# razvanmatisan/duodiff

Measured on AMD Instinct MI355X. Metric: images/sec (whole node) DuoDiff 1000-step CelebA-64, higher is better.
Workload: dtype bf16

## Files before the change

duodiff_amd/_lib.py:

```python
import ctypes as C
import os
from pathlib import Path

LIB_PATH = Path(os.environ.get("DUODIFF_LIB") or Path(__file__).resolve().parent / "libduodiff.so")

DD_OK = 0
DD_ERR_INVALID, DD_ERR_NOT_FOUND, DD_ERR_STATE, DD_ERR_HIP, DD_ERR_NOMEM, DD_ERR_UNSUPPORTED = -1, -2, -3, -4, -5, -6
DD_PREC_BF16, DD_PREC_FP32 = 0, 1
DD_VAR_BETA_TILDE, DD_VAR_BETA = 0, 1
DD_NOISE_NONE, DD_NOISE_BUFFER, DD_NOISE_PHILOX = 0, 1, 2
DD_X0_STATIC, DD_X0_DYNAMIC = 0, 1
DD_EE_MLP_PER_LAYER, DD_EE_MLP_PER_TIMESTEP, DD_EE_MLP_PER_LAYER_PER_TIMESTEP, DD_EE_ATTENTION_PROBE = 0, 1, 2, 3
ABI_VERSION = 6
DD_DEV_NO_FUSED_MLP, DD_DEV_NO_FUSED_PROJ, DD_DEV_NO_FUSED_HEAD, DD_DEV_GENERIC_EMBED, DD_DEV_MLP_EXTRAS_ONLY = 1, 2, 4, 8, 16
DD_DEV_NO_FUSED_SKIP, DD_DEV_NO_FUSED_QKV, DD_DEV_NO_FUSED_QA = 32, 64, 128
DD_PROF_DOMINANT, DD_PROF_BLOCK_TAIL, DD_PROF_FC1, DD_PROF_ROWLIN, DD_PROF_QKV_ATTENTION, DD_PROF_SPLITK = 0, 1, 2, 3, 4, 5
DD_DEV_NO_CHAINS, DD_DEV_FORCE_CHAINS, DD_DEV_NO_ROWLIN, DD_DEV_NO_ROWLIN_PROJ, DD_DEV_NO_EMBED_LN, DD_DEV_NO_SPLITK, DD_DEV_NO_ROWLIN_SKIP = 256, 512, 1024, 2048, 4096, 8192, 16384
DD_DEV_NO_SPLIT_HEADS = 32768


class dd_config(C.Structure):
    _fields_ = [(n, C.c_int32) for n in (
        "img_size", "patch_size", "in_chans", "embed_dim", "depth", "num_heads", "mlp_ratio",
        "num_classes", "normalize_timesteps", "max_batch", "qkv_bias", "mlp_time_embed")]


class dd_sample_args(C.Structure):
    _fields_ = [("first", C.c_void_p), ("late", C.c_void_p), ("t_switch", C.c_int32),
                ("t_start", C.c_int32), ("t_end", C.c_int32), ("variance", C.c_int32),
                ("noise_mode", C.c_int32), ("use_graph", C.c_int32), ("seed", C.c_uint64),
                ("y_dev", C.c_void_p), ("x_dev", C.c_void_p), ("B", C.c_int32), ("reserved", C.c_int32)]


class dd_affine_sample_args(C.Structure):
    _fields_ = [("first", C.c_void_p), ("late", C.c_void_p), ("n_steps", C.c_int32), ("switch_after", C.c_int32),
                ("t", C.POINTER(C.c_float)), ("a", C.POINTER(C.c_float)), ("b", C.POINTER(C.c_float)),
                ("c", C.POINTER(C.c_float)), ("noise", C.POINTER(C.c_int32)), ("noise_mode", C.c_int32),
                ("use_graph", C.c_int32), ("seed", C.c_uint64), ("y_dev", C.c_void_p), ("x_dev", C.c_void_p),
                ("B", C.c_int32), ("counter_base", C.c_int32)]


class dd_multistep_sample_args(C.Structure):
    _fields_ = dd_affine_sample_args._fields_ + [
        ("d", C.POINTER(C.c_float)), ("p", C.POINTER(C.c_float)), ("q", C.POINTER(C.c_float)), ("hist", C.POINTER(C.c_int32)),
        ("h_dev", C.c_void_p)]


class dd_guidance(C.Structure):
    _fields_ = [("scale", C.c_float), ("null_label", C.c_int32)]


class dd_autoguidance(C.Structure):
    _fields_ = [("guide", C.c_void_p), ("scale", C.c_float)]


class dd_pag(C.Structure):
    _fields_ = [("scale", C.c_float), ("layers_first", C.c_uint32), ("layers_late", C.c_uint32)]


class dd_known_region(C.Structure):
    _fields_ = [("x0_dev", C.c_void_p), ("mask_dev", C.c_void_p), ("ka", C.POINTER(C.c_float)), ("kb", C.POINTER(C.c_float))]


class dd_x0_threshold(C.Structure):
    _fields_ = [("mode", C.c_int32), ("quantile", C.c_float), ("range", C.c_float), ("s_max", C.c_float)]


class dd_ee_sample_args(C.Structure):
    _fields_ = [("model", C.c_void_p), ("threshold", C.c_float), ("t_start", C.c_int32), ("t_end", C.c_int32),
                ("noise_mode", C.c_int32), ("use_graph", C.c_int32), ("B", C.c_int32), ("seed", C.c_uint64),
                ("y_dev", C.c_void_p), ("x_dev", C.c_void_p), ("err_dev", C.c_void_p), ("idx_dev", C.c_void_p)]


SIGNATURES = {
    "dd_abi_version": (C.c_int, []),
    "dd_build_id": (C.c_char_p, []),
    "dd_ctx_create": (C.c_int, [C.c_int, C.POINTER(C.c_void_p)]),
    "dd_ctx_destroy": (None, [C.c_void_p]),
    "dd_last_error": (C.c_char_p, [C.c_void_p]),
    "dd_sync": (C.c_int, [C.c_void_p, C.c_void_p]),
    "dd_schedule_table": (C.c_int, [C.c_int, C.POINTER(C.c_float)]),
    "dd_schedule_build": (C.c_int, [C.c_float, C.c_float, C.c_int] + [C.POINTER(C.c_float)] * 5),
    "dd_model_create": (C.c_int, [C.c_void_p, C.POINTER(dd_config), C.POINTER(C.c_void_p)]),
    "dd_model_set_param": (C.c_int, [C.c_void_p, C.c_char_p, C.c_void_p, C.POINTER(C.c_int64), C.c_int]),
    "dd_model_finalize": (C.c_int, [C.c_void_p, C.c_int]),
    "dd_model_num_params": (C.c_int64, [C.c_void_p]),
    "dd_model_destroy": (None, [C.c_void_p]),
    "dd_forward": (C.c_int, [C.c_void_p, C.c_void_p, C.c_void_p, C.c_float, C.c_void_p, C.c_void_p, C.c_void_p, C.c_int, C.c_void_p]),
    "dd_model_enable_early_exit": (C.c_int, [C.c_void_p, C.c_int]),
    "dd_forward_early_exit": (C.c_int, [C.c_void_p, C.c_void_p, C.c_void_p, C.c_float, C.c_void_p, C.c_void_p, C.c_void_p,
                                        C.c_void_p, C.c_void_p, C.c_int, C.c_void_p]),
    "dd_early_exit_select": (C.c_int, [C.c_void_p, C.c_void_p, C.c_void_p, C.c_void_p, C.c_float, C.c_int, C.c_int, C.c_int64,
                                       C.c_void_p, C.c_void_p, C.c_void_p, C.c_void_p]),
    "dd_ddpm_step": (C.c_int, [C.c_void_p, C.c_void_p, C.c_void_p, C.c_void_p, C.c_int, C.c_int, C.c_void_p, C.c_int64, C.c_void_p]),
    "dd_ddpm_step_coef": (C.c_int, [C.c_void_p, C.c_void_p, C.c_void_p, C.c_void_p, C.c_float, C.c_float, C.c_float,
                                    C.c_void_p, C.c_int64, C.c_void_p]),
    "dd_affine_step": (C.c_int, [C.c_void_p, C.c_void_p, C.c_void_p, C.c_void_p, C.c_float, C.c_float, C.c_float,
                                 C.c_void_p, C.c_int64, C.c_void_p]),
    "dd_sample_step": (C.c_int, [C.c_void_p, C.c_void_p, C.c_void_p, C.c_int, C.c_void_p, C.c_int, C.c_void_p,
                                 C.c_uint64, C.c_int, C.c_void_p, C.c_int, C.c_void_p]),
    "dd_to_images": (C.c_int, [C.c_void_p, C.c_void_p, C.c_void_p, C.c_int, C.c_int, C.c_int, C.c_void_p]),
    "dd_sample": (C.c_int, [C.c_void_p, C.POINTER(dd_sample_args), C.c_void_p]),
    "dd_sample_affine": (C.c_int, [C.c_void_p, C.POINTER(dd_affine_sample_args), C.c_void_p]),
    "dd_sample_early_exit": (C.c_int, [C.c_void_p, C.POINTER(dd_ee_sample_args), C.c_void_p]),
    "dd_forward_guided": (C.c_int, [C.c_void_p, C.c_void_p, C.c_void_p, C.c_float, C.c_void_p, C.POINTER(dd_guidance), C.c_void_p,
                                    C.c_int, C.c_void_p]),
    "dd_sample_guided": (C.c_int, [C.c_void_p, C.POINTER(dd_sample_args), C.POINTER(dd_guidance), C.c_void_p]),
    "dd_sample_affine_guided": (C.c_int, [C.c_void_p, C.POINTER(dd_affine_sample_args), C.POINTER(dd_guidance), C.c_void_p]),
    "dd_multistep_step": (C.c_int, [C.c_void_p, C.c_void_p, C.c_void_p, C.c_void_p, C.c_void_p] + [C.c_float] * 6 +
                          [C.c_int, C.c_void_p, C.c_int64, C.c_void_p]),
    "dd_sample_multistep": (C.c_int, [C.c_void_p, C.POINTER(dd_multistep_sample_args), C.c_void_p]),
    "dd_sample_multistep_guided": (C.c_int, [C.c_void_p, C.POINTER(dd_multistep_sample_args), C.POINTER(dd_guidance), C.c_void_p]),
    "dd_forward_autoguided": (C.c_int, [C.c_void_p, C.c_void_p, C.c_void_p, C.c_float, C.c_void_p, C.POINTER(dd_autoguidance), C.c_void_p,
                                        C.c_int, C.c_void_p]),
    "dd_sample_autoguided": (C.c_int, [C.c_void_p, C.POINTER(dd_sample_args), C.POINTER(dd_autoguidance), C.c_void_p]),
    "dd_sample_affine_autoguided": (C.c_int, [C.c_void_p, C.POINTER(dd_affine_sample_args), C.POINTER(dd_autoguidance), C.c_void_p]),
    "dd_sample_multistep_autoguided": (C.c_int, [C.c_void_p, C.POINTER(dd_multistep_sample_args), C.POINTER(dd_autoguidance), C.c_void_p]),
    "dd_forward_perturbed": (C.c_int, [C.c_void_p, C.c_void_p, C.c_void_p, C.c_float, C.c_void_p, C.POINTER(dd_pag), C.c_void_p,
                                       C.c_int, C.c_void_p]),
    "dd_sample_perturbed": (C.c_int, [C.c_void_p, C.POINTER(dd_sample_args), C.POINTER(dd_pag), C.c_void_p]),
    "dd_sample_affine_perturbed": (C.c_int, [C.c_void_p, C.POINTER(dd_affine_sample_args), C.POINTER(dd_pag), C.c_void_p]),
    "dd_sample_multistep_perturbed": (C.c_int, [C.c_void_p, C.POINTER(dd_multistep_sample_args), C.POINTER(dd_pag), C.c_void_p]),
    "dd_known_blend": (C.c_int, [C.c_void_p] * 5 + [C.c_float, C.c_float, C.c_void_p, C.c_int, C.c_int, C.c_int, C.c_void_p]),
    "dd_sample_region": (C.c_int, [C.c_void_p, C.POINTER(dd_sample_args), C.POINTER(dd_guidance), C.POINTER(dd_autoguidance),
                                   C.POINTER(dd_known_region), C.c_void_p]),
    "dd_sample_affine_region": (C.c_int, [C.c_void_p, C.POINTER(dd_affine_sample_args), C.POINTER(dd_guidance), C.POINTER(dd_autoguidance),
                                          C.POINTER(dd_known_region), C.c_void_p]),
    "dd_sample_multistep_region": (C.c_int, [C.c_void_p, C.POINTER(dd_multistep_sample_args), C.POINTER(dd_guidance),
                                             C.POINTER(dd_autoguidance), C.POINTER(dd_known_region), C.c_void_p]),
    "dd_threshold_step": (C.c_int, [C.c_void_p] * 5 + [C.POINTER(dd_x0_threshold)] + [C.c_float] * 6 +
                          [C.c_int, C.c_void_p, C.c_int, C.c_int, C.c_int, C.c_void_p]),
    "dd_sample_multistep_threshold": (C.c_int, [C.c_void_p, C.POINTER(dd_multistep_sample_args), C.POINTER(dd_guidance),
                                                C.POINTER(dd_autoguidance), C.POINTER(dd_known_region), C.POINTER(dd_x0_threshold), C.c_void_p]),
    "dd_bench_gemm": (C.c_int, [C.c_void_p, C.c_void_p, C.c_int, C.c_int, C.c_void_p, C.POINTER(C.c_float), C.POINTER(C.c_double)]),
    "dd_vae_create": (C.c_int, [C.c_void_p, C.c_int, C.c_int, C.POINTER(C.c_void_p)]),
    "dd_vae_set_param": (C.c_int, [C.c_void_p, C.c_char_p, C.c_void_p, C.POINTER(C.c_int64), C.c_int]),
    "dd_vae_finalize": (C.c_int, [C.c_void_p, C.c_int]),
    "dd_vae_decode": (C.c_int, [C.c_void_p, C.c_void_p, C.c_void_p, C.c_void_p, C.c_int, C.c_int, C.c_void_p]),
    "dd_vae_destroy": (None, [C.c_void_p]),
    "dd_vae_has_encoder": (C.c_int, [C.c_void_p]),
    "dd_vae_encode": (C.c_int, [C.c_void_p, C.c_void_p, C.c_void_p, C.c_void_p, C.c_void_p, C.c_void_p, C.c_int, C.c_int, C.c_void_p]),
    "dd_vae_sample": (C.c_int, [C.c_void_p, C.c_void_p, C.c_void_p, C.c_void_p, C.c_int, C.c_int, C.c_void_p]),
    "dd_profile_steps": (C.c_int, [C.c_void_p, C.c_void_p, C.c_void_p, C.c_void_p, C.c_int, C.c_int, C.c_int, C.c_void_p,
                                   C.POINTER(C.c_float), C.POINTER(C.c_int)]),
    "dd_profile_steps_chained": (C.c_int, [C.c_void_p, C.c_void_p, C.c_void_p, C.c_void_p, C.c_int, C.c_int, C.c_int, C.c_void_p,
                                           C.POINTER(C.c_float), C.POINTER(C.c_int)]),
    "dd_profile_select": (C.c_int, [C.c_void_p, C.c_int]),
    "dd_dev_qkv_attention": (C.c_int, [C.c_void_p, C.c_int, C.c_int, C.c_int, C.c_int, C.c_void_p, C.c_void_p, C.c_void_p, C.c_void_p,
                                       C.c_int, C.c_void_p, C.POINTER(C.c_float)]),
    "dd_dev_qkv_attention_rows": (C.c_int, [C.c_void_p, C.c_int, C.c_int, C.c_int, C.c_int] + [C.c_void_p] * 6 + [C.c_int, C.c_void_p, C.POINTER(C.c_float)]),
    "dd_dev_v_identity": (C.c_int, [C.c_void_p, C.c_int, C.c_int, C.c_int, C.c_int] + [C.c_void_p] * 6 + [C.c_int, C.c_void_p, C.POINTER(C.c_float)]),
    "dd_dev_v_copy": (C.c_int, [C.c_void_p] + [C.c_int] * 4 + [C.c_void_p] * 2 + [C.c_int, C.c_void_p, C.POINTER(C.c_float)]),
    "dd_dev_mlp": (C.c_int, [C.c_void_p, C.c_int, C.c_int, C.c_int, C.c_int] + [C.c_void_p] * 10 + [C.c_int, C.c_void_p, C.POINTER(C.c_float)] + [C.c_void_p] * 8),
    "dd_dev_block_tail": (C.c_int, [C.c_void_p] + [C.c_int] * 7 + [C.c_void_p] * 21 + [C.c_int, C.c_void_p, C.c_int, C.c_void_p, C.POINTER(C.c_float)]),
    "dd_dev_head_dec": (C.c_int, [C.c_void_p] + [C.c_int] * 5 + [C.c_void_p] * 9 + [C.c_int, C.c_int, C.c_void_p, C.POINTER(C.c_float)]),
    "dd_dev_gemm": (C.c_int, [C.c_void_p] + [C.c_int] * 5 + [C.c_void_p] * 4 + [C.c_int] * 6 + [C.c_void_p] + [C.c_int] * 2 + [C.c_void_p] * 2 +
                    [C.c_int] + [C.c_void_p] * 3 + [C.c_int, C.c_int, C.c_void_p, C.POINTER(C.c_float)]),
    "dd_dev_rowlin": (C.c_int, [C.c_void_p] + [C.c_int] * 6 + [C.c_void_p] * 5 + [C.c_void_p] * 3 + [C.c_int, C.c_int, C.c_void_p, C.POINTER(C.c_float)]),
    "dd_dev_attention": (C.c_int, [C.c_void_p] + [C.c_int] * 4 + [C.c_void_p] * 4 + [C.c_int, C.c_void_p, C.POINTER(C.c_float)]),
    "dd_dev_layernorm": (C.c_int, [C.c_void_p] + [C.c_int] * 3 + [C.c_void_p] * 4 + [C.c_int] * 3 + [C.c_void_p, C.POINTER(C.c_float)]),
    "dd_dev_embed": (C.c_int, [C.c_void_p] + [C.c_int] * 9 + [C.c_void_p] * 7 + [C.c_float] + [C.c_void_p] * 3 + [C.c_int, C.c_void_p, C.POINTER(C.c_float)]),
    "dd_dev_time_mlp": (C.c_int, [C.c_void_p] + [C.c_int] * 5 + [C.c_void_p] * 6 + [C.c_float, C.c_void_p, C.c_int, C.c_void_p, C.POINTER(C.c_float)]),
    "dd_dev_vae_gather": (C.c_int, [C.c_void_p] + [C.c_int] * 6 + [C.c_void_p, C.c_void_p, C.c_size_t, C.c_void_p]),
    "dd_dev_poison_workspaces": (C.c_int, [C.c_void_p, C.c_void_p, C.c_void_p]),
    "dd_dev_graph_captures": (C.c_longlong, [C.c_void_p]),
    "dd_dev_last_sample_chains": (C.c_int, [C.c_void_p]),
    "dd_dev_set_flags": (C.c_int, [C.c_void_p, C.c_uint]),
    "dd_set_num_cus": (C.c_int, [C.c_void_p, C.c_int]),
    "dd_plan_rows": (C.c_int, [C.c_int, C.c_int, C.c_int, C.c_int, C.POINTER(C.c_int), C.POINTER(C.c_int)]),
    "dd_last_sample_timing": (C.c_int, [C.c_void_p, C.POINTER(C.c_float)]),
}

_lib = None


class EngineUnavailable(RuntimeError):
    """libduodiff.so is missing or unusable.  There is no CPU path to fall back to."""


def load():
    global _lib
    if _lib is not None:
        return _lib
    if not LIB_PATH.exists():
        raise EngineUnavailable(
            f"{LIB_PATH} not found: build it with `python -m duodiff_amd.build` "
            "(hipcc --offload-arch=gfx950).  duodiff_amd has no CPU fallback.")
    try:
        lib = C.CDLL(str(LIB_PATH))
    except OSError as e:
        raise EngineUnavailable(f"cannot load {LIB_PATH}: {e}") from e
    lib.dd_abi_version.restype = C.c_int
    if lib.dd_abi_version() != ABI_VERSION:
        raise EngineUnavailable(f"{LIB_PATH}: ABI version {lib.dd_abi_version()}, this package binds version {ABI_VERSION}; rebuild")
    for name, (res, args) in SIGNATURES.items():
        try:
            fn = getattr(lib, name)
        except AttributeError:
            if name.startswith("dd_dev_"):
                continue
            raise
        fn.restype = res
        fn.argtypes = args
    _lib = lib
    return lib
```

duodiff_amd/csrc/attention.hip:

```cpp
#include "dd_internal.h"
#include "wave_prims.h"

#include <type_traits>
#include <utility>

namespace dd {
namespace {

constexpr int kMaxKeyTiles = 9;
constexpr int kLP = kMaxKeyTiles * 32;
constexpr int kHD = 64;
constexpr int kPartBytes = 4 * 2 * 66 * 4;

__device__ __forceinline__ int k_swz(int r) { return ((r >> 1) & 7) ^ ((r & 1) << 2); }
__device__ __forceinline__ int v_swz(int r) { return (2 * (r & 3)) ^ ((r >> 2) & 1); }

template <typename T> struct AttnLayout;
template <> struct AttnLayout<bf16_t> {
    static constexpr int kRowK = 128;
    static constexpr int kRowV = 128;
    static constexpr int kVBytes = kLP * kRowV;
};
template <> struct AttnLayout<float> {
    static constexpr int kRowK = 256 + 16;
// ... 252 lines not shown
        f32x16 o[2];
        float mx, sum;
        attend_tiles<T, NKT, kMaxKeyTiles, false>(Ks, Vt, L, nkt, lane, [&](int k) { return k < nkt ? k : -1; }, qcur, o, mx, sum);
        const float inv = 1.0f / sum;

        T* orow = out + ((long long)b * L + (q < L ? q : L - 1)) * D + hh * kHD;
        if constexpr (sizeof(T) == 2) {
#pragma unroll
            for (int dt = 0; dt < 2; ++dt) {
                uint2 v[4];
#pragma unroll
                for (int g = 0; g < 4; ++g) {
                    bf16_t v4[4];
#pragma unroll
                    for (int e = 0; e < 4; ++e) v4[e] = f2bf(o[dt][4 * g + e] * inv);
                    v[g] = *reinterpret_cast<const uint2*>(v4);
                }
#pragma unroll
                for (int gp = 0; gp < 4; gp += 2) {
                    const auto s0 = __builtin_amdgcn_permlane32_swap(v[gp].x, v[gp + 1].x, false, false);
                    const auto s1 = __builtin_amdgcn_permlane32_swap(v[gp].y, v[gp + 1].y, false, false);
                    const uint4 o4 = {s0[0], s1[0], s0[1], s1[1]};
                    if (q < L) *reinterpret_cast<uint4*>(orow + dt * 32 + 8 * gp + 8 * half) = o4;
                }
            }
        } else if (q < L) {
#pragma unroll
            for (int dt = 0; dt < 2; ++dt)
#pragma unroll
                for (int g = 0; g < 4; ++g) {
                    const int d = dt * 32 + 8 * g + 4 * half;
                    *reinterpret_cast<f32x4*>(orow + d) = f32x4{o[dt][4 * g] * inv, o[dt][4 * g + 1] * inv, o[dt][4 * g + 2] * inv, o[dt][4 * g + 3] * inv};
                }
        }
    }

    if constexpr (SPLIT_LAST) {
        float* part = reinterpret_cast<float*>(smem + kLP * Lay::kRowK + Lay::kVBytes);
        const int rem = L - 256;
        f32x16 o[2];
        float mx, sum;
        attend_tiles<T, NKT, 3, false>(Ks, Vt, L, nkt, lane, [&](int k) { return k < 2 ? wave + 4 * k : (wave == 3 ? 8 : -1); }, qnext, o, mx, sum);
        if (r32 < rem) {
            float* pw = part + (wave * 2 + r32) * 66;
#pragma unroll
            for (int dt = 0; dt < 2; ++dt)
#pragma unroll
                for (int g = 0; g < 4; ++g)
                    *reinterpret_cast<f32x4*>(pw + dt * 32 + 8 * g + 4 * half) =
                        f32x4{o[dt][4 * g], o[dt][4 * g + 1], o[dt][4 * g + 2], o[dt][4 * g + 3]};
            if (half == 0) { pw[64] = mx; pw[65] = sum; }
        }
        __syncthreads();
        if (tid < rem * 64) {
            const int qi = tid >> 6, d = tid & 63;
            float m[4], M = -INFINITY;
#pragma unroll
            for (int w = 0; w < 4; ++w) { m[w] = part[(w * 2 + qi) * 66 + 64]; M = fmaxf(M, m[w]); }
            float num = 0.f, den = 0.f;
#pragma unroll
            for (int w = 0; w < 4; ++w) {
                float f;
                if constexpr (sizeof(T) == 2) f = __builtin_amdgcn_exp2f((m[w] - M) * (0.125f * 1.4426950408889634f));
                else f = expf((m[w] - M) * 0.125f);
                num = fmaf(f, part[(w * 2 + qi) * 66 + d], num);
                den = fmaf(f, part[(w * 2 + qi) * 66 + 65], den);
            }
            out[((long long)b * L + 256 + qi) * D + hh * kHD + d] = Elem<T>::from_f32(num / den);
        }
    }
}


struct QkvAttnArgs {
    const bf16_t* h;
    const bf16_t* wimg;
    const float* bias;
    const bf16_t* hx;
    const float* xres;
    const float* ln_g;
    const float* ln_b;
    bf16_t* out;
    int B, L, H, Lp, E;
};

constexpr int kQaPxBytes = 8 * 6 * 2 * 32 * 4;
constexpr int kQaHxPad = 64;
constexpr int kQaHxBytes = 2 * (1024 * 2 + kQaHxPad);
constexpr int kQaAuxBytes = kQaPxBytes + kQaHxBytes + 256;
constexpr int kQaKQ = 8;
constexpr int kQaBlk = 2 * kQaKQ * 1024;
constexpr int kQaRing = 4 * kQaBlk;
static_assert(8 * 2 * 66 * 4 <= kQaPxBytes, "the split chunk's partials reuse the px area");

constexpr int qa_dma_ops(int b, int nb) { return b < nb ? 2 : 0; }
constexpr int qa_pref_ops(int b, int nb) { return (b >= 0 && b % 3 == 0 && b / 3 + 1 < nb / 3) ? kQaKQ : 0; }
constexpr int qa_younger_dma(int b, int nb) { return qa_pref_ops(b - 1, nb) + qa_dma_ops(b + 2, nb) + qa_pref_ops(b, nb); }
constexpr int qa_younger_rows(int b, int nb) { return qa_dma_ops(b, nb) + qa_dma_ops(b + 1, nb) + qa_dma_ops(b + 2, nb); }

template <int D>
__global__ void __launch_bounds__(512, 1) qkv_attention_kernel(const QkvAttnArgs a) {
    using Lay = AttnLayout<bf16_t>;
    constexpr int KS = D / 16, NS = KS / kQaKQ, NB = 3 * NS;
    static_assert(D % 128 == 0 && D >= 512 && D <= 1024, "k range in slices of 8 k-steps; hxl holds two rows of D <= 1024");
    extern __shared__ __attribute__((aligned(16))) char smem[];
    char* Ks = smem;
    char* Vt = smem + kLP * Lay::kRowK;
    float* px = reinterpret_cast<float*>(smem + kLP * Lay::kRowK + Lay::kVBytes);
    float* part = px;
    char* hxl = smem + kLP * Lay::kRowK + Lay::kVBytes + kQaPxBytes;
    char* qxl = hxl + kQaHxBytes;
    char* ring = smem + kLP * Lay::kRowK + Lay::kVBytes + kQaAuxBytes;

    int b, hh;
    if ((a.B & 7) == 0) { const int slot = blockIdx.x >> 3; b = (blockIdx.x & 7) + 8 * (slot / a.H); hh = slot % a.H; }
    else { b = blockIdx.x / a.H; hh = blockIdx.x % a.H; }
    const int tid = threadIdx.x, lane = tid & 63, wave = __builtin_amdgcn_readfirstlane(tid >> 6);
    const int half = lane >> 5, r32 = lane & 31;
    const int L = a.L, E = a.E;

    const char* wsrc = reinterpret_cast<const char*>(a.wimg) + (size_t)hh * NB * kQaBlk;
    const unsigned lane16 = lane * 16;
    auto dma_block = [&](int bb) {
#pragma unroll
        for (int i = 0; i < 2; ++i) {
            const int pc = wave * 2 + i;
            lds_dma16s(wsrc + (size_t)bb * kQaBlk + pc * 1024, lane16, ring + (bb & 3) * kQaBlk + pc * 1024);
        }
    };
    dma_block(0);
    dma_block(1);
    dma_block(2);

    const int row = 32 * wave + r32;
    const bf16x8* hfr_u = reinterpret_cast<const bf16x8*>(a.h) + ((long long)b * 8 + wave) * KS * 64;
    const bf16x8* hfr = hfr_u + lane;
    bf16x8 xs[2][kQaKQ];
#pragma unroll
    for (int ks = 0; ks < kQaKQ; ++ks) xs[0][ks] = hfr[ks * 64];

    if (a.hx) {
        for (int i = tid; i < E * (D / 8); i += 512) {
            const int e = i / (D / 8), cch = i % (D / 8);
            *reinterpret_cast<f32x4*>(hxl + e * (D * 2 + kQaHxPad) + cch * 16) = *reinterpret_cast<const f32x4*>(a.hx + ((long long)b * L + e) * D + cch * 8);
        }
    } else if (wave < E) {
        constexpr int NV = D / 256;
        const float* xr = a.xres + ((long long)b * L + wave) * D + lane * (D / 64);
        f32x4 xv[NV];
        float s1 = 0.f;
#pragma unroll
        for (int v = 0; v < NV; ++v) {
            xv[v] = *reinterpret_cast<const f32x4*>(xr + 4 * v);
            s1 += (xv[v][0] + xv[v][1]) + (xv[v][2] + xv[v][3]);
        }
        const float mean = wave_reduce_add(s1) / (float)D;
        float s2 = 0.f;
#pragma unroll
        for (int v = 0; v < NV; ++v) {
            xv[v] = xv[v] - mean;
            s2 += (xv[v][0] * xv[v][0] + xv[v][1] * xv[v][1]) + (xv[v][2] * xv[v][2] + xv[v][3] * xv[v][3]);
        }
        const float rstd = 1.0f / sqrtf(wave_reduce_add(s2) / (float)D + 1e-5f);
#pragma unroll
        for (int v = 0; v < NV; ++v) {
            const f32x4 g = *reinterpret_cast<const f32x4*>(a.ln_g + lane * (D / 64) + 4 * v), c0 = *reinterpret_cast<const f32x4*>(a.ln_b + lane * (D / 64) + 4 * v);
// ... 51 lines not shown
                        const bf16x8 wa = *reinterpret_cast<const bf16x8*>(ring + (bb & 3) * kQaBlk + t * (kQaKQ * 1024) + wx16);
                        accx[2 * jj + t] = __builtin_amdgcn_mfma_f32_16x16x32_bf16(wa, hb, accx[2 * jj + t], 0, 0, 0);
                    }
                }
                const bf16x8 w0 = wq[f & 3];
                if (f + 4 < 2 * kQaKQ) wq[f & 3] = *reinterpret_cast<const bf16x8*>(wb + (f + 4) * 1024);
                else if (bb + 1 < NB) wq[f & 3] = *reinterpret_cast<const bf16x8*>(wbn + (f + 4 - 2 * kQaKQ) * 1024);
                acc[2 * jj + (f >> 3)] = __builtin_amdgcn_mfma_f32_32x32x16_bf16(w0, xs[S][f & 7], acc[2 * jj + (f >> 3)], 0, 0, 0);
            }
        }(), ...);
    }(std::make_integer_sequence<int, NB>{});

    if (xn < E) {
#pragma unroll
        for (int j = 0; j < 6; ++j) *reinterpret_cast<f32x4*>(px + (((wave * 6 + j) * 2 + xn) * 16 + 4 * xg)) = accx[j];
    }
    f32x4 qcur[4];
    const int swk = k_swz(row), swv = v_swz(row);
#pragma unroll
    for (int j = 0; j < 6; ++j) {
        if (a.bias) {
            const float* bj = a.bias + (j >> 1) * D + hh * kHD + 32 * (j & 1) + 4 * half;
#pragma unroll
            for (int g = 0; g < 4; ++g) {
                const f32x4 bv = *reinterpret_cast<const f32x4*>(bj + 8 * g);
#pragma unroll
                for (int e = 0; e < 4; ++e) acc[j][4 * g + e] += bv[e];
            }
        }
        unsigned pk[8];
#pragma unroll
        for (int i = 0; i < 8; ++i) pk[i] = cvt_pk_bf16(acc[j][2 * i], acc[j][2 * i + 1]);
        const int T = j & 1;
        if (j < 2) {
            qcur[2 * T] = __builtin_bit_cast(f32x4, uint4{pk[0], pk[1], pk[2], pk[3]});
            qcur[2 * T + 1] = __builtin_bit_cast(f32x4, uint4{pk[4], pk[5], pk[6], pk[7]});
        } else if (j < 4) {
            *reinterpret_cast<uint4*>(Ks + row * 128 + (((4 * T + 2 * half) ^ swk) << 4)) = uint4{pk[0], pk[1], pk[2], pk[3]};
            *reinterpret_cast<uint4*>(Ks + row * 128 + (((4 * T + 2 * half + 1) ^ swk) << 4)) = uint4{pk[4], pk[5], pk[6], pk[7]};
        } else {
#pragma unroll
            for (int gp = 0; gp < 4; gp += 2) {
                const auto s0 = __builtin_amdgcn_permlane32_swap(pk[2 * gp], pk[2 * gp + 2], false, false);
                const auto s1 = __builtin_amdgcn_permlane32_swap(pk[2 * gp + 1], pk[2 * gp + 3], false, false);
                *reinterpret_cast<uint4*>(Vt + row * 128 + (((4 * T + gp + half) ^ swv) << 4)) = uint4{s0[0], s1[0], s0[1], s1[1]};
            }
        }
    }
    __syncthreads();
    if (tid < E * 192) {
        const int e = tid / 192, c = tid % 192, j = c >> 5, col = c & 31;
        float v = a.bias ? a.bias[(j >> 1) * D + hh * kHD + 32 * (j & 1) + col] : 0.f;
#pragma unroll
        for (int kb = 0; kb < 4; ++kb) v += px[(((2 * kb + (col >> 4)) * 6 + j) * 2 + e) * 16 + (col & 15)];
        const bf16_t vb = f2bf(v);
        const int d = 32 * (j & 1) + col, r = 256 + e;
        if (j < 2) {
            *reinterpret_cast<bf16_t*>(qxl + e * 128 + d * 2) = vb;
        } else if (j < 4) {
            const int T = d >> 5, dd = d & 31, hf = (dd >> 2) & 1, ae = (dd & 3) + 4 * (dd >> 3);
            *reinterpret_cast<bf16_t*>(Ks + r * 128 + (((4 * T + 2 * hf + (ae >> 3)) ^ k_swz(r)) << 4) + (ae & 7) * 2) = vb;
        } else {
            *reinterpret_cast<bf16_t*>(Vt + r * 128 + (((d >> 3) ^ v_swz(r)) << 4) + (d & 7) * 2) = vb;
        }
    }
    __syncthreads();

    f32x4 qe[4];
    {
        const bf16_t* qrow = reinterpret_cast<const bf16_t*>(qxl) + (r32 < E ? r32 : E - 1) * kHD + 4 * half;
#pragma unroll
        for (int st = 0; st < 4; ++st) {
            const uint2 lo = *reinterpret_cast<const uint2*>(qrow + 32 * (st >> 1) + 16 * (st & 1));
            const uint2 hi = *reinterpret_cast<const uint2*>(qrow + 32 * (st >> 1) + 16 * (st & 1) + 8);
            qe[st] = __builtin_bit_cast(f32x4, uint4{lo.x, lo.y, hi.x, hi.y});
        }
    }

    {
        f32x16 o[2];
        float mx, sum;
        attend_tiles<bf16_t, 9, kMaxKeyTiles, true>(Ks, Vt, L, kMaxKeyTiles, lane, [&](int k) { return k; }, qcur, o, mx, sum);
        const float inv = 1.0f / sum;
        bf16_t* orow = a.out + ((long long)b * L + E + row) * D + hh * kHD;
#pragma unroll
        for (int dt = 0; dt < 2; ++dt) {
            uint2 v[4];
#pragma unroll
            for (int g = 0; g < 4; ++g) {
                bf16_t v4[4];
#pragma unroll
                for (int e = 0; e < 4; ++e) v4[e] = f2bf(o[dt][4 * g + e] * inv);
                v[g] = *reinterpret_cast<const uint2*>(v4);
            }
#pragma unroll
            for (int gp = 0; gp < 4; gp += 2) {
                const auto s0 = __builtin_amdgcn_permlane32_swap(v[gp].x, v[gp + 1].x, false, false);
                const auto s1 = __builtin_amdgcn_permlane32_swap(v[gp].y, v[gp + 1].y, false, false);
                *reinterpret_cast<uint4*>(orow + dt * 32 + 8 * gp + 8 * half) = uint4{s0[0], s1[0], s0[1], s1[1]};
            }
        }
    }

    {
        f32x16 o[2];
        float mx, sum;
        attend_tiles<bf16_t, 9, 2, true>(Ks, Vt, L, kMaxKeyTiles, lane, [&](int k) { return k == 0 ? wave : (wave == 7 ? 8 : -1); }, qe, o, mx, sum);
        if (r32 < E) {
            float* pw = part + (wave * 2 + r32) * 66;
#pragma unroll
            for (int dt = 0; dt < 2; ++dt)
#pragma unroll
                for (int g = 0; g < 4; ++g)
                    *reinterpret_cast<f32x4*>(pw + dt * 32 + 8 * g + 4 * half) =
                        f32x4{o[dt][4 * g], o[dt][4 * g + 1], o[dt][4 * g + 2], o[dt][4 * g + 3]};
            if (half == 0) { pw[64] = mx; pw[65] = sum; }
        }
        __syncthreads();
        if (tid < E * 64) {
            const int qi = tid >> 6, d = tid & 63;
            float m[8], M = -INFINITY;
#pragma unroll
            for (int w = 0; w < 8; ++w) { m[w] = part[(w * 2 + qi) * 66 + 64]; M = fmaxf(M, m[w]); }
            float num = 0.f, den = 0.f;
#pragma unroll
            for (int w = 0; w < 8; ++w) {
                const float f = __builtin_amdgcn_exp2f((m[w] - M) * (0.125f * 1.4426950408889634f));
                num = fmaf(f, part[(w * 2 + qi) * 66 + d], num);
                den = fmaf(f, part[(w * 2 + qi) * 66 + 65], den);
            }
            a.out[((long long)b * L + qi) * D + hh * kHD + d] = f2bf(num / den);
        }
    }
}


struct VIdentityArgs {
    const bf16_t* h;
    const bf16_t* wimg;
    const float* bias;
    const float* xres;
    const float* ln_g;
    const float* ln_b;
    bf16_t* out;
    int B, L, E;
};

template <int D>
__global__ void __launch_bounds__(512, 1) v_identity_kernel(const VIdentityArgs a) {
    constexpr int KS = D / 16, NS = KS / kQaKQ, NT = D / 256;
    static_assert(D % 256 == 0 && D >= 512 && D <= 1024, "8 waves share D / 32 column tiles; a lane normalises D / 64 columns in float4s");
    extern __shared__ __attribute__((aligned(16))) char smem[];
    const int tid = threadIdx.x, lane = tid & 63, wave = __builtin_amdgcn_readfirstlane(tid >> 6);
    const int half = lane >> 5, r32 = lane & 31;
    const int L = a.L, E = a.E, n_extra = a.B * E;
    const int wg_patch = a.B * 4;
    const bool extra_wg = (int)blockIdx.x >= wg_patch;
    const int q0 = ((int)blockIdx.x - wg_patch) * 64;

    if (!extra_wg) {
        const f32x4* src = reinterpret_cast<const f32x4*>(a.h) + (size_t)blockIdx.x * (2 * KS * 64);
        for (int i = tid; i < 2 * KS * 64; i += 512) reinterpret_cast<f32x4*>(smem)[i] = src[i];
    } else {
        constexpr int NV = D / 256;
        for (int i = wave; i < 64; i += 8) {
            const int q = q0 + i;
            f32x4 y[NV];
#pragma unroll
            for (int v = 0; v < NV; ++v) y[v] = f32x4{0.f, 0.f, 0.f, 0.f};
            if (q < n_extra) {
                const int b = q / E, l = q - b * E;
                const float* xr = a.xres + ((long long)b * L + l) * D + lane * (D / 64);
                f32x4 xv[NV];
                float s1 = 0.f;
#pragma unroll
                for (int v = 0; v < NV; ++v) {
                    xv[v] = *reinterpret_cast<const f32x4*>(xr + 4 * v);
                    s1 += (xv[v][0] + xv[v][1]) + (xv[v][2] + xv[v][3]);
                }
                const float mean = wave_reduce_add(s1) / (float)D;
                float s2 = 0.f;
#pragma unroll
// ... 49 lines not shown
        const int q = idx % NS;
        if (idx + 1 < NT * NS) load_w(idx + 1, wb[(idx + 1) & 1]);
        if (q == 0) { acc[0] = zero16; acc[1] = zero16; }
#pragma unroll
        for (int ks = 0; ks < kQaKQ; ++ks) {
            const bf16x8 h0 = hl[(q * kQaKQ + ks) * 64], h1 = hl[(KS + q * kQaKQ + ks) * 64];
            acc[0] = __builtin_amdgcn_mfma_f32_32x32x16_bf16(wb[idx & 1][ks], h0, acc[0], 0, 0, 0);
            acc[1] = __builtin_amdgcn_mfma_f32_32x32x16_bf16(wb[idx & 1][ks], h1, acc[1], 0, 0, 0);
        }
        if (q == NS - 1) {
            const int T = wave + 8 * (idx / NS), col0 = 32 * T;
#pragma unroll
            for (int g = 0; g < 2; ++g) {
                if (a.bias) {
                    const float* bj = a.bias + 2 * D + col0 + 4 * half;
#pragma unroll
                    for (int gq = 0; gq < 4; ++gq) {
                        const f32x4 bv = *reinterpret_cast<const f32x4*>(bj + 8 * gq);
#pragma unroll
                        for (int e = 0; e < 4; ++e) acc[g][4 * gq + e] += bv[e];
                    }
                }
                unsigned pk[8];
#pragma unroll
                for (int i = 0; i < 8; ++i) pk[i] = cvt_pk_bf16(acc[g][2 * i], acc[g][2 * i + 1]);
                bf16_t* op = a.out + orow[g] * D + col0 + 8 * half;
#pragma unroll
                for (int gp = 0; gp < 4; gp += 2) {
                    const auto s0 = __builtin_amdgcn_permlane32_swap(pk[2 * gp], pk[2 * gp + 2], false, false);
                    const auto s1 = __builtin_amdgcn_permlane32_swap(pk[2 * gp + 1], pk[2 * gp + 3], false, false);
                    if (valid[g]) *reinterpret_cast<uint4*>(op + 8 * gp) = uint4{s0[0], s1[0], s0[1], s1[1]};
                }
            }
        }
    }
}

template <typename T>
__global__ void __launch_bounds__(256) v_copy_kernel(const T* __restrict__ qkv, T* __restrict__ out, long long n_chunks, int L, int H, int Lp) {
    constexpr int EPC = 16 / (int)sizeof(T), CPR = kHD / EPC;
    const long long idx = (long long)blockIdx.x * 256 + threadIdx.x;
    if (idx >= n_chunks) return;
    const int ch = (int)(idx % CPR);
    long long r = idx / CPR;
    const int hh = (int)(r % H);
    r /= H;
    const int l = (int)(r % L);
    const long long b = r / L;
    const T* src = qkv + (((b * 3 + 2) * H + hh) * Lp + l) * kHD + ch * EPC;
    *reinterpret_cast<f32x4*>(out + idx * EPC) = *reinterpret_cast<const f32x4*>(src);
}

}

template <typename T>
hipError_t launch_attention(const T* qkv, T* out, int B, int L, int H, int D, hipStream_t s) {
    if (L > kLP || D != H * kHD || L < 1) return hipErrorInvalidValue;
    using Lay = AttnLayout<T>;
    const size_t lds = (size_t)kLP * Lay::kRowK + (size_t)Lay::kVBytes + kPartBytes;
    const int Lp = make_head_major(L, H).Lp;
    if (L == 257 || L == 258) hipLaunchKernelGGL((attention_kernel<T, 9>), dim3(B * H), dim3(256), lds, s, qkv, out, B, L, H, D, Lp);
    else hipLaunchKernelGGL((attention_kernel<T, 0>), dim3(B * H), dim3(256), lds, s, qkv, out, B, L, H, D, Lp);
    return hipGetLastError();
}

void qkv_attention_pack(int D, int H, const float* w, unsigned short (*to_bf16)(float), unsigned short* img) {
    const int NS = D / 16 / kQaKQ;
    for (int hh = 0; hh < H; ++hh)
        for (int q = 0; q < NS; ++q)
            for (int j = 0; j < 6; ++j)
                for (int ks = 0; ks < kQaKQ; ++ks)
                    pack_fragment(w, D, (j >> 1) * D + 64 * hh + 32 * (j & 1), 16 * (q * kQaKQ + ks), FRAG_K_NATURAL, to_bf16,
                                  img + ((((size_t)hh * NS + q) * 6 + j) * kQaKQ + ks) * 512);
}

bool qkv_attention_supported(int D, int H, int L, int extras) {
    return (D == 512 || D == 768 || D == 1024) && H * kHD == D && (extras == 1 || extras == 2) && L == 256 + extras;
}

static size_t v_identity_lds(int D) { return (size_t)2 * (D / 16) * 1024; }
static size_t qkv_attention_lds() { return (size_t)kLP * AttnLayout<bf16_t>::kRowK + AttnLayout<bf16_t>::kVBytes + kQaAuxBytes + kQaRing; }

hipError_t launch_qkv_attention(const bf16_t* h, const bf16_t* wimg, const float* bias, const bf16_t* hx, const float* xres,
                                const float* ln_g, const float* ln_b, bf16_t* out, int B, int L, int H, int D, int extras, hipStream_t s) {
    if (!qkv_attention_supported(D, H, L, extras) || !h || !wimg || (!hx && (!xres || !ln_g || !ln_b)) || !out || B < 1) return hipErrorInvalidValue;
    const QkvAttnArgs a{h, wimg, bias, hx, xres, ln_g, ln_b, out, B, L, H, make_head_major(L, H).Lp, extras};
    switch (D) {
        case 512: hipLaunchKernelGGL((qkv_attention_kernel<512>), dim3(B * H), dim3(512), qkv_attention_lds(), s, a); break;
        case 768: hipLaunchKernelGGL((qkv_attention_kernel<768>), dim3(B * H), dim3(512), qkv_attention_lds(), s, a); break;
        default: hipLaunchKernelGGL((qkv_attention_kernel<1024>), dim3(B * H), dim3(512), qkv_attention_lds(), s, a); break;
    }
    return hipGetLastError();
}

hipError_t launch_v_identity(const bf16_t* h, const bf16_t* wimg, const float* bias, const float* xres, const float* ln_g, const float* ln_b,
                             bf16_t* out, int B, int L, int H, int D, int extras, hipStream_t s) {
    if (!qkv_attention_supported(D, H, L, extras) || !h || !wimg || !xres || !ln_g || !ln_b || !out || B < 1) return hipErrorInvalidValue;
    const VIdentityArgs a{h, wimg, bias, xres, ln_g, ln_b, out, B, L, extras};
    const dim3 grid(B * 4 + (B * extras + 63) / 64);
    switch (D) {
        case 512: hipLaunchKernelGGL((v_identity_kernel<512>), grid, dim3(512), v_identity_lds(512), s, a); break;
        case 768: hipLaunchKernelGGL((v_identity_kernel<768>), grid, dim3(512), v_identity_lds(768), s, a); break;
        default: hipLaunchKernelGGL((v_identity_kernel<1024>), grid, dim3(512), v_identity_lds(1024), s, a); break;
    }
    return hipGetLastError();
}

template <typename T>
hipError_t launch_v_copy(const T* qkv, T* out, int B, int L, int H, int D, hipStream_t s) {
    if (!qkv || !out || B < 1 || L < 1 || L > kLP || H < 1 || D != H * kHD) return hipErrorInvalidValue;
    const long long n_chunks = (long long)B * L * D / (16 / (int)sizeof(T));
    hipLaunchKernelGGL((v_copy_kernel<T>), dim3((unsigned)((n_chunks + 255) / 256)), dim3(256), 0, s, qkv, out, n_chunks, L, H, make_head_major(L, H).Lp);
    return hipGetLastError();
}

hipError_t init_attention_kernels() {
    for (const void* f : {(const void*)qkv_attention_kernel<512>, (const void*)qkv_attention_kernel<768>, (const void*)qkv_attention_kernel<1024>})
        if (hipError_t e = hipFuncSetAttribute(f, hipFuncAttributeMaxDynamicSharedMemorySize, (int)qkv_attention_lds()); e != hipSuccess) return e;
    if (hipError_t e = hipFuncSetAttribute((const void*)v_identity_kernel<512>, hipFuncAttributeMaxDynamicSharedMemorySize, (int)v_identity_lds(512)); e != hipSuccess) return e;
    if (hipError_t e = hipFuncSetAttribute((const void*)v_identity_kernel<768>, hipFuncAttributeMaxDynamicSharedMemorySize, (int)v_identity_lds(768)); e != hipSuccess) return e;
    if (hipError_t e = hipFuncSetAttribute((const void*)v_identity_kernel<1024>, hipFuncAttributeMaxDynamicSharedMemorySize, (int)v_identity_lds(1024)); e != hipSuccess) return e;
    const int lb = kLP * AttnLayout<bf16_t>::kRowK + AttnLayout<bf16_t>::kVBytes + kPartBytes;
    const int lf = kLP * AttnLayout<float>::kRowK + AttnLayout<float>::kVBytes + kPartBytes;
    hipError_t e = hipFuncSetAttribute((const void*)attention_kernel<bf16_t, 9>, hipFuncAttributeMaxDynamicSharedMemorySize, lb);
    if (e == hipSuccess) e = hipFuncSetAttribute((const void*)attention_kernel<bf16_t, 0>, hipFuncAttributeMaxDynamicSharedMemorySize, lb);
    if (e == hipSuccess) e = hipFuncSetAttribute((const void*)attention_kernel<float, 9>, hipFuncAttributeMaxDynamicSharedMemorySize, lf);
    if (e == hipSuccess) e = hipFuncSetAttribute((const void*)attention_kernel<float, 0>, hipFuncAttributeMaxDynamicSharedMemorySize, lf);
    return e;
}

template hipError_t launch_attention<bf16_t>(const bf16_t*, bf16_t*, int, int, int, int, hipStream_t);
template hipError_t launch_attention<float>(const float*, float*, int, int, int, int, hipStream_t);
template hipError_t launch_v_copy<bf16_t>(const bf16_t*, bf16_t*, int, int, int, int, hipStream_t);
template hipError_t launch_v_copy<float>(const float*, float*, int, int, int, int, hipStream_t);

}
```

duodiff_amd/csrc/capi.hip:

```cpp
#include "../../include/duodiff.h"
#include "../../include/duodiff_dev.h"
#include "dd_internal.h"
#include "dev_scope.h"
#include "host_arena.h"
#include "launch_args.h"

#include <algorithm>
#include <atomic>
#include <cmath>
#include <cstdio>
#include <cstdlib>
#include <cstring>
#include <functional>
#include <map>
#include <new>
#include <string>
#include <vector>

using namespace dd;

namespace dd {
hipError_t init_gemm_kernels();
hipError_t init_attention_kernels();
hipError_t init_rowops_kernels();
// ... 44 lines not shown
    hipEvent_t ev_fork = nullptr, ev_join = nullptr;
    hipEvent_t ev_ee_fork = nullptr, ev_ee_join = nullptr;
    StepCoef* coef = nullptr;
    StepCoef coef_host[1000];
    hipEvent_t ev[3] = {nullptr, nullptr, nullptr};
    float timing[3] = {0, 0, 0};
    int num_cus = 256;
    DevBuf<float> x_stage;
    DevBuf<int64_t> y_stage;
    long long graph_captures = 0;
    int last_chains = 1;
    RowTable<AffineRow> atab;
    RowTable<HistRow> htab;
    DevBuf<float> h_stage;
    RowTable<KnownRow> ktab;
    DevBuf<float> k_stage;
    DevBuf<float> m_stage;
    int prof_kind = 0;
    unsigned dev_flags = 0;
};

namespace {

struct HostParam {
    std::vector<float> data;
    std::vector<int64_t> shape;
    bool set = false;
};

struct BlockW {
    const float *ln1_g, *ln1_b, *ln2_g, *ln2_b, *proj_b, *fc1_b, *fc2_b, *skip_b, *qkv_b;
    const void *qkv_w, *proj_w, *fc1_w, *fc2_w, *skip_w;
    const char* mlp_img;
    const float* mlp_b1p;
    const bf16_t* qa_img;
    const char* rl_img = nullptr;
    const char* rlp_img = nullptr;
    const char* rls_img = nullptr;
};

struct HeadW { const float *ng, *nb, *wdec, *bdec, *wconv, *bconv; const float *wg = nullptr, *dc = nullptr; const float *wsplit = nullptr, *dcs = nullptr; };

struct GraphKey {
    const void* x; const void* y; int B, noise, variance, num_cus;
    const void* atab;
    const void *aux0 = nullptr, *aux1 = nullptr;
    float thr = 0.f;
    int b0 = 0;
    int gnull = -1;
    unsigned gscale = 0;
    const void* aguide = nullptr;
    unsigned long long aserial = 0;
    const void *kx0 = nullptr, *kmask = nullptr, *ktab = nullptr;
    int tmode = -1;
    unsigned tq = 0, tr = 0, ts = 0;
    const void* tscratch = nullptr;
    int pag = 0;
    unsigned pfirst = 0, plate = 0;
    bool operator==(const GraphKey& o) const {
        return x == o.x && y == o.y && B == o.B && noise == o.noise && variance == o.variance && num_cus == o.num_cus &&
               atab == o.atab && aux0 == o.aux0 && aux1 == o.aux1 && thr == o.thr && b0 == o.b0 && gnull == o.gnull && gscale == o.gscale &&
               aguide == o.aguide && aserial == o.aserial && kx0 == o.kx0 && kmask == o.kmask && ktab == o.ktab && tmode == o.tmode &&
               tq == o.tq && tr == o.tr && ts == o.ts && tscratch == o.tscratch && pag == o.pag && pfirst == o.pfirst && plate == o.plate;
    }
    void perturb(const dd_pag* p) {
        if (p) { pag = 1; gscale = __builtin_bit_cast(unsigned, p->scale); pfirst = p->layers_first; plate = p->layers_late; }
    }
    void guide(const dd_guidance* g) {
        if (g) { gnull = g->null_label; gscale = __builtin_bit_cast(unsigned, g->scale); }
    }
};

enum GraphKind { GRAPH_DDPM, GRAPH_AFFINE, GRAPH_EARLY_EXIT, GRAPH_MULTISTEP, GRAPH_KINDS };

}

struct WsPtrs {
    float* x = nullptr; void *h = nullptr, *ao = nullptr, *qkv = nullptr, *hid = nullptr, *xb = nullptr;
    std::vector<void*> skips;
    float* dec = nullptr;
    float* mlp_partial = nullptr;
    bf16_t* qkv_dump = nullptr;
    bf16_t* hfrag = nullptr;
    float* ytap = nullptr;
};

struct dd_model {
    dd_ctx* ctx = nullptr;
    unsigned long long serial = 0;
    dd_config cfg{};
    int D = 0, L = 0, N = 0, extras = 0, pd = 0, pdp = 0, H = 0, hidden = 0, hid_ld = 0, half_depth = 0, Mp_max = 0;
    std::map<std::string, HostParam> params;
    bool finalized = false;
    int prec = DD_PREC_BF16;
    size_t esize = 2;
    char* warena = nullptr;
    std::vector<BlockW> blocks;
    const float *emb_wt = nullptr, *emb_b = nullptr, *pos = nullptr, *label = nullptr;
    const float *tm_w1t = nullptr, *tm_b1 = nullptr, *tm_w2t = nullptr, *tm_b2 = nullptr;
    HeadW head{};
    int ee_type = -1, n_probe = 0;
    std::vector<HeadW> heads;
    const float *probe_w = nullptr, *probe_b = nullptr;
    std::vector<AttnProbeW> attn_probes;
    bool ee_conv_stride_ok = false;
    long long ee_wconv_stride = 0, ee_bconv_stride = 0;
    bool ee_batched = false;
    bool fused_mlp = false;
    bool fused_proj = false;
    bool fused_skip = false;
    bool fused_qkv = false;
    bool splitk = false;
    bool rowlin_skip = false;
    bool rowlin_proj = false;
    bool rowlin_fc2 = false;
    bool fused_qa = false;
    size_t ws_bytes[2] = {0, 0};
    char* wsarena[2] = {nullptr, nullptr};
    WsPtrs ws[2];
    hipGraphExec_t graph[GRAPH_KINDS][2] = {};
    GraphKey gkey[GRAPH_KINDS][2]{};
    float* ee_ws = nullptr;
    bool time_fc1 = false;
    std::vector<hipEvent_t> fc1_events;
    size_t fc1_used = 0;
};

namespace dd {
int ctx_fail(dd_ctx* c, int code, const std::string& msg) {
    if (c) c->err = msg;
    return code;
}
int ctx_device(dd_ctx* c) { return c->device; }
int ctx_num_cus(dd_ctx* c) { return c->num_cus; }
unsigned ctx_dev_flags(dd_ctx* c) { return c->dev_flags; }
}

namespace {

void base_tables(float beta_init, float beta_final, int n, float* betas, float* alphas, float* abar, float* abar_prev) {
    const float start = beta_init, end = beta_final;
    const float stepf = n > 1 ? (end - start) / (float)(n - 1) : 0.0f;
    const double step = (double)stepf;
    const int half = n / 2;
    for (int i = 0; i < n; ++i) {
        betas[i] = i < half ? (float)((double)start + step * i) : (float)((double)end - step * (n - 1 - i));
        alphas[i] = 1.0f - betas[i];
    }
    double run = 1.0;
    for (int i = 0; i < n; ++i) {
        run *= (double)alphas[i];
        abar[i] = (float)run;
    }
    for (int i = 0; i < n; ++i) abar_prev[i] = i ? abar[i - 1] : 1.0f;
}
float bt_sampler_order(float beta, float abar_prev, float abar) {
    volatile float num = beta * (1.0f - abar_prev);
    return num / (1.0f - abar);
}
float bt_scheduler_order(float beta, float abar_prev, float abar) {
    volatile float ratio = (1.0f - abar_prev) / (1.0f - abar);
    return ratio * beta;
}

struct Schedule {
    float betas[1000], alphas[1000], abar[1000], abar_prev[1000], bt_sampler[1000], bt_sched[1000];
    float c1[1000], c2[1000], sigma[1000], sigma_beta[1000];
    Schedule() {
        base_tables(1e-4f, 0.02f, 1000, betas, alphas, abar, abar_prev);
        for (int i = 0; i < 1000; ++i) {
            bt_sampler[i] = bt_sampler_order(betas[i], abar_prev[i], abar[i]);
            bt_sched[i] = bt_scheduler_order(betas[i], abar_prev[i], abar[i]);
            c1[i] = sqrtf(1.0f / alphas[i]);
            c2[i] = (1.0f - alphas[i]) / sqrtf(1.0f - abar[i]);
            sigma[i] = sqrtf(bt_sampler[i]);
            sigma_beta[i] = sqrtf(betas[i]);
        }
    }
};
const Schedule& schedule() {
    static const Schedule s;
    return s;
}

void probe_grid(const dd_model* m, int& nt, int& nl) {
    nt = m->ee_type == DD_EE_MLP_PER_LAYER || m->ee_type == DD_EE_ATTENTION_PROBE ? 1 : 1000;
    nl = m->ee_type == DD_EE_MLP_PER_TIMESTEP ? 1 : m->cfg.depth;
}
std::string probe_key(const dd_model* m, int layer, int t) {
    switch (m->ee_type) {
        case DD_EE_MLP_PER_LAYER:
        case DD_EE_ATTENTION_PROBE: return std::to_string(layer);
        case DD_EE_MLP_PER_TIMESTEP: return std::to_string(t);
        default: return std::to_string(layer) + ", " + std::to_string(t);
    }
}
std::string block_prefix(const dd_model* m, int bi) {
    if (bi < m->half_depth) return "in_blocks." + std::to_string(bi) + ".";
    if (bi == m->half_depth) return "mid_block.";
    return "out_blocks." + std::to_string(bi - m->half_depth - 1) + ".";
}
std::string head_prefix(const dd_model* m, int layer) {
    if (layer < m->half_depth) return "in_blocks_heads." + std::to_string(layer) + ".";
    if (layer == m->half_depth) return "mid_block_head.";
    return "out_blocks_heads." + std::to_string(layer - m->half_depth - 1) + ".";
}

std::map<std::string, HostParam> catalogue(const dd_model* m) {
    std::map<std::string, HostParam> c;
    const int64_t D = m->D, C = m->cfg.in_chans, P = m->cfg.patch_size, hid = m->hidden;
    auto add = [&](const std::string& n, std::vector<int64_t> shape) { c[n].shape = std::move(shape); };
    auto linear = [&](const std::string& n, int64_t out, int64_t in) { add(n + ".weight", {out, in}); add(n + ".bias", {out}); };
    auto head = [&](const std::string& p) {
        add(p + "norm.weight", {D}); add(p + "norm.bias", {D});
        linear(p + "decoder_pred", m->pd, D);
        add(p + "final_layer.weight", {C, C, 3, 3}); add(p + "final_layer.bias", {C});
    };
    add("pos_embed", {1, m->L, D});
    add("patch_embed.proj.weight", {D, C, P, P}); add("patch_embed.proj.bias", {D});
    if (m->cfg.mlp_time_embed) { linear("time_embed.0", 4 * D, D); linear("time_embed.2", D, 4 * D); }
    if (m->cfg.num_classes > 0) add("label_emb.weight", {m->cfg.num_classes, D});
    for (int bi = 0; bi < m->cfg.depth; ++bi) {
        const std::string p = block_prefix(m, bi);
        add(p + "norm1.weight", {D}); add(p + "norm1.bias", {D});
        add(p + "attn.qkv.weight", {3 * D, D});
        if (m->cfg.qkv_bias) add(p + "attn.qkv.bias", {3 * D});
        linear(p + "attn.proj", D, D);
        add(p + "norm2.weight", {D}); add(p + "norm2.bias", {D});
        linear(p + "mlp.fc1", hid, D); linear(p + "mlp.fc2", D, hid);
        if (bi > m->half_depth) linear(p + "skip_linear", D, 2 * D);
    }
    head("");
    if (m->ee_type < 0) return c;
    for (int layer = 0; layer < m->cfg.depth; ++layer) head(head_prefix(m, layer));
    int nt, nl;
    probe_grid(m, nt, nl);
    for (int t = 0; t < nt; ++t)
        for (int layer = 0; layer < nl; ++layer) {
            const std::string p = "matrix." + probe_key(m, layer, t) + ".";
            if (m->ee_type == DD_EE_ATTENTION_PROBE) {
                add(p + "q", {1, 1, 1, D});
                linear(p + "weight_kv", 2 * D, D); linear(p + "classification.0", D, D); linear(p + "classification.2", 1, D);
            } else {
                linear(p + "classifier.0", 1, D);
            }
        }
    return c;
}

void ws_layout(const dd_model* m, int batch, WsPtrs& w, Arena& a) {
    const int D = m->D, L = m->L, hid = m->hidden;
    const size_t es = m->esize;
    const size_t Mp = (size_t)round_up(batch * L, 256);
    const size_t qkv_elems = (size_t)batch * 3 * D * (size_t)make_head_major(L, m->H).Lp;
    a.space(w.x, Mp * D * 4); a.space(w.h, Mp * D * es); a.space(w.ao, Mp * D * es); a.space(w.qkv, std::max(Mp * 3 * D, qkv_elems) * es);
    a.space(w.hid, Mp * (size_t)m->hid_ld * es); a.space(w.xb, Mp * D * es);
    w.skips.assign(m->half_depth, nullptr);
    for (void*& sk : w.skips) a.space(sk, Mp * D * es);
    a.space(w.dec, Mp * m->pd * 4);
    const size_t part_bytes = m->fused_mlp ? mlp_fused_partial_bytes(batch, m->extras, D, hid)
                              : m->splitk ? (size_t)2 * Mp * D * 4
                              : m->rowlin_fc2 ? std::max(std::max(rowlin_partial_bytes(batch, m->extras, hid), rowlin_partial_bytes(batch, m->extras, 2 * D)), rowlin_partial_bytes(batch, m->extras, D)) : 0;
    if (part_bytes) a.space(w.mlp_partial, part_bytes);
    if (m->fused_qkv) a.space(w.qkv_dump, 16384);
    if (m->fused_qa) a.space(w.hfrag, (size_t)batch * m->N * D * 2);
    if (m->ee_type >= 0 && m->fused_skip) a.space(w.ytap, Mp * D * 4);
}
void choose_paths(dd_model* m, int precision, unsigned flags) {
    const int D = m->D, hid = m->hidden, L = m->L;
    m->fused_mlp = precision == DD_PREC_BF16 && mlp_fused_supported(D, hid) && !(flags & DD_DEV_NO_FUSED_MLP);
    m->fused_proj = m->fused_mlp && D % 128 == 0 && !(flags & DD_DEV_NO_FUSED_PROJ);
    m->fused_skip = m->fused_proj && (hid / 32) % 2 == 0 && !(flags & DD_DEV_NO_FUSED_SKIP);
    m->fused_qkv = m->fused_proj && m->ee_type < 0 && (hid / 32) % 2 == 0 && !m->cfg.qkv_bias && !(flags & DD_DEV_NO_FUSED_QKV);
    m->fused_qa = precision == DD_PREC_BF16 && qkv_attention_supported(D, m->H, L, m->extras) && !(flags & DD_DEV_NO_FUSED_QA);
    m->rowlin_fc2 = precision == DD_PREC_BF16 && !m->fused_mlp && rowlin_supported(D, hid) && m->N % 32 == 0 && !(flags & DD_DEV_NO_ROWLIN);
    m->rowlin_proj = m->rowlin_fc2 && !(flags & DD_DEV_NO_ROWLIN_PROJ);
    m->rowlin_skip = m->rowlin_fc2 && rowlin_supported(D, 2 * D) && !(flags & DD_DEV_NO_ROWLIN_SKIP);
    m->splitk = precision == DD_PREC_BF16 && !m->fused_mlp && !m->rowlin_fc2 && D % 256 == 0 && !(flags & DD_DEV_NO_SPLITK) &&
                (long long)(m->cfg.max_batch * L / 256) * (D / 256) * 2 <= device_num_cus() &&
                (hid / 64) % 2 == 0;
    for (int b = 1; m->splitk && b <= m->cfg.max_batch; ++b)
        m->splitk = gemm_splitk_supported(b * L, D, D, D, 2);
}

const std::vector<float>& param(const dd_model* m, const std::string& name) { return m->params.at(name).data; }

void pack_block(dd_model* m, Arena& a, int bi, const std::string& next_skip, const std::string& next_qkv) {
    const int D = m->D, hid = m->hidden;
    const std::string p = block_prefix(m, bi);
    auto P = [&](const std::string& n) -> const std::vector<float>& { return param(m, n); };
    BlockW& w = m->blocks[bi];
    a.f32(w.ln1_g, P(p + "norm1.weight")); a.f32(w.ln1_b, P(p + "norm1.bias"));
    a.f32(w.ln2_g, P(p + "norm2.weight")); a.f32(w.ln2_b, P(p + "norm2.bias"));
    a.f32(w.proj_b, P(p + "attn.proj.bias"));
    a.f32(w.fc1_b, P(p + "mlp.fc1.bias")); a.f32(w.fc2_b, P(p + "mlp.fc2.bias"));
    a.mat(w.qkv_w, P(p + "attn.qkv.weight")); a.mat(w.proj_w, P(p + "attn.proj.weight"));
    if (m->cfg.qkv_bias) a.f32(w.qkv_b, P(p + "attn.qkv.bias"));
    a.mat(w.fc1_w, P(p + "mlp.fc1.weight")); a.mat(w.fc2_w, P(p + "mlp.fc2.weight"));
    const bool skip = bi > m->half_depth;
    if (skip) { a.f32(w.skip_b, P(p + "skip_linear.bias")); a.mat(w.skip_w, P(p + "skip_linear.weight")); }
    if (m->fused_mlp) {
        const bool with_skip = m->fused_skip && !next_skip.empty();
        const bool with_qkv = m->fused_qkv && !m->fused_qa && !next_qkv.empty() && (next_skip.empty() || with_skip);
        const MlpImage im = MlpImage::of(D, hid, m->fused_proj, with_skip, with_qkv);
        char* img = a.raw(w.mlp_img, im.bytes());
        auto section = [&](size_t block) { return (unsigned short*)(img + im.at(block)); };
        std::vector<float> b1p(hid);
        if (m->fused_proj) mlp_fused_pack_proj(D, P(p + "attn.proj.weight").data(), host_f2bf, section(0));
        mlp_fused_pack(D, hid, P(p + "mlp.fc1.weight").data(), P(p + "mlp.fc1.bias").data(), P(p + "mlp.fc2.weight").data(), true, host_f2bf,
                       section(im.mlp), b1p.data());
        if (with_skip) mlp_fused_pack_skip(D, P(next_skip + "skip_linear.weight").data(), host_f2bf, section(im.skip));
        if (with_qkv) mlp_fused_pack_rows(D, 3 * D, P(next_qkv + "attn.qkv.weight").data(), host_f2bf, section(im.qkv));
        a.f32(w.mlp_b1p, b1p);
    }
    if (m->fused_qa)
        qkv_attention_pack(D, m->H, P(p + "attn.qkv.weight").data(), host_f2bf, (unsigned short*)a.raw(w.qa_img, (size_t)3 * D * D * 2));
    if (m->rowlin_fc2) {
        rowlin_pack(hid, P(p + "mlp.fc2.weight").data(), host_f2bf, (unsigned short*)a.raw(w.rl_img, (size_t)D * hid * 2));
        rowlin_pack(D, P(p + "attn.proj.weight").data(), host_f2bf, (unsigned short*)a.raw(w.rlp_img, (size_t)D * D * 2));
        if (skip) rowlin_pack(2 * D, P(p + "skip_linear.weight").data(), host_f2bf, (unsigned short*)a.raw(w.rls_img, (size_t)D * 2 * D * 2));
    }
}

void pack_embed(dd_model* m, Arena& a) {
    const int D = m->D, pd = m->pd;
    auto P = [&](const std::string& n) -> const std::vector<float>& { return param(m, n); };
    std::vector<float> wt((size_t)pd * D);
    const std::vector<float>& pe = P("patch_embed.proj.weight");
    for (int d = 0; d < D; ++d) for (int k = 0; k < pd; ++k) wt[(size_t)k * D + d] = pe[(size_t)d * pd + k];
    a.f32(m->emb_wt, wt); a.f32(m->emb_b, P("patch_embed.proj.bias")); a.f32(m->pos, P("pos_embed"));
    if (m->cfg.num_classes > 0) a.f32(m->label, P("label_emb.weight"));
    if (m->cfg.mlp_time_embed) {
        const std::vector<float>&w1 = P("time_embed.0.weight"), &w2 = P("time_embed.2.weight");
        std::vector<float> w1t((size_t)D * 4 * D), w2t((size_t)4 * D * D);
        for (int j = 0; j < 4 * D; ++j) for (int k = 0; k < D; ++k) w1t[(size_t)k * 4 * D + j] = w1[(size_t)j * D + k];
        for (int d = 0; d < D; ++d) for (int k = 0; k < 4 * D; ++k) w2t[(size_t)k * D + d] = w2[(size_t)d * 4 * D + k];
        a.f32(m->tm_w1t, w1t); a.f32(m->tm_b1, P("time_embed.0.bias"));
        a.f32(m->tm_w2t, w2t); a.f32(m->tm_b2, P("time_embed.2.bias"));
    }
}

void pack_head(const dd_model* m, Arena& a, const std::string& p, HeadW& h, bool fused, bool split) {
    const int D = m->D, pd = m->pd;
    auto P = [&](const std::string& n) -> const std::vector<float>& { return param(m, n); };
    const std::vector<float>&ng = P(p + "norm.weight"), &nb = P(p + "norm.bias"), &wd = P(p + "decoder_pred.weight"), &bd = P(p + "decoder_pred.bias");
    a.f32(h.ng, ng); a.f32(h.nb, nb); a.f32(h.wdec, wd); a.f32(h.bdec, bd);
    a.f32(h.wconv, P(p + "final_layer.weight")); a.f32(h.bconv, P(p + "final_layer.bias"));
    if (!fused) return;
    std::vector<float> wg, dc;
    fold_head_norm(D, pd, wd.data(), bd.data(), ng.data(), nb.data(), wg, dc);
    a.f32(h.wg, wg); a.f32(h.dc, dc);
    if (!split) return;
    const size_t img_bytes = (size_t)(D / 32) * ((pd + 15) / 16) * 2 * 64 * 8 * 2;
    std::vector<float> dcs(dc);
    pack_head_split(D, pd, wg.data(), host_f2bf, (unsigned short*)a.raw(h.wsplit, img_bytes), dcs.data() + pd);
    a.f32(h.dcs, dcs);
}
// ... 34 lines not shown
        for (int layer = 0; layer < nl; ++layer) {
            const std::string pre = "matrix." + probe_key(m, layer, t) + ".classifier.0.";
            const int row = t * nl + layer;
            std::memcpy(&pw[(size_t)row * D], P(pre + "weight").data(), (size_t)D * 4);
            pb[row] = P(pre + "bias")[0];
        }
    a.f32(m->probe_w, pw); a.f32(m->probe_b, pb);
}

struct Chain {
    const WsPtrs* ws;
    StepState* st;
    int cus;
    bool ee_fork;
};
Chain whole_batch(dd_ctx* c, dd_model* m) { return Chain{&m->ws[0], c->st[0], c->num_cus, true}; }

struct Known {
    const float* x0 = nullptr;
    const float* mask = nullptr;
    const KnownRow* ktab = nullptr;
    Known at(int b0, const dd_model* m) const {
        if (!x0) return *this;
        const size_t hw = (size_t)m->cfg.img_size * m->cfg.img_size;
        return Known{x0 + (size_t)b0 * hw * m->cfg.in_chans, mask + (size_t)b0 * hw, ktab};
    }
};

struct Mods {
    const dd_guidance* g = nullptr;
    const dd_autoguidance* ag = nullptr;
    const dd_known_region* kr = nullptr;
    bool region = false;
    Known kn{};
    const char* missing = nullptr;
    const dd_x0_threshold* thr = nullptr;
    bool thresholded = false;
    const dd_pag* pag = nullptr;
    const dd_model* pag_late = nullptr;
    unsigned pag_mask(const dd_model* m) const { return !pag ? 0u : (pag_late && m == pag_late) ? pag->layers_late : pag->layers_first; }
};
Mods guided(const dd_guidance* g) { return Mods{.g = g, .missing = g ? nullptr : "null dd_guidance"}; }
Mods perturbed(const dd_pag* p, const dd_model* late) {
    Mods mo{};
    mo.pag = p; mo.pag_late = late; mo.missing = p ? nullptr : "null dd_pag";
    return mo;
}
Mods autoguided(const dd_autoguidance* ag) { return Mods{.ag = ag, .missing = ag ? nullptr : "null dd_autoguidance"}; }
Mods in_region(const dd_guidance* g, const dd_autoguidance* ag, const dd_known_region* kr) { return Mods{.g = g, .ag = ag, .kr = kr, .region = true}; }
Mods thresholding(const dd_guidance* g, const dd_autoguidance* ag, const dd_known_region* kr, const dd_x0_threshold* thr) {
    return Mods{.g = g, .ag = ag, .kr = kr, .region = kr != nullptr, .thr = thr, .thresholded = true};
}

const char* check_threshold(const dd_x0_threshold* t) {
    if (!t) return "null dd_x0_threshold";
    if (t->mode == DD_X0_STATIC) return t->range > 0.f && std::isfinite(t->range) ? nullptr : "dd_x0_threshold: range must be positive and finite";
    if (t->mode != DD_X0_DYNAMIC) return "dd_x0_threshold: unknown mode";
    if (!(t->quantile > 0.f && t->quantile <= 1.f)) return "dd_x0_threshold: quantile outside (0, 1]";
    if (!(t->s_max >= 1.f)) return "dd_x0_threshold: s_max must be at least 1 (it may be +inf)";
    return nullptr;
}
X0Threshold kernel_threshold(const dd_x0_threshold* t, long long n) {
    if (t->mode == DD_X0_STATIC) return X0Threshold{0, 0, 0.f, t->range, 0.f};
    const double pos = (double)t->quantile * (double)(n - 1);
    const double i = std::floor(pos);
    return X0Threshold{1, (int)i, (float)(pos - i), 0.f, t->s_max};
}

FinalArgs final_args(const dd_model* m, const Chain& ch, const float* dec, const float* wconv, const float* bconv, int B) {
    FinalArgs fa{};
    fa.dec = dec; fa.wconv = wconv; fa.bconv = bconv;
    fa.st = ch.st; fa.coef = m->ctx->coef;
    fa.B = B; fa.C = m->cfg.in_chans; fa.S = m->cfg.img_size; fa.P = m->cfg.patch_size; fa.L = m->L; fa.extras = m->extras;
    return fa;
}

struct EeTaps { float* cls; float* outs; int t; };

struct Handoff {
    bool h = false;
    bool frag = false;
    bool qkv = false;
    bool skip = false;
};

template <typename T>
struct Backbone {
    static constexpr bool bf16 = sizeof(T) == 2;
    dd_model* m;
    const Chain& ch;
    int B;
    hipStream_t s;
    const EeTaps* ee;
    int pert_first = 0;
    unsigned pert_mask = 0;
    dd_ctx* c = m->ctx;
    const WsPtrs& ws = *ch.ws;
    const int D = m->D, L = m->L, M = B * L, nb = (int)m->blocks.size();
    const int prof = c->prof_kind == DD_PROF_DOMINANT ? ((bf16 && m->fused_mlp) ? DD_PROF_BLOCK_TAIL : DD_PROF_FC1) : c->prof_kind;
    T *h = (T*)ws.h, *ao = (T*)ws.ao, *qkv = (T*)ws.qkv, *hid = (T*)ws.hid, *xb = (T*)ws.xb;
    float* ee_dec_all = ee && m->ee_batched ? (float*)ws.hid : nullptr;
    float* ee_srow_all = ee_dec_all ? ee_dec_all + (size_t)nb * M * m->pd : nullptr;

    int mark(int kind) {
        if (!m->time_fc1 || kind != prof) return DD_OK;
        while (m->fc1_events.size() < m->fc1_used + 1) {
            hipEvent_t e;
            DD_HIP(c, hipEventCreate(&e));
            m->fc1_events.push_back(e);
        }
        DD_HIP(c, hipEventRecord(m->fc1_events[m->fc1_used++], s));
        return DD_OK;
    }
#define DD_TIMED(kind, expr) \
    do { if (int rc_ = mark(kind)) return rc_; DD_HIP(c, expr); if (int rc_ = mark(kind)) return rc_; } while (0)

    int tile128(int N, int K, int K1) const { return bf16 && gemm_prefers_128(m->cfg.max_batch * L, N, K, K1, c->num_cus) ? 1 : 0; }
    const T* skip_of(int bi) const { return (const T*)ws.skips[nb - 1 - bi]; }
    Handoff norm1_written() const { return Handoff{!m->fused_qa, m->fused_qa}; }

    int rowlin_then_reduce(const GemmArgs<bf16_t>& g, int resid, const char* wimg, const float* ln_g, const float* ln_b, bool frag) {
        const RowLinArgs ra = rowlin_args(g, resid, wimg, ws.mlp_partial, ln_g, ln_b, (bf16_t*)h, frag ? ws.hfrag : nullptr, B, m->N, m->extras);
        DD_TIMED(DD_PROF_ROWLIN, launch_rowlin(ra, s));
        DD_HIP(c, launch_mlp_reduce(rowlin_reduce_args(ra), D, s));
        return DD_OK;
    }
    int splitk_then_reduce_ln(GemmArgs<bf16_t> g, int resid, const float* ln_g, const float* ln_b, bool frag) {
        g.partial = ws.mlp_partial; g.splits = 2;
        DD_TIMED(DD_PROF_SPLITK, launch_gemm_splitk(g, s, ch.cus));
        DD_HIP(c, launch_reduce_ln(splitk_reduce_args(g, resid, ln_g, ln_b, (bf16_t*)h, frag ? ws.hfrag : nullptr, L, m->extras), D, s));
        return DD_OK;
    }

    int embed(const float* x_img, const float* t_vec, const int64_t* y_dev, Handoff& first) {
        EmbedArgs ea{x_img, m->emb_wt, m->emb_b, m->pos, m->label, (const long long*)y_dev, t_vec, ch.st, ws.x,
                     B, m->cfg.in_chans, m->cfg.img_size, m->cfg.patch_size, D, L, m->extras,
                     m->cfg.num_classes, m->cfg.normalize_timesteps, round_up(M, 256), (c->dev_flags & DD_DEV_GENERIC_EMBED) ? 1 : 0};
        if constexpr (bf16) {
            if (m->fused_qa && !(c->dev_flags & DD_DEV_NO_EMBED_LN) && embed_ln_supported(ea)) {
                ea.ln_g = m->blocks[0].ln1_g; ea.ln_b = m->blocks[0].ln1_b; ea.ln_frag = ws.hfrag;
                first.frag = true;
            }
        }
        DD_HIP(c, launch_embed(ea, s));
        if (m->tm_w1t) {
            TimeMlpArgs ta{m->tm_w1t, m->tm_b1, m->tm_w2t, m->tm_b2, m->pos, t_vec, ch.st, ws.x, B, D, L, m->extras, m->cfg.normalize_timesteps};
            DD_HIP(c, launch_time_mlp(ta, s));
        }
        return DD_OK;
    }

    int ee_taps(int bi, const Handoff& in, bool& side) {
        if (!ee) return DD_OK;
        const HeadW& hd = m->heads[bi];
        const float* xin = (in.skip && ws.ytap) ? ws.ytap : ws.x;
        side = bi <= m->half_depth && ch.ee_fork && c->side && s != c->side;
        hipStream_t hs = side ? c->side : s;
        if (side) {
            DD_HIP(c, hipEventRecord(c->ev_ee_fork, s));
            DD_HIP(c, hipStreamWaitEvent(c->side, c->ev_ee_fork, 0));
        }
        const int t_mul = m->ee_type == DD_EE_MLP_PER_LAYER ? 0 : m->ee_type == DD_EE_MLP_PER_TIMESTEP ? 1 : nb;
        const int add = m->ee_type == DD_EE_MLP_PER_TIMESTEP ? 0 : bi;
        bool probe_done = false;
        if (hd.wg) {
            HeadDecArgs ha{xin, hd.wg, hd.dc, ee_dec_all ? ee_dec_all + (size_t)bi * M * m->pd : ws.dec, M, m->pd, (L - m->extras) % 16 == 0 ? L : 0, m->extras};
            if (hd.wsplit) { ha.wg = hd.wsplit; ha.c = hd.dcs; ha.split = 1; }
            if (ee_srow_all && m->ee_type != DD_EE_ATTENTION_PROBE && head_dec_probe_supported(D)) {
                ha.srow = ee_srow_all + (size_t)bi * B * L; ha.pw_base = m->probe_w; ha.pb_base = m->probe_b; ha.st = ch.st; ha.t_mul = t_mul; ha.add = add;
                probe_done = true;
            }
            DD_HIP(c, launch_head_dec(ha, D, ch.cus, hs));
        } else {
            float* hf = (float*)ws.hid;
            DD_HIP(c, launch_layernorm<float>(xin, hd.ng, hd.nb, hf, M, D, hs));
            GemmArgs<float> g{hf, nullptr, hd.wdec, hd.bdec, ws.dec, nullptr, M, m->pd, D, D, D, 0, m->pd};
            DD_HIP(c, launch_gemm<float>(g, EPI_BIAS_SET, hs, ch.cus));
        }
        if (!ee_dec_all) {
            const long long chw = (long long)m->cfg.in_chans * m->cfg.img_size * m->cfg.img_size;
            FinalArgs fa = final_args(m, ch, ws.dec, hd.wconv, hd.bconv, B);
            fa.eps_out = ee->outs + (long long)bi * B * chw;
            DD_HIP(c, launch_final(fa, hs));
        }
        if (m->ee_type == DD_EE_ATTENTION_PROBE) {
            DD_HIP(c, launch_ee_attn_probe(xin, m->attn_probes[bi], ee->cls + (long long)bi * B, B, L, D, hs));
        } else if (!probe_done) {
            if (ee_srow_all) DD_HIP(c, launch_ee_probe(xin, m->probe_w, m->probe_b, nullptr, ee_srow_all + (size_t)bi * B * L, B, L, D, ch.st, t_mul, add, hs));
            else DD_HIP(c, launch_ee_probe(xin, m->probe_w, m->probe_b, ee->cls + (long long)bi * B, (float*)ws.hid, B, L, D, ch.st, t_mul, add, hs));
        }
        if (side) DD_HIP(c, hipEventRecord(c->ev_ee_join, c->side));
        return DD_OK;
    }

    int skip_linear(int bi, Handoff& hand) {
        if (bi <= m->half_depth || hand.skip) return DD_OK;
        const BlockW& w = m->blocks[bi];
        GemmArgs<T> g{xb, skip_of(bi), (const T*)w.skip_w, w.skip_b, ws.x, nullptr, M, D, 2 * D, D, D, D, D};
        g.tile128 = tile128(D, 2 * D, D);
        if constexpr (bf16) {
            if (m->rowlin_skip || m->splitk) hand = norm1_written();
            if (m->rowlin_skip) return rowlin_then_reduce(g, 0, w.rls_img, w.ln1_g, w.ln1_b, m->fused_qa);
            if (m->splitk) return splitk_then_reduce_ln(g, 0, w.ln1_g, w.ln1_b, m->fused_qa);
        }
        DD_HIP(c, launch_gemm<T>(g, EPI_BIAS_SET, s, ch.cus));
        return DD_OK;
    }

    int norm1_attention(int bi, const Handoff& in) {
        const BlockW& w = m->blocks[bi];
        bool qa = in.frag;
        if (!in.h && !in.frag && !in.qkv) {
            if (bf16 && m->fused_qa) {
                DD_HIP(c, launch_layernorm_frag(ws.x, w.ln1_g, w.ln1_b, (bf16_t*)h, ws.hfrag, M, D, L, m->extras, s));
                qa = true;
            } else {
                DD_HIP(c, launch_layernorm<T>(ws.x, w.ln1_g, w.ln1_b, h, M, D, s));
            }
        }
        const bool masked = (pert_mask >> bi) & 1u;
        const int Bn = masked ? pert_first : B, Bi = B - Bn;
        if (qa) {
            if constexpr (bf16) {
                if (Bn > 0)
                    DD_TIMED(DD_PROF_QKV_ATTENTION, launch_qkv_attention(ws.hfrag, w.qa_img, w.qkv_b, nullptr, ws.x, w.ln1_g, w.ln1_b, (bf16_t*)ao, Bn, L, m->H, D, m->extras, s));
                if (Bi > 0)
                    DD_HIP(c, launch_v_identity(ws.hfrag + (size_t)Bn * m->N * D, w.qa_img, w.qkv_b, ws.x + (size_t)Bn * L * D, w.ln1_g, w.ln1_b,
                                                (bf16_t*)ao + (size_t)Bn * L * D, Bi, L, m->H, D, m->extras, s));
            }
            return DD_OK;
        }
        if (!in.qkv) {
            GemmArgs<T> g{h, nullptr, (const T*)w.qkv_w, w.qkv_b, nullptr, qkv, M, 3 * D, D, D, D, 0, 3 * D};
            g.hm = make_head_major(L, m->H);
            DD_HIP(c, launch_gemm<T>(g, w.qkv_b ? EPI_BIAS_STORE : EPI_STORE, s, ch.cus));
        }
        if (Bn > 0) DD_TIMED(DD_PROF_QKV_ATTENTION, launch_attention<T>(qkv, ao, Bn, L, m->H, D, s));
        if (Bi > 0)
            DD_HIP(c, launch_v_copy<T>(qkv + (size_t)Bn * 3 * D * make_head_major(L, m->H).Lp, ao + (size_t)Bn * L * D, Bi, L, m->H, D, s));
        return DD_OK;
    }

    int proj(int bi) {
        const BlockW& w = m->blocks[bi];
        GemmArgs<T> g{ao, nullptr, (const T*)w.proj_w, w.proj_b, ws.x, nullptr, M, D, D, D, D, 0, D};
        g.tile128 = tile128(D, D, D);
        if constexpr (bf16) {
            if (m->rowlin_proj) return rowlin_then_reduce(g, 1, w.rlp_img, w.ln2_g, w.ln2_b, false);
            if (m->splitk) return splitk_then_reduce_ln(g, 1, w.ln2_g, w.ln2_b, false);
            if (m->fused_proj) return DD_OK;
        }
        DD_HIP(c, launch_gemm<T>(g, EPI_BIAS_RESID, s, ch.cus));
        if (!(bf16 && m->fused_mlp)) DD_HIP(c, launch_layernorm<T>(ws.x, w.ln2_g, w.ln2_b, h, M, D, s));
        return DD_OK;
    }

    int mlp(int bi, Handoff& next) {
        const BlockW& w = m->blocks[bi];
        const bool is_in = bi < m->half_depth;
        const BlockW* wn = bi + 1 < nb ? &m->blocks[bi + 1] : nullptr;
        T* copy = is_in ? (T*)ws.skips[bi] : (wn ? xb : nullptr);
        next = Handoff{};
        if constexpr (bf16) {
            if (m->fused_mlp) return block_tail(bi, copy, next);
        }
        GemmArgs<T> g1{h, nullptr, (const T*)w.fc1_w, w.fc1_b, nullptr, hid, M, m->hidden, D, D, D, 0, m->hid_ld};
        g1.tile128 = tile128(m->hidden, D, D);
        DD_TIMED(DD_PROF_FC1, launch_gemm<T>(g1, EPI_BIAS_GELU, s, ch.cus));
        GemmArgs<T> g{hid, nullptr, (const T*)w.fc2_w, w.fc2_b, ws.x, copy, M, D, m->hidden, m->hidden, m->hid_ld, m->hid_ld, D};
        g.tile128 = tile128(D, m->hidden, m->hidden);
        if constexpr (bf16) {
            const float *ln_g = is_in ? wn->ln1_g : nullptr, *ln_b = is_in ? wn->ln1_b : nullptr;
            if (is_in && (m->rowlin_fc2 || m->splitk)) next = norm1_written();
            if (m->rowlin_fc2) return rowlin_then_reduce(g, 1, w.rl_img, ln_g, ln_b, m->fused_qa);
            if (m->splitk) return splitk_then_reduce_ln(g, 1, ln_g, ln_b, m->fused_qa);
        }
        DD_HIP(c, launch_gemm<T>(g, EPI_BIAS_RESID, s, ch.cus));
        return DD_OK;
    }

    int block_tail(int bi, T* copy, Handoff& next) {
        const BlockW& w = m->blocks[bi];
        MlpFusedArgs fa{};
        fa.X = nullptr; fa.ldx = D; fa.wimg = w.mlp_img; fa.b1p = w.mlp_b1p; fa.b2 = w.fc2_b;
        fa.ln_in_g = w.ln2_g; fa.ln_in_b = w.ln2_b;
        fa.xres = ws.x; fa.out = (bf16_t*)copy; fa.ldo = D; fa.partial = ws.mlp_partial;
        if (m->fused_proj) { fa.ao = (const bf16_t*)ao; fa.bproj = w.proj_b; fa.nproj = D / 32; }
        next.skip = m->fused_skip && bi >= m->half_depth && bi + 1 < nb;
        if (next.skip) {
            fa.skip = (const bf16_t*)skip_of(bi + 1);
            if (ee) fa.y_tap = ws.ytap;
            fa.bskip = m->blocks[bi + 1].skip_b; fa.nskip = D / 16;
        }
        const bool h_next = bi < m->half_depth || next.skip;
        next.frag = m->fused_qa && h_next;
        next.qkv = !next.frag && m->fused_qkv && h_next;
        next.h = h_next && !next.frag && !next.qkv;
        if (h_next) { fa.ln_out_g = m->blocks[bi + 1].ln1_g; fa.ln_out_b = m->blocks[bi + 1].ln1_b; fa.ln_out = (bf16_t*)h; }
        if (next.frag) fa.ln_out_frag = ws.hfrag;
        if (next.qkv) { fa.qkv_out = (bf16_t*)qkv; fa.qkv_dump = ws.qkv_dump; fa.hm = make_head_major(L, m->H); fa.nqkv = 3 * D / 32; }
        mlp_fused_plan(B, m->N, m->extras, L, m->hidden, fa);
        if (bi + 1 == nb && m->fused_proj) { fa.n_extra = 0; fa.tiles_left = 0; }
        if (m->fused_proj) fa.reduce_set = 1;
        DD_TIMED(DD_PROF_BLOCK_TAIL, launch_mlp_fused(fa, D, s));
        MlpFusedArgs fr = fa;
        if (next.skip || next.frag) fr.ln_out = nullptr;
        DD_HIP(c, launch_mlp_reduce(fr, D, s));
        if (next.skip) DD_HIP(c, launch_skip_rows_ln(fa, D, s, !next.frag));
        if (next.qkv) DD_HIP(c, launch_qkv_rows(fa, D, s));
        return DD_OK;
    }

    int ee_finish() {
        if (!ee_dec_all) return DD_OK;
        FinalArgs fa = final_args(m, ch, ee_dec_all, m->heads[0].wconv, m->heads[0].bconv, nb * B);
        fa.eps_out = ee->outs;
        fa.layer_B = B; fa.w_stride = m->ee_wconv_stride; fa.b_stride = m->ee_bconv_stride;
        DD_HIP(c, launch_final(fa, s));
        if (m->ee_type != DD_EE_ATTENTION_PROBE) DD_HIP(c, launch_ee_probe_reduce(ee_srow_all, ee->cls, nb * B, L, s));
        return DD_OK;
    }

    int head() {
        const HeadW& hd = m->head;
        if (hd.wg) {
            HeadDecArgs ha{ws.x, hd.wg, hd.dc, ws.dec, M, m->pd, (L - m->extras) % 16 == 0 ? L : 0, m->extras};
            DD_HIP(c, launch_head_dec(ha, D, ch.cus, s));
            return DD_OK;
        }
        float* hf = (float*)ws.hid;
        DD_HIP(c, launch_layernorm<float>(ws.x, hd.ng, hd.nb, hf, M, D, s));
        GemmArgs<float> g{hf, nullptr, hd.wdec, hd.bdec, ws.dec, nullptr, M, m->pd, D, D, D, 0, m->pd};
        DD_HIP(c, launch_gemm<float>(g, EPI_BIAS_SET, s, ch.cus));
        return DD_OK;
    }
#undef DD_TIMED
};

struct Perturb { int first = 0; unsigned mask = 0; };

template <typename T>
int run_backbone(dd_model* m, const Chain& ch, const float* x_img, const float* t_vec, const int64_t* y_dev, int B, hipStream_t s,
                 const EeTaps* ee = nullptr, Perturb pert = {}) {
    Backbone<T> f{m, ch, B, s, ee, pert.first, pert.mask};
    Handoff hand;
    if (int rc = f.embed(x_img, t_vec, y_dev, hand)) return rc;
    for (int bi = 0; bi < f.nb; ++bi) {
        bool side = false;
        if (int rc = f.ee_taps(bi, hand, side)) return rc;
        if (int rc = f.skip_linear(bi, hand)) return rc;
        if (int rc = f.norm1_attention(bi, hand)) return rc;
        if (side) DD_HIP(m->ctx, hipStreamWaitEvent(s, m->ctx->ev_ee_join, 0));
        if (int rc = f.proj(bi)) return rc;
        if (int rc = f.mlp(bi, hand)) return rc;
    }
    if (int rc = f.ee_finish()) return rc;
    return f.head();
}

int run_model(dd_model* m, const Chain& ch, const float* x_img, const float* t_vec, const int64_t* y_dev, int B, hipStream_t s,
              const EeTaps* ee = nullptr, Perturb pert = {}) {
    return m->prec == DD_PREC_BF16 ? run_backbone<bf16_t>(m, ch, x_img, t_vec, y_dev, B, s, ee, pert)
                                   : run_backbone<float>(m, ch, x_img, t_vec, y_dev, B, s, ee, pert);
}

int check_model(dd_ctx* c, dd_model* m, int B) {
    if (!c || !m) return DD_ERR_INVALID;
    if (m->ctx != c) return ctx_fail(c, DD_ERR_INVALID, "model belongs to another context");
    if (!m->finalized) return ctx_fail(c, DD_ERR_STATE, "dd_model_finalize has not been called");
    if (B < 1 || B > m->cfg.max_batch) return ctx_fail(c, DD_ERR_INVALID, "batch size outside [1, max_batch]");
    return DD_OK;
}
int check_call(dd_ctx* c, dd_model* m, int B, const int64_t* y_dev) {
    if (int rc = check_model(c, m, B)) return rc;
    if (m->cfg.num_classes > 0 && !y_dev)
        return ctx_fail(c, DD_ERR_INVALID, "class-conditional model called without labels (pos_embed has L=extras+N rows)");
    if (m->cfg.num_classes <= 0 && y_dev)
// ... 1130 lines not shown
```

duodiff_amd/csrc/dd_internal.h:

```cpp
#pragma once
#include <hip/hip_runtime.h>
#include <stdint.h>

namespace dd {

typedef unsigned short bf16_t;

typedef __attribute__((ext_vector_type(8))) short bf16x8;
typedef __attribute__((ext_vector_type(4))) float f32x4;
typedef __attribute__((ext_vector_type(16))) float f32x16;
typedef unsigned u32x2 __attribute__((ext_vector_type(2)));
typedef unsigned u32x4 __attribute__((ext_vector_type(4)));

__device__ __forceinline__ bf16_t f2bf(float f) {
    __bf16 b = (__bf16)f;
    return __builtin_bit_cast(unsigned short, b);
}
__device__ __forceinline__ float bf2f(bf16_t b) {
    return __builtin_bit_cast(float, ((unsigned)b) << 16);
}

template <typename T> struct Elem;
template <> struct Elem<float> {
    static constexpr int kPerChunk = 4;
// ... 28 lines not shown
};

struct KnownRow {
    float ka, kb;
};

enum GemmEpilogue {
    EPI_STORE = 0,
    EPI_BIAS_GELU = 1,
    EPI_BIAS_RESID = 2,
    EPI_BIAS_SET = 3,
    EPI_BIAS_STORE = 4,
    EPI_PARTIAL = 5
};

struct HeadMajor {
    int L, Lp, H;
    unsigned magic;
};
inline HeadMajor make_head_major(int L, int H) {
    return HeadMajor{L, (L + 7) / 8 * 8, H, (unsigned)((1ull << 32) / (unsigned)L + 1ull)};
}
__device__ __forceinline__ long long hm_offset(const HeadMajor& hm, int row, int col) {
    const int b = (int)__umulhi((unsigned)row, hm.magic), l = row - b * hm.L;
    return (((long long)b * (3 * hm.H) + (col >> 6)) * hm.Lp + l) * 64 + (col & 63);
}

template <typename T>
struct GemmArgs {
    const T* A;
    const T* A2;
    const T* W;
    const float* bias;
    float* xres;
    T* out;
    int M, N, K, K1;
    int lda, lda2, ldo;
    HeadMajor hm;
    float* partial = nullptr;
    int splits = 0;
    int tile128 = -1;
};

template <typename T> hipError_t launch_gemm(const GemmArgs<T>& a, int epilogue, hipStream_t s, int num_cus);
bool plan_rows_256(int M, int N, int K, int num_cus, int* q, int* e);
bool gemm_prefers_128(int M, int N, int K, int K1, int num_cus);
bool gemm_splitk_supported(int M, int N, int K, int K1, int splits);
hipError_t launch_gemm_splitk(const GemmArgs<bf16_t>& a, hipStream_t s, int num_cus);
int device_num_cus();

struct MlpFusedArgs {
    const bf16_t* X;
    int ldx;
    const float* ln_in_g;
    const float* ln_in_b;
    const bf16_t* ao;
    const float* bproj;
    int nproj;
    const bf16_t* skip;
    const float* bskip;
    int nskip;
    bf16_t* qkv_out;
    bf16_t* ln_out_frag;
    bf16_t* qkv_dump;
    HeadMajor hm;
    int nqkv;
    const float* ln_out_g;
    const float* ln_out_b;
    bf16_t* ln_out;
    const char* wimg;
    const float* b1p;
    const float* b2;
    float* xres;
    bf16_t* out;
    int ldo;
    float* partial;
    int nchunks;
    int tok_n, tok_e, tok_l;
    int n_main, n_extra;
    int tiles_main, tiles_left, groups, cpg;
    int prows;
    float* y_tap = nullptr;
    int reduce_set = 0;
};
enum FragK { FRAG_K_NATURAL = 0, FRAG_K_ACC = 1 };
__host__ __device__ constexpr int frag_k_natural(int h, int j) { return 8 * h + j; }
__host__ __device__ constexpr int frag_k_acc(int h, int j) { return 8 * (j >> 2) + 4 * h + (j & 3); }
inline void pack_fragment(const float* w, size_t ld, int row0, int k0, FragK order, unsigned short (*to_bf16)(float), unsigned short* dst) {
    for (int lane = 0; lane < 64; ++lane)
        for (int j = 0; j < 8; ++j) {
            const int h = lane >> 5, k = order == FRAG_K_ACC ? frag_k_acc(h, j) : frag_k_natural(h, j);
            dst[lane * 8 + j] = to_bf16(w[(size_t)(row0 + (lane & 31)) * ld + k0 + k]);
        }
}

struct MlpImage {
    size_t blk;
    size_t mlp, skip, qkv;
    size_t end;
    __host__ __device__ constexpr MlpImage(int D, int nproj, int nchunks, int nskip, int nqkv)
        : blk((size_t)(D / 16) * 1024), mlp((size_t)nproj), skip(mlp + 2 * (size_t)nchunks), qkv(skip + (size_t)nskip), end(qkv + (size_t)nqkv) {}
    static MlpImage of(int D, int hidden, bool with_proj, bool with_skip, bool with_qkv) {
        return MlpImage(D, with_proj ? D / 32 : 0, hidden / 32, with_skip ? D / 16 : 0, with_qkv ? 3 * D / 32 : 0);
    }
    __host__ __device__ constexpr size_t at(size_t block) const { return block * blk; }
    constexpr size_t bytes() const { return at(end + 4); }
};
bool mlp_fused_supported(int D, int hidden);
void mlp_fused_pack_rows(int D, int nrows, const float* w, unsigned short (*to_bf16)(float), unsigned short* img);
hipError_t launch_qkv_rows(const MlpFusedArgs& a, int D, hipStream_t s);
void mlp_fused_pack_proj(int D, const float* wp, unsigned short (*to_bf16)(float), unsigned short* img);
void mlp_fused_pack_skip(int D, const float* ws, unsigned short (*to_bf16)(float), unsigned short* img);
hipError_t launch_skip_rows_ln(const MlpFusedArgs& a, int D, hipStream_t s, bool with_ln = true);
size_t mlp_fused_partial_bytes(int max_batch, int extras, int D, int hidden);
void mlp_fused_plan(int B, int n_patches, int extras, int seq_len, int hidden, MlpFusedArgs& a);
void mlp_fused_pack(int D, int hidden, const float* w1, const float* b1, const float* w2, bool kperm,
                    unsigned short (*to_bf16)(float), unsigned short* img, float* b1p);
hipError_t launch_mlp_fused(const MlpFusedArgs& a, int D, hipStream_t s);
hipError_t launch_mlp_reduce(const MlpFusedArgs& a, int D, hipStream_t s);
hipError_t init_mlp_fused_kernels();

struct RowLinArgs {
    const bf16_t* A;
    const bf16_t* A2;
    int k_split;
    int set_x;
    int lda, K;
    const char* wimg;
    const float* bias;
    float* xres;
    const float *ln_g, *ln_b;
    bf16_t* h_out;
    bf16_t* h_frag;
    bf16_t* x_copy;
    float* partial;
    int M;
    int tok_n, tok_e, tok_l, n_main, n_extra, tiles_main, tiles_extra, groups, cpg;
};
bool rowlin_supported(int D, int K);
void rowlin_pack(int K, const float* w, unsigned short (*to_bf16)(float), unsigned short* img);
void rowlin_plan(int B, int n_patches, int extras, int seq_len, int K, RowLinArgs& a);
size_t rowlin_partial_bytes(int max_batch, int extras, int K);
hipError_t launch_rowlin(const RowLinArgs& a, hipStream_t s);
hipError_t init_rowlin_kernels();

struct EmbedArgs {
    const float* x_img;
    const float* wt;
    const float* bias;
    const float* pos;
    const float* label_emb;
    const long long* y;
    const float* t_vec;
    StepState* st;
    float* x_tok;
    int B, C, S, P, D, L, extras, num_classes, normalize, Mp;
    int generic;
    const float* ln_g = nullptr;
    const float* ln_b = nullptr;
    bf16_t* ln_frag = nullptr;
};
bool embed_ln_supported(const EmbedArgs& a);

struct ReduceLnArgs {
    float* x;
    const float* partial;
    long long slab;
    int splits, resid;
    const float* bias;
    bf16_t* copy;
    int ldo;
    const float *ln_g, *ln_b;
    bf16_t* h;
    bf16_t* frag;
    int tok_l, tok_e;
    int rows;
};
hipError_t launch_reduce_ln(const ReduceLnArgs& a, int D, hipStream_t s);
hipError_t launch_embed(const EmbedArgs& a, hipStream_t s);

struct TimeMlpArgs {
    const float *w1t, *b1, *w2t, *b2, *pos, *t_vec;
    const StepState* st;
    float* x_tok;
    int B, D, L, extras, normalize;
};
hipError_t launch_time_mlp(const TimeMlpArgs& a, hipStream_t s);

template <typename T>
hipError_t launch_layernorm(const float* x, const float* gamma, const float* beta, T* out,
                            int rows, int D, hipStream_t s);
hipError_t launch_layernorm_frag(const float* x, const float* gamma, const float* beta, bf16_t* out, bf16_t* frag, int rows, int D,
                                 int tok_l, int tok_e, hipStream_t s);

template <typename T>
hipError_t launch_attention(const T* qkv, T* out, int B, int L, int H, int D, hipStream_t s);
bool qkv_attention_supported(int D, int H, int L, int extras);
void qkv_attention_pack(int D, int H, const float* w, unsigned short (*to_bf16)(float), unsigned short* img);
hipError_t launch_qkv_attention(const bf16_t* h, const bf16_t* wimg, const float* bias, const bf16_t* hx, const float* xres,
                                const float* ln_g, const float* ln_b, bf16_t* out, int B, int L, int H, int D, int extras, hipStream_t s);

hipError_t launch_v_identity(const bf16_t* h, const bf16_t* wimg, const float* bias, const float* xres, const float* ln_g, const float* ln_b,
                             bf16_t* out, int B, int L, int H, int D, int extras, hipStream_t s);
template <typename T>
hipError_t launch_v_copy(const T* qkv, T* out, int B, int L, int H, int D, hipStream_t s);

struct FinalArgs {
    const float* dec;
    const float* wconv;
    const float* bconv;
    const float* x_in;
    const float* z;
    float* eps_out;
    float* x_out;
    StepState* st;
    const StepCoef* coef;
    int B, C, S, P, L, extras, noise_mode, variance;
    int advance;
    const AffineRow* atab;
    int b0 = 0;
    int layer_B = 0;
    long long w_stride = 0, b_stride = 0;
    float guide_scale = 0.f;
    int pair_B = 0;
    const HistRow* htab = nullptr;
    float* h = nullptr;
    const float* dec2 = nullptr;
    const float* wconv2 = nullptr;
    const float* bconv2 = nullptr;
    int L2 = 0, extras2 = 0;
    const float* kx0 = nullptr;
    const float* kmask = nullptr;
    const KnownRow* ktab = nullptr;
};
hipError_t launch_final(const FinalArgs& a, hipStream_t s);

struct HeadDecArgs {
    const float* x;
    const float* wg;
    const float* c;
    float* dec;
    int M, pd;
    int tok_l, tok_e;
    float* srow = nullptr;
    const float* pw_base = nullptr;
    const float* pb_base = nullptr;
    const StepState* st = nullptr;
    int t_mul = 0, add = 0;
    int split = 0;
};
bool head_dec_probe_supported(int D);
void pack_head_split(int D, int pd, const float* wg, unsigned short (*f2bf)(float), unsigned short* img, float* wsum);
bool head_dec_supported(int D, int pd);
hipError_t launch_head_dec(const HeadDecArgs& a, int D, int num_cus, hipStream_t s);

hipError_t launch_ddpm_step(const float* x, const float* eps, const float* z, float* out,
                            StepCoef c, int use_noise, long long n, hipStream_t s);
template <typename T> hipError_t launch_fill_random(T* p, long long n, unsigned seed, float scale, hipStream_t s);
hipError_t launch_vae_input(const float* z, const float* w, const float* b, float inv_scale, float* out, int B, int HW, hipStream_t s);
hipError_t launch_vae_output(const float* in, float* out, int B, int C, int HW, int ldc, hipStream_t s);
template <typename T> hipError_t launch_im2col3x3(const T* src, T* dst, int B, int H, int W, int C, int up, int Kpad, hipStream_t s);
template <typename T> hipError_t launch_im2col3x3_s2(const T* src, T* dst, int B, int H, int W, int C, int Kpad, hipStream_t s);
hipError_t launch_vae_image(const float* x, float* out, int B, int HW, hipStream_t s);
hipError_t launch_vae_moments(const float* h, const float* w, const float* b, const float* eps, float* moments, float* z, int B, int HW,
                              hipStream_t s);
hipError_t launch_vae_sample(const float* moments, const float* eps, float* z, int B, int HW, hipStream_t s);
template <typename T> hipError_t launch_im2col3x3_c4(const float* src, T* dst, int B, int H, int W, int Kpad, hipStream_t s);
template <typename T> hipError_t launch_groupnorm(const float* x, float* part, const float* gamma, const float* beta, T* out, int B, int HW, int C, int swish, hipStream_t s);
int groupnorm_partials(int B, int HW);
template <typename T> hipError_t launch_softmax_rows(const float* sc, T* p, long long rows, int n, float scale, hipStream_t s);
template <typename T> hipError_t launch_cast(const float* x, T* out, long long n, hipStream_t s);

hipError_t launch_affine_step(const float* x, const float* m, const float* z, float* out, float a, float b, float c,
                              long long n, hipStream_t s);
hipError_t launch_multistep_step(const float* x, const float* m, const float* z, float* h, float* out, float a, float b, float c, float d,
                                 float p, float q, int use_hist, long long n, hipStream_t s);
hipError_t launch_known_blend(const float* x, const float* x0, const float* mask, const float* z2, float ka, float kb, float* out, int B, int C,
                              int S, hipStream_t s);
struct X0Threshold {
    int dynamic;
    int i;
    float f;
    float range, s_max;
// ... 38 lines not shown
```

duodiff_amd/csrc/dev_harness.hip:

```cpp
#include "../../include/duodiff.h"
#include "../../include/duodiff_dev.h"
#include "dd_internal.h"
#include "dev_scope.h"
#include "launch_args.h"

#include <cstring>
#include <vector>

using namespace dd;

extern "C" {

int dd_dev_mlp(dd_ctx* c, int M, int D, int hidden, int extras, const float* x_host, const float* w1, const float* b1, const float* w2,
               const float* b2, float* xres_host, unsigned short* out_host, const float* ln_in, const float* ln_out,
               unsigned short* ln_out_host, int iters, void* stream, float* ms_out, const float* ao_host, const float* wproj,
               const float* bproj, const float* skip_host, const float* wskip, const float* bskip, const float* wqkv,
               unsigned short* qkv_out_host) {
    const bool proj = ao_host && wproj && bproj;
    const bool skp = skip_host && wskip && bskip;
    const bool qk = wqkv && qkv_out_host;
    if (qk && (!proj || !ln_out || (hidden / 32) % 2)) return DD_ERR_INVALID;
    if (proj && (!ln_in || D % 128)) return DD_ERR_INVALID;
    if (skp && (!proj || !ln_out || !ln_out_host || (hidden / 32) % 2)) return DD_ERR_INVALID;
    if (!c || !x_host || !w1 || !b1 || !w2 || !b2 || !xres_host || M < 1 || iters < 0 || extras < 0 || (extras > 0 && M % (1 + extras))) return DD_ERR_INVALID;
    if (!mlp_fused_supported(D, hidden)) return ctx_fail(c, DD_ERR_UNSUPPORTED, "fused MLP: D in {64,128,256,512}, hidden % 64 == 0");
    hipStream_t s = (hipStream_t)stream;
    const size_t Mp = (size_t)round_up(M, 256), row_bytes = Mp * D * 2;
    const MlpImage im = MlpImage::of(D, hidden, proj, skp, qk);
    std::vector<unsigned short> img(im.bytes() / 2, 0);
    auto section = [&](size_t block) { return img.data() + im.at(block) / 2; };
    std::vector<float> b1p(hidden), xr(Mp * D, 0.f);
    std::memcpy(xr.data(), xres_host, (size_t)M * D * 4);
    if (proj) mlp_fused_pack_proj(D, wproj, host_f2bf, section(0));
    mlp_fused_pack(D, hidden, w1, b1, w2, ln_in != nullptr, host_f2bf, section(im.mlp), b1p.data());
    if (skp) mlp_fused_pack_skip(D, wskip, host_f2bf, section(im.skip));
    if (qk) mlp_fused_pack_rows(D, 3 * D, wqkv, host_f2bf, section(im.qkv));
    MlpFusedArgs a{};
    if (extras > 0) mlp_fused_plan(M / (1 + extras), 1, extras, 1 + extras, hidden, a);
    else mlp_fused_plan(1, M, 0, M, hidden, a);
    if (ctx_dev_flags(c) & DD_DEV_MLP_EXTRAS_ONLY) { a.tiles_main = 0; a.n_main = 0; }
    const size_t part = (size_t)a.tiles_left * a.groups * 128 * D * sizeof(float);
    DevScope dev(c);
    a.X = dev.upload(bf16_rows(x_host, M, D, Mp, 0).data(), row_bytes); a.ldx = D;
    a.wimg = (const char*)dev.upload(img.data(), img.size() * 2);
    a.b1p = dev.upload(b1p.data(), (size_t)hidden * 4); a.b2 = dev.upload(b2, (size_t)D * 4);
    a.xres = dev.upload(xr.data(), xr.size() * 4);
    bf16_t* dO = dev.filled<bf16_t>(row_bytes, 0);
    a.out = out_host ? dO : nullptr; a.ldo = D;
    a.partial = part ? dev.alloc<float>(part) : nullptr;
    bf16_t* dH = dev.filled<bf16_t>(row_bytes, 0);
    if (ln_in) { a.ln_in_g = dev.upload(ln_in, (size_t)2 * D * 4); a.ln_in_b = a.ln_in_g + D; }
    if (ln_out && ln_out_host) { a.ln_out_g = dev.upload(ln_out, (size_t)2 * D * 4); a.ln_out_b = a.ln_out_g + D; a.ln_out = dH; }
    if (proj) {
        a.ao = dev.upload(bf16_rows(ao_host, M, D, Mp, 0).data(), row_bytes); a.bproj = dev.upload(bproj, (size_t)D * 4); a.nproj = D / 32;
        a.reduce_set = 1;
    }
    MlpFusedArgs ar = a;
    if (skp) {
        a.skip = dev.upload(bf16_rows(skip_host, M, D, Mp, 0).data(), row_bytes); a.bskip = dev.upload(bskip, (size_t)D * 4); a.nskip = D / 16;
        a.out = dO;
        ar = a; ar.ln_out = nullptr;
    }
    size_t qkv_elems = 0;
    if (qk) {
        a.hm = make_head_major(a.tok_l, D / 64);
        const size_t images = (size_t)(M / a.tok_l);
        qkv_elems = images * 3 * D * (size_t)a.hm.Lp;
        a.qkv_out = dev.filled<bf16_t>(qkv_elems * 2, 0); a.qkv_dump = dev.alloc<bf16_t>(16384); a.nqkv = 3 * D / 32;
        ar.qkv_out = a.qkv_out; ar.qkv_dump = a.qkv_dump; ar.nqkv = a.nqkv; ar.hm = a.hm;
        if (!skp) ar = a;
    }
    auto once = [&]() -> hipError_t {
        hipError_t e = launch_mlp_fused(a, D, s);
        if (e == hipSuccess) e = launch_mlp_reduce(ar, D, s);
        if (e == hipSuccess) e = launch_skip_rows_ln(a, D, s);
        return e == hipSuccess ? launch_qkv_rows(a, D, s) : e;
    };
    DEV_HIP(dev, once());
    DEV_HIP(dev, hipStreamSynchronize(s));
    if (qk) dev.download(qkv_out_host, a.qkv_out, qkv_elems * 2);
    dev.download(xres_host, a.xres, (size_t)M * D * 4);
    if (out_host) dev.download(out_host, dO, (size_t)M * D * 2);
    if (a.ln_out) dev.download(ln_out_host, dH, (size_t)M * D * 2);
    DEV_HIP(dev, time_launches(s, iters, once, ms_out));
    return dev.status();
}

int dd_dev_block_tail(dd_ctx* c, int B, int n_patches, int extras, int D, int hidden, int last, int poison, const float* h_host,
                      const float* w1, const float* b1, const float* w2, const float* b2, const float* ln_in, const float* ao_host,
                      const float* wproj, const float* bproj, const float* ln_out, const float* skip_host, const float* wskip,
                      const float* bskip, const float* wqkv, float* xres_host, unsigned short* out_host, unsigned short* ln_out_host,
                      unsigned short* frag_host, float* tap_host, unsigned short* qkv_host, float* slab_host, int slab_rows, int* plan_out,
                      int iters, void* stream, float* ms_out) {
    const bool proj = ao_host && wproj && bproj;
    const bool skp = skip_host && wskip && bskip;
    const bool qk = wqkv && qkv_host;
    const bool lnout = ln_out && ln_out_host;
    const bool frag = frag_host != nullptr, tap = tap_host != nullptr;
    if (!c || B < 1 || n_patches < 1 || extras < 0 || extras > 2 || D < 1 || hidden < 1 || !w1 || !b1 || !w2 || !b2 || !xres_host || iters < 0 ||
        poison < 0 || poison > 255 || slab_rows < 0 || (slab_rows > 0) != (slab_host != nullptr) || (ln_in != nullptr) == (h_host != nullptr))
        return DD_ERR_INVALID;
    if ((proj && !ln_in) || (lnout && !ln_in) || (frag && !lnout) || (skp && (!proj || !lnout || !out_host)) || (tap && !skp) ||
        (qk && (!proj || !lnout)) || (last && (!proj || lnout || skp || qk)))
        return DD_ERR_INVALID;
    if (!mlp_fused_supported(D, hidden)) return ctx_fail(c, DD_ERR_UNSUPPORTED, "fused MLP: D in {64,128,256,512}, hidden % 64 == 0");
    if (frag && skp && extras > 0 && D != 512) return ctx_fail(c, DD_ERR_UNSUPPORTED, "block tail: skip rows without their LayerNorm at D = 512 only");
    hipStream_t s = (hipStream_t)stream;
    const int L = extras + n_patches, M = B * L;
    const size_t Mo = (size_t)round_up(M, 256) + 8, n16 = Mo * D * 2, n32 = Mo * D * 4;
    const MlpImage im = MlpImage::of(D, hidden, proj, skp, qk);
    std::vector<unsigned short> img(im.bytes() / 2, 0);
    auto section = [&](size_t block) { return img.data() + im.at(block) / 2; };
    std::vector<float> b1p(hidden);
    if (proj) mlp_fused_pack_proj(D, wproj, host_f2bf, section(0));
    mlp_fused_pack(D, hidden, w1, b1, w2, ln_in != nullptr, host_f2bf, section(im.mlp), b1p.data());
    if (skp) mlp_fused_pack_skip(D, wskip, host_f2bf, section(im.skip));
    if (qk) mlp_fused_pack_rows(D, 3 * D, wqkv, host_f2bf, section(im.qkv));
    MlpFusedArgs a{};
    mlp_fused_plan(B, n_patches, extras, L, hidden, a);
    if (last) { a.n_extra = 0; a.tiles_left = 0; }
    if ((size_t)slab_rows < (size_t)a.tiles_left * a.groups * a.prows) return DD_ERR_INVALID;
    if (plan_out) { plan_out[0] = a.tiles_main; plan_out[1] = a.tiles_left; plan_out[2] = a.groups; plan_out[3] = a.prows; }
    DevScope dev(c);
    a.X = h_host ? dev.upload(bf16_rows(h_host, M, D, Mo, (unsigned char)poison).data(), n16) : nullptr; a.ldx = D;
    a.wimg = (const char*)dev.upload(img.data(), img.size() * 2);
    a.b1p = dev.upload(b1p.data(), (size_t)hidden * 4); a.b2 = dev.upload(b2, (size_t)D * 4);
    if (ln_in) { a.ln_in_g = dev.upload(ln_in, (size_t)2 * D * 4); a.ln_in_b = a.ln_in_g + D; }
    a.xres = dev.upload(xres_host, n32);
    a.out = out_host ? dev.filled<bf16_t>(n16, 0xFF) : nullptr; a.ldo = D;
    a.partial = slab_rows ? dev.filled<float>((size_t)slab_rows * D * 4, poison) : nullptr;
    if (proj) {
        a.ao = dev.upload(bf16_rows(ao_host, M, D, Mo, (unsigned char)poison).data(), n16); a.bproj = dev.upload(bproj, (size_t)D * 4); a.nproj = D / 32;
        a.reduce_set = 1;
    }
    if (skp) {
        a.skip = dev.upload(bf16_rows(skip_host, M, D, Mo, (unsigned char)poison).data(), n16);
        if (tap) a.y_tap = dev.filled<float>(n32, 0xFF);
        a.bskip = dev.upload(bskip, (size_t)D * 4); a.nskip = D / 16;
    }
    if (lnout) { a.ln_out_g = dev.upload(ln_out, (size_t)2 * D * 4); a.ln_out_b = a.ln_out_g + D; a.ln_out = dev.filled<bf16_t>(n16, 0xFF); }
    if (frag) a.ln_out_frag = dev.filled<bf16_t>(n16, 0xFF);
    const size_t qkv_elems = qk ? ((size_t)B * 3 * (D / 64) * make_head_major(L, D / 64).Lp + 64) * 64 : 0;
    if (qk) { a.qkv_out = dev.filled<bf16_t>(qkv_elems * 2, 0xFF); a.qkv_dump = dev.alloc<bf16_t>(16384); a.hm = make_head_major(L, D / 64); a.nqkv = 3 * D / 32; }
    MlpFusedArgs fr = a;
    if (skp || frag) fr.ln_out = nullptr;
    auto rest = [&]() -> hipError_t {
        hipError_t e = launch_mlp_reduce(fr, D, s);
        if (e == hipSuccess && skp) e = launch_skip_rows_ln(a, D, s, !frag);
        if (e == hipSuccess && qk) e = launch_qkv_rows(a, D, s);
        return e;
    };
    auto once = [&]() -> hipError_t {
        const hipError_t e = launch_mlp_fused(a, D, s);
        return e == hipSuccess ? rest() : e;
    };
    const hipError_t first = dev.ok() ? launch_mlp_fused(a, D, s) : hipSuccess;
    if (first == hipErrorInvalidValue) return ctx_fail(c, DD_ERR_UNSUPPORTED, "block tail: a combination of modes launch_mlp_fused refuses");
    DEV_HIP(dev, first);
    DEV_HIP(dev, rest());
    DEV_HIP(dev, hipStreamSynchronize(s));
    dev.download(xres_host, a.xres, n32);
    if (out_host) dev.download(out_host, a.out, n16);
    if (lnout) dev.download(ln_out_host, a.ln_out, n16);
    if (frag) dev.download(frag_host, a.ln_out_frag, n16);
    if (tap) dev.download(tap_host, a.y_tap, n32);
    if (qk) dev.download(qkv_host, a.qkv_out, qkv_elems * 2);
    if (slab_rows) dev.download(slab_host, a.partial, (size_t)slab_rows * D * 4);
    DEV_HIP(dev, time_launches(s, iters, once, ms_out));
    return dev.status();
}

int dd_dev_qkv_attention_rows(dd_ctx* c, int B, int L, int H, int extras, const float* h_host, const float* wqkv, const float* bqkv,
                              const float* xres_host, const float* ln, unsigned short* out_host, int iters, void* stream, float* ms_out) {
    if (!c || !h_host || !wqkv || !out_host || (xres_host && !ln) || B < 1 || iters < 0) return DD_ERR_INVALID;
    const int D = 64 * H;
    if (!qkv_attention_supported(D, H, L, extras)) return ctx_fail(c, DD_ERR_UNSUPPORTED, "qkv_attention: D = 512 / 768 / 1024, L = 256 + 1 or 2 extra tokens only");
    hipStream_t s = (hipStream_t)stream;
    const size_t M = (size_t)B * L;
    std::vector<unsigned short> hb = bf16_rows(h_host, M, D, M, 0);
    std::vector<unsigned short> hf((size_t)B * 256 * D), img((size_t)3 * D * D);
    for (int b = 0; b < B; ++b)
        for (int n = 0; n < 256; ++n)
            for (int k = 0; k < D; ++k)
                hf[((((size_t)b * 8 + n / 32) * (D / 16) + k / 16) * 64 + (n % 32) + 32 * ((k % 16) / 8)) * 8 + k % 8] = hb[((size_t)b * L + extras + n) * D + k];
    qkv_attention_pack(D, H, wqkv, host_f2bf, img.data());
    std::vector<float> xr;
    if (xres_host) {
        xr.resize(M * D);
        std::memset(xr.data(), 0xFF, xr.size() * 4);
        for (int b = 0; b < B; ++b) std::memcpy(xr.data() + (size_t)b * L * D, xres_host + (size_t)b * L * D, (size_t)extras * D * 4);
    } else {
        for (int b = 0; b < B; ++b) std::memset(hb.data() + ((size_t)b * L + extras) * D, 0xFF, (size_t)256 * D * 2);
    }
    DevScope dev(c);
    const bf16_t* dH = dev.upload(hf.data(), hf.size() * 2);
    const bf16_t* dW = dev.upload(img.data(), img.size() * 2);
    const bf16_t* dQ = xres_host ? nullptr : dev.upload(hb.data(), hb.size() * 2);
    const float* dX = xres_host ? dev.upload(xr.data(), xr.size() * 4) : nullptr;
    const float* dL = xres_host ? dev.upload(ln, (size_t)2 * D * 4) : nullptr;
    bf16_t* dO = dev.filled<bf16_t>((M + 8) * D * 2, 0xFF);
    const float* dB = bqkv ? dev.upload(bqkv, (size_t)3 * D * 4) : nullptr;
    auto once = [&]() { return launch_qkv_attention(dH, dW, dB, dQ, dX, dL, dL ? dL + D : nullptr, dO, B, L, H, D, extras, s); };
    DEV_HIP(dev, once());
    DEV_HIP(dev, hipStreamSynchronize(s));
    dev.download(out_host, dO, (M + 8) * D * 2);
    DEV_HIP(dev, time_launches(s, iters, once, ms_out));
    return dev.status();
}

int dd_dev_v_identity(dd_ctx* c, int B, int L, int H, int extras, const float* h_host, const float* wqkv, const float* bqkv,
                      const float* xres_host, const float* ln, unsigned short* out_host, int iters, void* stream, float* ms_out) {
    if (!c || !h_host || !wqkv || !out_host || !xres_host || !ln || B < 1 || iters < 0) return DD_ERR_INVALID;
    const int D = 64 * H;
    if (!qkv_attention_supported(D, H, L, extras)) return ctx_fail(c, DD_ERR_UNSUPPORTED, "v_identity: D = 512 / 768 / 1024, L = 256 + 1 or 2 extra tokens only");
    hipStream_t s = (hipStream_t)stream;
    const size_t M = (size_t)B * L;
    std::vector<unsigned short> hb = bf16_rows(h_host, M, D, M, 0);
    std::vector<unsigned short> hf((size_t)B * 256 * D), img((size_t)3 * D * D);
    for (int b = 0; b < B; ++b)
        for (int n = 0; n < 256; ++n)
            for (int k = 0; k < D; ++k)
                hf[((((size_t)b * 8 + n / 32) * (D / 16) + k / 16) * 64 + (n % 32) + 32 * ((k % 16) / 8)) * 8 + k % 8] = hb[((size_t)b * L + extras + n) * D + k];
    qkv_attention_pack(D, H, wqkv, host_f2bf, img.data());
    std::vector<float> xr(M * D);
    std::memset(xr.data(), 0xFF, xr.size() * 4);
    for (int b = 0; b < B; ++b) std::memcpy(xr.data() + (size_t)b * L * D, xres_host + (size_t)b * L * D, (size_t)extras * D * 4);
    DevScope dev(c);
    const bf16_t* dH = dev.upload(hf.data(), hf.size() * 2);
    const bf16_t* dW = dev.upload(img.data(), img.size() * 2);
    const float* dX = dev.upload(xr.data(), xr.size() * 4);
    const float* dL = dev.upload(ln, (size_t)2 * D * 4);
    bf16_t* dO = dev.filled<bf16_t>((M + 8) * D * 2, 0xFF);
    const float* dB = bqkv ? dev.upload(bqkv, (size_t)3 * D * 4) : nullptr;
    auto once = [&]() { return launch_v_identity(dH, dW, dB, dX, dL, dL ? dL + D : nullptr, dO, B, L, H, D, extras, s); };
    DEV_HIP(dev, once());
    DEV_HIP(dev, hipStreamSynchronize(s));
    dev.download(out_host, dO, (M + 8) * D * 2);
    DEV_HIP(dev, time_launches(s, iters, once, ms_out));
    return dev.status();
}

int dd_dev_v_copy(dd_ctx* c, int precision, int B, int L, int H, const float* qkv_host, void* out_host, int iters, void* stream, float* ms_out) {
    const bool bf = precision == DD_PREC_BF16;
    if (!c || (!bf && precision != DD_PREC_FP32) || B < 1 || L < 1 || H < 1 || !qkv_host || !out_host || iters < 0) return DD_ERR_INVALID;
    hipStream_t s = (hipStream_t)stream;
    const int D = 64 * H;
    const size_t esz = bf ? 2 : 4, Lp = (size_t)make_head_major(L, H).Lp;
    const size_t qkv_elems = ((size_t)B * 3 * H * Lp + 64) * 64, out_elems = ((size_t)B * L + 8) * D;
    std::vector<unsigned char> img(qkv_elems * esz, 0xFF);
    for (size_t u = 0; u < (size_t)B * 3 * H; ++u)
        for (int l = 0; l < L; ++l) {
            const float* row = qkv_host + (u * L + l) * 64;
            const size_t at = (u * Lp + l) * 64;
            if (bf) for (int d = 0; d < 64; ++d) reinterpret_cast<unsigned short*>(img.data())[at + d] = host_f2bf(row[d]);
            else std::memcpy(img.data() + at * 4, row, 64 * 4);
        }
    DevScope dev(c);
    const void* dQ = dev.upload(img.data(), img.size());
    void* dO = dev.filled(out_elems * esz, 0xFF);
    auto once = [&]() {
        return bf ? launch_v_copy<bf16_t>((const bf16_t*)dQ, (bf16_t*)dO, B, L, H, D, s) : launch_v_copy<float>((const float*)dQ, (float*)dO, B, L, H, D, s);
    };
    const hipError_t first = dev.ok() ? once() : hipSuccess;
    if (first == hipErrorInvalidValue) return ctx_fail(c, DD_ERR_UNSUPPORTED, "v_copy: 1 <= L <= 288, heads of 64");
    DEV_HIP(dev, first);
    DEV_HIP(dev, hipStreamSynchronize(s));
    dev.download(out_host, dO, out_elems * esz);
    DEV_HIP(dev, time_launches(s, iters, once, ms_out));
    return dev.status();
}

int dd_dev_qkv_attention(dd_ctx* c, int B, int L, int H, int extras, const float* h_host, const float* wqkv, const float* bqkv,
                         unsigned short* out_host, int iters, void* stream, float* ms_out) {
    if (!out_host) return DD_ERR_INVALID;
    std::vector<unsigned short> whole(B > 0 && L > 0 && H > 0 ? ((size_t)B * L + 8) * 64 * H : 0);
    const int st = dd_dev_qkv_attention_rows(c, B, L, H, extras, h_host, wqkv, bqkv, nullptr, nullptr, whole.data(), iters, stream, ms_out);
    if (st == DD_OK) std::memcpy(out_host, whole.data(), (size_t)B * L * 64 * H * 2);
    return st;
}

int dd_dev_head_dec(dd_ctx* c, int M, int D, int pd, int tok_l, int tok_e, const float* x_host, const float* norm_g, const float* norm_b,
                    const float* wdec, const float* bdec, float* dec_host, const float* probe_w, const float* probe_b, float* srow_host,
                    int split, int iters, void* stream, float* ms_out) {
    if (!c || !x_host || !norm_g || !norm_b || !wdec || !bdec || !dec_host || M < 1 || iters < 0) return DD_ERR_INVALID;
    if (!head_dec_supported(D, pd)) return ctx_fail(c, DD_ERR_UNSUPPORTED, "head_dec: D in {256, 512, 768, 1024}, pd % 4 == 0, pd <= 64");
    const bool probe = probe_w && probe_b && srow_host;
    if (probe && !head_dec_probe_supported(D)) return ctx_fail(c, DD_ERR_UNSUPPORTED, "head_dec with the probe: D in {256, 512}");
    hipStream_t s = (hipStream_t)stream;
    if (split && !head_dec_probe_supported(D)) return ctx_fail(c, DD_ERR_UNSUPPORTED, "head_dec as a split-bf16 product: D in {256, 512}");
    std::vector<float> wg, dc;
// ... 300 lines not shown
```

duodiff_amd/csrc/mlp_fused.hip:

```cpp
#include "dd_internal.h"
#include "wave_prims.h"

#include <type_traits>
#include <utility>

namespace dd {
namespace {

constexpr int kMaxHidden = 4096;
constexpr int kProjRowsLds = 4 * 32 * (1024 + 32);
constexpr int kGroups = 16;

__device__ __forceinline__ const char* uniform_ptr(const char* p) {
    asm volatile("" : "+s"(p));
    return p;
}
__device__ __forceinline__ void glds16u(const char* ubase, unsigned voff, void* lds_dst) {
    __builtin_amdgcn_global_load_lds((gptr_t)(ubase + voff), (lptr_t)lds_dst, 16, 0, 0);
}
template <int J>
__device__ __forceinline__ void glds16u_j(const char* ublock, unsigned voff, char* lds_block) {
    constexpr int HI = (J >> 2) * 4096, IMM = (J & 3) * 1024;
    __builtin_amdgcn_global_load_lds((gptr_t)(ublock + HI + voff), (lptr_t)(lds_block + HI), 16, IMM, 0);
}
// ... 21 lines not shown
    if constexpr (LG >= 0) {                                                      \
        if constexpr (READ) DD_GAP_ASM(DD_S_MFMA_W DD_S_READ GSTR, ACC_C);        \
        else DD_GAP_ASM(DD_S_MFMA_W GSTR, ACC_C);                                 \
    } else {                                                                      \
        if constexpr (READ) DD_GAP_ASM(DD_S_MFMA_N DD_S_READ GSTR, ACC_C);        \
        else DD_GAP_ASM(DD_S_MFMA_N GSTR, ACC_C);                                 \
    }
#define DD_GAP_K(KK, GSTR, ACC_C) else if constexpr (K == KK) { DD_GAP_SEL(GSTR, ACC_C) }
template <int KIND, int LG, bool READ, int LO, int K>
__device__ __forceinline__ void gap_stmt(f32x16& acc, bf16x8& wa, const bf16x8& xb, unsigned la, float va, float vb,
                                         const GeluConst& k, GeluPair& r, unsigned& out) {
    if constexpr (KIND == 0) {
        if constexpr (K < 0) { DD_GAP_SEL("", "+v") }
        DD_GAP_K(0, DD_S_G0, "+v") DD_GAP_K(1, DD_S_G1, "+v") DD_GAP_K(2, DD_S_G2, "+v") DD_GAP_K(3, DD_S_G3, "+v")
        DD_GAP_K(4, DD_S_G4, "+v") DD_GAP_K(5, DD_S_G5, "+v") DD_GAP_K(6, DD_S_G6, "+v") DD_GAP_K(7, DD_S_G7, "+v")
    } else {
        if constexpr (K < 0) { DD_GAP_SEL("", "+a") }
        DD_GAP_K(0, DD_S_G0, "+a") DD_GAP_K(1, DD_S_G1, "+a") DD_GAP_K(2, DD_S_G2, "+a") DD_GAP_K(3, DD_S_G3, "+a")
        DD_GAP_K(4, DD_S_G4, "+a") DD_GAP_K(5, DD_S_G5, "+a") DD_GAP_K(6, DD_S_G6, "+a") DD_GAP_K(7, DD_S_G7, "+a")
    }
}

template <int K>
__device__ __forceinline__ void gelu_piece(float va, float vb, const GeluConst& k, GeluPair& r, unsigned& out) {
    if constexpr (K == 0) asm volatile(DD_S_G0 : [sa] "+v"(r.sa), [sb] "+v"(r.sb), [s2a] "+v"(r.s2a) : [va] "v"(va), [vb] "v"(vb), [kn] "s"(-3.8f), [kh] "v"(k.hi));
    else if constexpr (K == 1) asm volatile(DD_S_G1 : [s2b] "+v"(r.s2b), [pa] "+v"(r.pa), [pb] "+v"(r.pb) : [sb] "v"(r.sb), [s2a] "v"(r.s2a), [kc] "v"(k.c5));
    else if constexpr (K == 2) asm volatile(DD_S_G2 : [pa] "+v"(r.pa), [pb] "+v"(r.pb) : [s2a] "v"(r.s2a), [s2b] "v"(r.s2b));
    else if constexpr (K == 3) asm volatile(DD_S_G3 : [pa] "+v"(r.pa), [pb] "+v"(r.pb) : [s2a] "v"(r.s2a), [s2b] "v"(r.s2b));
    else if constexpr (K == 4) asm volatile(DD_S_G4 : [pa] "+v"(r.pa), [pb] "+v"(r.pb) : [s2a] "v"(r.s2a), [s2b] "v"(r.s2b));
    else if constexpr (K == 5) asm volatile(DD_S_G5 : [pb] "+v"(r.pb), [ha] "+v"(r.ha), [hb] "+v"(r.hb) : [s2b] "v"(r.s2b), [sa] "v"(r.sa), [sb] "v"(r.sb), [pa] "v"(r.pa));
    else if constexpr (K == 6) asm volatile(DD_S_G6 : [ha] "+v"(r.ha), [hb] "+v"(r.hb) : [va] "v"(va), [vb] "v"(vb));
    else asm volatile(DD_S_G7 : [out] "+v"(out) : [ha] "v"(r.ha), [hb] "v"(r.hb));
}

template <int OFF>
__device__ __forceinline__ void load_quad_agpr(f32x4& q, const float* p) {
    asm volatile("global_load_dwordx4 %0, %1, off offset:%2" : "=a"(q) : "v"(p), "i"(OFF));
}

__device__ __forceinline__ void acc_pin(f32x16& y) { asm volatile("" : "+a"(y)); }

template <int NT>
__device__ __forceinline__ void pin_tiles(f32x16 (&y)[NT]) {
    static_assert(NT == 2 || NT == 4 || NT == 8 || NT == 16, "D in {64, 128, 256, 512}");
    if constexpr (NT == 2) asm volatile("" : "+a"(y[0]), "+a"(y[1]));
    else if constexpr (NT == 4) asm volatile("" : "+a"(y[0]), "+a"(y[1]), "+a"(y[2]), "+a"(y[3]));
    else if constexpr (NT == 8)
        asm volatile("" : "+a"(y[0]), "+a"(y[1]), "+a"(y[2]), "+a"(y[3]), "+a"(y[4]), "+a"(y[5]), "+a"(y[6]), "+a"(y[7]));
    else
        asm volatile("" : "+a"(y[0]), "+a"(y[1]), "+a"(y[2]), "+a"(y[3]), "+a"(y[4]), "+a"(y[5]), "+a"(y[6]), "+a"(y[7]), "+a"(y[8]),
                     "+a"(y[9]), "+a"(y[10]), "+a"(y[11]), "+a"(y[12]), "+a"(y[13]), "+a"(y[14]), "+a"(y[15]));
}

template <int D>
__device__ __forceinline__ void ln_stats_shifted(float c, float s, float q, float& mean, float& rstd) {
    constexpr float n = (float)(D / 2);
    const float mh = c + s / n;
    const float m2h = q - s * s / n;
    const auto pm = __builtin_amdgcn_permlane32_swap(__builtin_bit_cast(unsigned, mh), __builtin_bit_cast(unsigned, mh), false, false);
    const auto p2 = __builtin_amdgcn_permlane32_swap(__builtin_bit_cast(unsigned, m2h), __builtin_bit_cast(unsigned, m2h), false, false);
    const unsigned u_lo = pm[0], u_hi = pm[1], w_lo = p2[0], w_hi = p2[1];
    const float m_lo = __builtin_bit_cast(float, u_lo), m_hi = __builtin_bit_cast(float, u_hi);
    const float q_lo = __builtin_bit_cast(float, w_lo), q_hi = __builtin_bit_cast(float, w_hi);
    mean = 0.5f * (m_lo + m_hi);
    const float d = m_lo - m_hi;
    const float m2 = (q_lo + q_hi) + d * d * (0.5f * n);
    const float var = m2 / (float)D;
    rstd = 1.0f / sqrtf((var > 0.f ? var : 0.f) + 1e-5f);
}

template <int D>
struct MlpCfg {
    static constexpr int NT = D / 32;
    static constexpr int KS = D / 16;
    static constexpr int F = D / 16;
    static constexpr int BLK = F * 1024;
    static constexpr int RING = 4 * BLK;
    static constexpr int FPW = F / 4;
};

template <int D, bool LNIN, bool PARTIAL, bool PROJ, bool SKIP = false, bool QKV = false, bool TAP = false>
__device__ __forceinline__ void mlp_body(const MlpFusedArgs& a, char* smem, const int tile_idx, const int c0, int c1, const int slab) {
    using C = MlpCfg<D>;
    static_assert(!PROJ || (LNIN && C::NT % 4 == 0), "proj fusion: the LayerNorm-in kernel, D % 128 == 0");
    static_assert(!SKIP || (PROJ && !PARTIAL), "skip fusion rides on the proj-fused main tiles");
    static_assert(!QKV || (PROJ && !PARTIAL), "qkv fusion rides on the proj-fused main tiles");
    float* b1s = reinterpret_cast<float*>(smem + C::RING);
    float* vecs = b1s + (a.nchunks + 1) * 32;
    const char* const wproj = a.wimg;
    const char* const wmlp = a.wimg + (size_t)a.nproj * C::BLK;

    const int tid = threadIdx.x;
    const int lane = tid & 63;
    const int wave = __builtin_amdgcn_readfirstlane(tid >> 6);
    const int h = lane >> 5, r32 = lane & 31;

    auto row_of = [&](bool& ok) -> long long {
        unsigned l = (unsigned)threadIdx.x;
        asm volatile("" : "+v"(l));
        const int local = (int)l / 64 * 32 + ((int)l & 31);
        const int idx = tile_idx * (PARTIAL ? a.prows : 128) + local;
        if constexpr (!PARTIAL) {
            ok = idx < a.n_main;
            const int p = ok ? idx : 0, b = p / a.tok_n;
            return (long long)b * a.tok_l + a.tok_e + (p - b * a.tok_n);
        } else {
            ok = local < a.prows && idx < a.n_extra;
            const int q = ok ? idx : 0, b = q / a.tok_e;
            return (long long)b * a.tok_l + (q - b * a.tok_e);
        }
    };
    auto half_of = [&]() -> int {
        unsigned l = (unsigned)threadIdx.x;
        asm volatile("" : "+v"(l));
        return (int)(l >> 5) & 1;
    };

    const unsigned dma_voff = (wave * C::FPW) * 1024 + lane * 16;
    auto dma_block = [&](int b, int slot) {
        const char* src = uniform_ptr((PROJ ? wproj : wmlp) + (size_t)b * C::BLK);
        char* dst = smem + slot * C::BLK + (wave * C::FPW) * 1024;
        [&]<int... J>(std::integer_sequence<int, J...>) { (glds16u_j<J>(src, dma_voff, dst), ...); }(std::make_integer_sequence<int, C::FPW>{});
    };

    const int pb0 = PROJ ? 0 : 2 * c0;
    dma_block(pb0, 0);
    dma_block(pb0 + 1, 1);
    dma_block(pb0 + 2, 2);
    if constexpr (!PROJ) {
        f32x4* z = reinterpret_cast<f32x4*>(smem + 3 * C::BLK);
        for (int i = tid; i < C::BLK / 16; i += 256) z[i] = f32x4{0.f, 0.f, 0.f, 0.f};
    }

    {
        constexpr int TB = kMaxHidden / 4 / 256, VQ = 7 * (D / 4), VI = (VQ + 255) / 256;
        const int nb1 = a.nchunks * 8;
        f32x4 tb[TB], tv[VI];
        bool tvok[VI];
#pragma unroll
        for (int k = 0; k < TB; ++k) {
            const int i = tid + 256 * k;
            tb[k] = reinterpret_cast<const f32x4*>(a.b1p)[i < nb1 ? i : 0];
        }
#pragma unroll
        for (int k = 0; k < VI; ++k) {
            const int item = tid + 256 * k, v = item / (D / 4), i = item - v * (D / 4);
            const float* sp = v == 0 ? a.ln_in_g : v == 1 ? a.ln_in_b : v == 2 ? a.ln_out_g : v == 3 ? a.ln_out_b : v == 4 ? a.b2 : v == 5 ? a.bproj : a.bskip;
            tvok[k] = item < VQ && sp != nullptr;
            tv[k] = f32x4{0.f, 0.f, 0.f, 0.f};
            if (tvok[k]) tv[k] = reinterpret_cast<const f32x4*>(sp)[i];
        }
        __builtin_amdgcn_sched_barrier(0);
#pragma unroll
        for (int k = 0; k < TB; ++k)
            if (tid + 256 * k < nb1) reinterpret_cast<f32x4*>(b1s)[tid + 256 * k] = tb[k];
#pragma unroll
        for (int k = 0; k < VI; ++k)
            if (tvok[k]) reinterpret_cast<f32x4*>(vecs)[tid + 256 * k] = tv[k];
    }
    const float* lg_in = vecs + 4 * h;
    const float* lb_in = vecs + D + 4 * h;
    bool row_ok_pro;
    const long long row_pro = row_of(row_ok_pro);

    bf16x8 xf[C::KS];
    f32x16 Y[C::NT];
    if constexpr (!LNIN) {
        const bf16_t* xr = a.X + row_pro * a.ldx + 8 * h;
#pragma unroll
        for (int ks = 0; ks < C::KS; ++ks) xf[ks] = *reinterpret_cast<const bf16x8*>(xr + 16 * ks);
#pragma unroll
        for (int t = 0; t < C::NT; ++t)
#pragma unroll
            for (int e = 0; e < 16; ++e) Y[t][e] = 0.f;
        __syncthreads();
    } else {
        const float* xr = a.xres + row_pro * D + 4 * h;
        f32x4 s4 = {0.f, 0.f, 0.f, 0.f}, q4 = {0.f, 0.f, 0.f, 0.f};
        float cshift = 0.f;
        constexpr int LA = C::NT < 4 ? C::NT : (PARTIAL && !PROJ && C::NT >= 8) ? 8 : 4;
        f32x4 xq[LA][4];
        const float* lbp = vecs + 5 * D + 4 * h;
        if constexpr (PROJ) {
            const bf16_t* ar = a.ao + row_pro * D + 8 * h;
#pragma unroll
            for (int ks = 0; ks < C::KS; ++ks) xf[ks] = *reinterpret_cast<const bf16x8*>(ar + 16 * ks);
            __syncthreads();
        }
#pragma unroll
        for (int t = 0; t < LA - 1; ++t)
#pragma unroll
            for (int g = 0; g < 4; ++g) xq[t][g] = *reinterpret_cast<const f32x4*>(xr + 32 * t + 8 * g);
#pragma unroll
        for (int t = 0; t < C::NT; ++t) {
            if (t + LA - 1 < C::NT) {
#pragma unroll
                for (int g = 0; g < 4; ++g) xq[(t + LA - 1) % LA][g] = *reinterpret_cast<const f32x4*>(xr + 32 * (t + LA - 1) + 8 * g);
            }
            __builtin_amdgcn_sched_barrier(0);
#pragma unroll
            for (int g = 0; g < 4; ++g) {
                f32x4 q = xq[t % LA][g];
                if constexpr (PROJ) q += *reinterpret_cast<const f32x4*>(lbp + 32 * t + 8 * g);
                if constexpr (!PROJ) {
                    if (t == 0 && g == 0) cshift = q[0];
                    const f32x4 dq = q - cshift;
                    s4 += dq;
                    q4 += dq * dq;
                }
#pragma unroll
                for (int e = 0; e < 4; ++e) Y[t][4 * g + e] = q[e];
            }
            acc_pin(Y[t]);
            __builtin_amdgcn_sched_barrier(0);
        }
        if constexpr (PROJ) {
            const unsigned lds_lo_p = lds_offset(smem) + lane * 16;
            const unsigned lds_hi_p = lds_lo_p + 65536u;
            constexpr int PDp = C::F / 2 < 8 ? C::F / 2 : 8;
            constexpr int NGp = C::NT * C::F;
            bf16x8 wp[PDp];
            GeluPair gr0{0.f, 0.f, 0.f, 0.f, 0.f, 0.f, 0.f, 0.f};
            const GeluConst gk0{0.f, 0.f};
            unsigned none = 0;
            [&]<int... J>(std::integer_sequence<int, J...>) {
                (ds_read16<J * 1024>(wp[J], lds_lo_p), ...);
            }(std::make_integer_sequence<int, PDp>{});
            [&]<int... GI>(std::integer_sequence<int, GI...>) {
                ([&] {
                    constexpr int g = GI, t = g / C::F, f = g % C::F;
                    if constexpr (f == C::F / 2) {
                        waitcnt_vm<C::FPW>();
                        __builtin_amdgcn_s_barrier();
                        const char* src = uniform_ptr(a.wimg + (size_t)(t + 3) * C::BLK + (t + 3 >= C::NT ? (size_t)(2 * c0) * C::BLK : (size_t)0));
                        char* dst = smem + ((t + 3) & 3) * C::BLK + (wave * C::FPW) * 1024;
                        [&]<int... J>(std::integer_sequence<int, J...>) { (glds16u_j<J>(src, dma_voff, dst), ...); }(std::make_integer_sequence<int, C::FPW>{});
                    }
                    constexpr int gn = g + PDp, left = NGp - 1 - g;
                    constexpr int lg_self = left < PDp - 1 ? left : PDp - 1, lg_next = left - 1 < PDp - 1 ? left - 1 : PDp - 1;
                    constexpr int LG = (g & 1) ? -1 : (left >= 1 ? lg_next - (left >= PDp ? 1 : 0) : lg_self);
                    constexpr bool RD = gn < NGp;
                    constexpr int LO = RD ? ((gn / C::F) & 3) * C::BLK + (gn % C::F) * 1024 : 0;
                    constexpr int LOA = LO < 65536 ? LO : LO - 65536;
                    gap_stmt<1, LG, RD, LOA, -1>(Y[t], wp[g % PDp], xf[f], LO < 65536 ? lds_lo_p : lds_hi_p, 0.f, 0.f, gk0, gr0, none);
                }(), ...);
            }(std::make_integer_sequence<int, NGp>{});
            mfma_drain();
            s4 = f32x4{0.f, 0.f, 0.f, 0.f};
            q4 = f32x4{0.f, 0.f, 0.f, 0.f};
#pragma unroll
            for (int t = 0; t < C::NT; ++t) {
                acc_pin(Y[t]);
                const f32x16 yt = Y[t];
                if (t == 0) cshift = yt[0];
#pragma unroll
                for (int g = 0; g < 4; ++g) {
                    const f32x4 q = {yt[4 * g], yt[4 * g + 1], yt[4 * g + 2], yt[4 * g + 3]};
                    const f32x4 dq = q - cshift;
                    s4 += dq;
                    q4 += dq * dq;
                }
                __builtin_amdgcn_sched_barrier(0);
            }
        }
        float mean, rstd;
        ln_stats_shifted<D>(cshift, (s4[0] + s4[1]) + (s4[2] + s4[3]), (q4[0] + q4[1]) + (q4[2] + q4[3]), mean, rstd);
        const float shift = -mean * rstd;
        __syncthreads();
#pragma unroll
        for (int t = 0; t < C::NT; ++t) {
            acc_pin(Y[t]);
            const f32x16 yt = Y[t];
#pragma unroll
            for (int kq = 0; kq < 2; ++kq) {
                const int ks = 2 * t + kq;
                unsigned u[4];
#pragma unroll
                for (int gq = 0; gq < 2; ++gq) {
                    const int col = 16 * ks + 8 * gq, g = 2 * kq + gq;
                    const f32x4 q = {yt[4 * g], yt[4 * g + 1], yt[4 * g + 2], yt[4 * g + 3]};
// ... 41 lines not shown
    GeluPair gr{0.f, 0.f, 0.f, 0.f, 0.f, 0.f, 0.f, 0.f};
    unsigned pw_none = 0;
    f32x16 sA, sB;
    bf16x8 wq[PD];
    bias_init(c0, sA);
    [&]<int... J>(std::integer_sequence<int, J...>) { (frag(std::integral_constant<int, frag_off(0, J)>{}, wq[J]), ...); }
    (std::make_integer_sequence<int, PD>{});
    [&]<int... FI>(std::integer_sequence<int, FI...>) {
        ([&] {
            constexpr int f = FI, left = C::F - 1 - f, LG = left < PD - 1 ? left : PD - 1;
            constexpr bool RD = f + PD < C::F;
            constexpr int LO = RD ? frag_off(0, f + PD) : 0;
            gap_stmt<0, LG, RD, LO, -1>(sA, wq[f % PD], xf[f], lds_lo, 0.f, 0.f, gk, gr, pw_none);
        }(), ...);
    }(std::make_integer_sequence<int, C::F>{});
    [&]<int... J>(std::integer_sequence<int, J...>) { (frag(std::integral_constant<int, frag_off(3, J)>{}, wq[J]), ...); }
    (std::make_integer_sequence<int, PD>{});

    constexpr int PPG = 32 / C::F;
    constexpr int KB = C::F / 2;
    constexpr int DSTEP = C::F / C::FPW;
    auto iteration = [&](auto par_tag, int c, f32x16& s_cur, f32x16& s_next, const bf16x8 (&p_prev)[2], bf16x8 (&p_out)[2]) {
        constexpr int PAR = decltype(par_tag)::value;
        constexpr int SLOT_A = PAR ? 1 : 3;
        constexpr int SLOT_B = PAR ? 0 : 2;
        constexpr int SLOT_N = PAR ? 3 : 1;
        constexpr int NG = 2 * C::F;
        unsigned pw[8];
        const char* src_e = uniform_ptr(wmlp + (size_t)(2 * c + 4) * C::BLK);
        const char* src_m = uniform_ptr(wmlp + (size_t)(2 * c + 3) * C::BLK);
        char* dst_e = smem + (PAR ? 2 : 0) * C::BLK + (wave * C::FPW) * 1024;
        char* dst_m = smem + (PAR ? 1 : 3) * C::BLK + (wave * C::FPW) * 1024;
        [&]<int... GI>(std::integer_sequence<int, GI...>) {
            ([&] {
                constexpr int g = GI;
                if constexpr (g == 0 || g == C::F) {
                    waitcnt_vm<C::FPW>();
                    __builtin_amdgcn_s_barrier();
                }
                constexpr int gn = g + PD;
                constexpr int LO = gn < C::F ? frag_off(SLOT_A, gn) : gn < NG ? frag_off(SLOT_B, gn - C::F) : frag_off(SLOT_N, gn - NG);
                constexpr int LOA = LO < 65536 ? LO : LO - 65536;
                const unsigned la = LO < 65536 ? lds_lo : lds_hi;
                constexpr int lg_next = PD - 1 + ((g + 1 > KB && g + 1 <= KB + PD) ? 4 : 0);
                constexpr int LG = (g & 1) ? -1 : lg_next - 1 - (g == KB ? 4 : 0);
                static_assert(KB % 2 == 0 || C::F < 4, "pair waits assume an even bias gap");
                constexpr int id0 = g * PPG;
                constexpr int K = PPG == 1 ? (id0 & 7) : -1;
                constexpr int pair = (g * PPG) >> 3;
                if constexpr (g < C::F)
                    gap_stmt<1, LG, true, LOA, K>(Y[g >> 1], wq[g % PD], p_prev[g & 1], la, s_cur[2 * pair], s_cur[2 * pair + 1], gk, gr, pw[pair]);
                else
                    gap_stmt<0, LG, true, LOA, K>(s_next, wq[g % PD], xf[g - C::F], la, s_cur[2 * pair], s_cur[2 * pair + 1], gk, gr, pw[pair]);
                if constexpr (PPG > 1) {
                    [&]<int... Q>(std::integer_sequence<int, Q...>) {
                        ([&] {
                            constexpr int id = g * PPG + Q, pr = id >> 3;
                            gelu_piece<(id & 7)>(s_cur[2 * pr], s_cur[2 * pr + 1], gk, gr, pw[pr]);
                        }(), ...);
                    }(std::make_integer_sequence<int, PPG>{});
                }
                if constexpr (g == KB) bias_init(c + 1, s_next);
                if constexpr (g % DSTEP == DSTEP / 2) {
                    constexpr int j = (g % C::F) / DSTEP;
                    if constexpr (g < C::F) glds16u_j<j>(src_e, dma_voff, dst_e);
                    else glds16u_j<j>(src_m, dma_voff, dst_m);
                }
            }(), ...);
        }(std::make_integer_sequence<int, NG>{});
        p_out[0] = __builtin_bit_cast(bf16x8, u32x4{pw[0], pw[1], pw[2], pw[3]});
        p_out[1] = __builtin_bit_cast(bf16x8, u32x4{pw[4], pw[5], pw[6], pw[7]});
    };

    bf16x8 pA[2], pB[2];
    pA[0] = pA[1] = bf16x8{0, 0, 0, 0, 0, 0, 0, 0};
    for (int c = c0; c < c1; c += 2) {
        iteration(std::integral_constant<int, 0>{}, c, sA, sB, pA, pB);
        iteration(std::integral_constant<int, 1>{}, c + 1, sB, sA, pB, pA);
    }
    bf16x8 sk[C::F / 2];
    const bf16_t* sr = nullptr;
    if constexpr (SKIP) {
        bool ok_s;
        sr = a.skip + row_of(ok_s) * D + 8 * half_of();
#pragma unroll
        for (int ks = 0; ks < C::F / 2; ++ks) sk[ks] = *reinterpret_cast<const bf16x8*>(sr + 16 * ks);
    }
    [&]<int... FI>(std::integer_sequence<int, FI...>) {
        ([&] {
            constexpr int f = FI, left = C::F - 1 - f, LG = left < PD - 1 ? left : PD - 1;
            constexpr bool RD = f + PD < C::F;
            constexpr int LO = RD ? frag_off(3, f + PD) : 0;
            constexpr int LOA = LO < 65536 ? LO : LO - 65536;
            gap_stmt<1, LG, RD, LOA, -1>(Y[f >> 1], wq[f % PD], pA[f & 1], LO < 65536 ? lds_lo : lds_hi, 0.f, 0.f, gk, gr, pw_none);
        }(), ...);
    }(std::make_integer_sequence<int, C::F>{});
    waitcnt_vm<0>();
    mfma_drain();
#pragma unroll
    for (int t = 0; t < C::NT; ++t) asm volatile("" : "+a"(Y[t]));

    if constexpr (SKIP) {
        __builtin_amdgcn_s_barrier();
        {
            const int hs = half_of();
            const float* lb2s = vecs + 4 * D + 4 * hs;
            const float* lbsk = vecs + 6 * D + 4 * hs;
            bool tap_ok = false;
            float* tap = nullptr;
            if constexpr (TAP) { tap = a.y_tap + row_of(tap_ok) * D + 4 * hs; }
#pragma unroll
            for (int t = 0; t < C::NT; ++t) {
                acc_pin(Y[t]);
                const f32x16 yt = Y[t];
#pragma unroll
                for (int kq = 0; kq < 2; ++kq) {
                    const int ks = 2 * t + kq;
                    unsigned u[4];
#pragma unroll
                    for (int gq = 0; gq < 2; ++gq) {
                        const int col = 16 * ks + 8 * gq, g = 2 * kq + gq;
                        f32x4 q = {yt[4 * g], yt[4 * g + 1], yt[4 * g + 2], yt[4 * g + 3]};
                        q += *reinterpret_cast<const f32x4*>(lb2s + col);
                        if constexpr (TAP) { if (tap_ok) *reinterpret_cast<f32x4*>(tap + col) = q; }
                        u[2 * gq] = cvt_pk_bf16(q[0], q[1]);
                        u[2 * gq + 1] = cvt_pk_bf16(q[2], q[3]);
                    }
                    xf[ks] = __builtin_bit_cast(bf16x8, u32x4{u[0], u[1], u[2], u[3]});
                }
#pragma unroll
                for (int g = 0; g < 4; ++g) {
                    const f32x4 bq = *reinterpret_cast<const f32x4*>(lbsk + 32 * t + 8 * g);
#pragma unroll
                    for (int e = 0; e < 4; ++e) Y[t][4 * g + e] = bq[e];
                }
                acc_pin(Y[t]);
                __builtin_amdgcn_sched_barrier(0);
            }
        }
        const char* const wskip = wmlp + (size_t)(2 * a.nchunks) * C::BLK;
        const unsigned lds_lo_s = lds_offset(smem) + lane * 16;
        const unsigned lds_hi_s = lds_lo_s + 65536u;
        constexpr int PDs = C::F / 2 < 8 ? C::F / 2 : 8;
        constexpr int NPs = 2 * C::NT, NGs = NPs * C::F, H2 = C::F / 2;
        bf16x8 ws[PDs];
        [&]<int... J>(std::integer_sequence<int, J...>) {
            (ds_read16<J * 1024>(ws[J], lds_lo_s), ...);
        }(std::make_integer_sequence<int, PDs>{});
        [&]<int... GI>(std::integer_sequence<int, GI...>) {
            ([&] {
                constexpr int g = GI, p = g / C::F, f = g % C::F;
                if constexpr (f == C::F / 2) {
                    constexpr int extra = (p == C::NT + 1 || p == C::NT + 2) ? H2 : 0;
                    waitcnt_vm<C::FPW + extra>();
                    __builtin_amdgcn_s_barrier();
                    const char* src = uniform_ptr(wskip + (size_t)(p + 3) * C::BLK);
                    char* dst = smem + ((p + 3) & 3) * C::BLK + (wave * C::FPW) * 1024;
                    [&]<int... J>(std::integer_sequence<int, J...>) { (glds16u_j<J>(src, dma_voff, dst), ...); }(std::make_integer_sequence<int, C::FPW>{});
                    if constexpr (p == C::NT) {
                        asm volatile("" ::: "memory");
                        __builtin_amdgcn_sched_barrier(0);
#pragma unroll
                        for (int ks = 0; ks < H2; ++ks) xf[ks] = *reinterpret_cast<const bf16x8*>(sr + 16 * (H2 + ks));
                        __builtin_amdgcn_sched_barrier(0);
                        asm volatile("" ::: "memory");
                    }
                }
                constexpr int gn = g + PDs, left = NGs - 1 - g;
                constexpr int lg_self = left < PDs - 1 ? left : PDs - 1, lg_next = left - 1 < PDs - 1 ? left - 1 : PDs - 1;
                constexpr int LG = (g & 1) ? -1 : (left >= 1 ? lg_next - (left >= PDs ? 1 : 0) : lg_self);
                constexpr bool RD = gn < NGs;
                constexpr int LO = RD ? ((gn / C::F) & 3) * C::BLK + (gn % C::F) * 1024 : 0;
                constexpr int LOA = LO < 65536 ? LO : LO - 65536;
                constexpr int tile = p < C::NT ? p : 2 * ((p - C::NT) % (C::NT / 2)) + (f >= H2 ? 1 : 0);
                if constexpr (p < C::NT)
                    mfma_gap<true, LG, RD, LOA>(Y[tile], ws[g % PDs], xf[f], LO < 65536 ? lds_lo_s : lds_hi_s);
                else if constexpr (p < C::NT + C::NT / 2)
                    mfma_gap<true, LG, RD, LOA>(Y[tile], ws[g % PDs], sk[f % H2], LO < 65536 ? lds_lo_s : lds_hi_s);
                else
                    mfma_gap<true, LG, RD, LOA>(Y[tile], ws[g % PDs], xf[f % H2], LO < 65536 ? lds_lo_s : lds_hi_s);
            }(), ...);
        }(std::make_integer_sequence<int, NGs>{});
        waitcnt_vm<0>();
        mfma_drain();
#pragma unroll
        for (int t = 0; t < C::NT; ++t) asm volatile("" : "+a"(Y[t]));
    }

    const int he = half_of();
    if constexpr (PARTIAL) {
        if (wave * 32 >= a.prows) return;
        float* pp = a.partial + ((long long)slab * a.prows + wave * 32 + r32) * D + 4 * he;
#pragma unroll
        for (int t = 0; t < C::NT; ++t) {
            const f32x16 yt = Y[t];
#pragma unroll
            for (int g = 0; g < 4; ++g)
                *reinterpret_cast<f32x4*>(pp + 32 * t + 8 * g) = f32x4{yt[4 * g], yt[4 * g + 1], yt[4 * g + 2], yt[4 * g + 3]};
        }
    } else {
        bool row_ok;
        const long long row = row_of(row_ok);
        if constexpr (!QKV) {
            if (!row_ok) return;
        }
        const float* lg_out = vecs + 2 * D + 4 * he;
        const float* lb_out = vecs + 3 * D + 4 * he;
        const float* lb2 = vecs + 4 * D + 4 * he;
        float* xrow = (!QKV || row_ok) ? a.xres + row * D + 4 * he : reinterpret_cast<float*>(reinterpret_cast<char*>(a.qkv_dump) + 8192) + 4 * he;
        bf16_t* orow = (!QKV || row_ok) ? a.out + row * a.ldo + 8 * he : reinterpret_cast<bf16_t*>(reinterpret_cast<char*>(a.qkv_dump) + 12288) + 8 * he;
        f32x4 xl[2][4];
        if constexpr (!LNIN) {
#pragma unroll
            for (int g = 0; g < 4; ++g) xl[0][g] = *reinterpret_cast<const f32x4*>(xrow + 8 * g);
        }
        f32x4 s4 = {0.f, 0.f, 0.f, 0.f}, q4 = {0.f, 0.f, 0.f, 0.f};
        float cshift = 0.f;
#pragma unroll
        for (int t = 0; t < C::NT; ++t) {
            if constexpr (!LNIN) {
                if (t + 1 < C::NT) {
#pragma unroll
                    for (int g = 0; g < 4; ++g) xl[(t + 1) & 1][g] = *reinterpret_cast<const f32x4*>(xrow + 32 * (t + 1) + 8 * g);
                }
            }
            uint2 v[4];
            const f32x16 yt = Y[t];
#pragma unroll
            for (int g = 0; g < 4; ++g) {
                f32x4 q = {yt[4 * g], yt[4 * g + 1], yt[4 * g + 2], yt[4 * g + 3]};
                if constexpr (!SKIP) q += *reinterpret_cast<const f32x4*>(lb2 + 32 * t + 8 * g);
                if constexpr (!LNIN) q = xl[t & 1][g] + q;
                *reinterpret_cast<f32x4*>(xrow + 32 * t + 8 * g) = q;
                v[g] = uint2{cvt_pk_bf16(q[0], q[1]), cvt_pk_bf16(q[2], q[3])};
                if (t == 0 && g == 0) cshift = q[0];
                const f32x4 dq = q - cshift;
                s4 += dq;
                q4 += dq * dq;
            }
            if (!SKIP && a.out) {
#pragma unroll
                for (int gp = 0; gp < 4; gp += 2) {
                    const auto s0 = __builtin_amdgcn_permlane32_swap(v[gp].x, v[gp + 1].x, false, false);
                    const auto s1 = __builtin_amdgcn_permlane32_swap(v[gp].y, v[gp + 1].y, false, false);
                    const uint4 o = {s0[0], s1[0], s0[1], s1[1]};
                    *reinterpret_cast<uint4*>(orow + 32 * t + 8 * gp) = o;
                }
            }
            acc_pin(Y[t]);
            asm volatile("" : "+v"(s4), "+v"(q4));
            __builtin_amdgcn_sched_barrier(0);
        }
        if (QKV || (LNIN && a.ln_out)) {
            float mean, rstd;
            ln_stats_shifted<D>(cshift, (s4[0] + s4[1]) + (s4[2] + s4[3]), (q4[0] + q4[1]) + (q4[2] + q4[3]), mean, rstd);
            const float shift = -mean * rstd;
            const float* lb2r = lb2;
            asm volatile("" : "+v"(lb2r));
            bf16_t* lnp = nullptr;
            long long lnstride = 16;
            if constexpr (!QKV && !PARTIAL) {
                unsigned l = (unsigned)threadIdx.x;
                asm volatile("" : "+v"(l));
                if (a.ln_out_frag) { lnp = a.ln_out_frag + (((long long)tile_idx * 4 + (l >> 6)) * C::F * 64 + (l & 63)) * 8; lnstride = 512; }
                else lnp = a.ln_out + row * D + 8 * he;
            }
#pragma unroll
            for (int t = 0; t < C::NT; ++t) {
                uint2 v[4];
                const f32x16 yt = Y[t];
#pragma unroll
                for (int g = 0; g < 4; ++g) {
                    f32x4 q = {yt[4 * g], yt[4 * g + 1], yt[4 * g + 2], yt[4 * g + 3]};
                    if constexpr (!SKIP) q += *reinterpret_cast<const f32x4*>(lb2r + 32 * t + 8 * g);
                    const f32x4 gv = *reinterpret_cast<const f32x4*>(lg_out + 32 * t + 8 * g), bv = *reinterpret_cast<const f32x4*>(lb_out + 32 * t + 8 * g);
                    const f32x4 w = (q * rstd + shift) * gv + bv;
                    v[g] = uint2{cvt_pk_bf16(w[0], w[1]), cvt_pk_bf16(w[2], w[3])};
                }
                if constexpr (QKV) {
                    xf[2 * t] = __builtin_bit_cast(bf16x8, u32x4{v[0].x, v[0].y, v[1].x, v[1].y});
                    xf[2 * t + 1] = __builtin_bit_cast(bf16x8, u32x4{v[2].x, v[2].y, v[3].x, v[3].y});
                    asm volatile("" : "+v"(xf[2 * t]), "+v"(xf[2 * t + 1]));
                    acc_pin(Y[t]);
                } else {
#pragma unroll
                    for (int gp2 = 0; gp2 < 4; gp2 += 2) {
                        const auto s0 = __builtin_amdgcn_permlane32_swap(v[gp2].x, v[gp2 + 1].x, false, false);
                        const auto s1 = __builtin_amdgcn_permlane32_swap(v[gp2].y, v[gp2 + 1].y, false, false);
                        const uint4 o = {s0[0], s1[0], s0[1], s1[1]};
                        *reinterpret_cast<uint4*>(lnp + (2 * t + gp2 / 2) * lnstride) = o;
                    }
                }
                __builtin_amdgcn_sched_barrier(0);
            }
        }

        if constexpr (QKV) {
            const char* const wqkv = wmlp + ((size_t)2 * a.nchunks + (SKIP ? 2 * C::NT : 0)) * C::BLK;
            const unsigned lds_lo_q = lds_offset(smem) + lane * 16;
            const unsigned lds_hi_q = lds_lo_q + 65536u;
            constexpr int PDq = C::F / 2 < 8 ? C::F / 2 : 8;
            constexpr int NQ = 3 * C::NT, NGq = NQ * C::F;
            const int pidx = (int)(row / a.tok_l), lidx = (int)(row - (long long)pidx * a.tok_l);
            char* qrow = row_ok ? reinterpret_cast<char*>(a.qkv_out) + (((long long)pidx * (3 * a.hm.H)) * a.hm.Lp + lidx) * 128 + 16 * he
                                : reinterpret_cast<char*>(a.qkv_dump) + (tid * 2) * 16;
            const long long ustride = row_ok ? (long long)a.hm.Lp * 128 : 0;
            const int tstride = row_ok ? 64 : 0, gstride = row_ok ? 32 : 16;
            __builtin_amdgcn_s_barrier();
            bf16x8 wq2[PDq];
            [&]<int... J>(std::integer_sequence<int, J...>) {
                (ds_read16<J * 1024>(wq2[J], lds_lo_q), ...);
            }(std::make_integer_sequence<int, PDq>{});
            f32x16 qa, qb;
#pragma unroll
            for (int e = 0; e < 16; ++e) { qa[e] = 0.f; qb[e] = 0.f; }
            asm volatile("" : "+a"(qa), "+a"(qb));
            auto flush_tile = [&](int tt, f32x16& acc) {
                uint2 v[4];
#pragma unroll
                for (int g = 0; g < 4; ++g) v[g] = uint2{cvt_pk_bf16(acc[4 * g], acc[4 * g + 1]), cvt_pk_bf16(acc[4 * g + 2], acc[4 * g + 3])};
                char* dst = qrow + (long long)(tt >> 1) * ustride + (tt & 1) * tstride;
#pragma unroll
                for (int gp = 0; gp < 4; gp += 2) {
                    const auto s0 = __builtin_amdgcn_permlane32_swap(v[gp].x, v[gp + 1].x, false, false);
                    const auto s1 = __builtin_amdgcn_permlane32_swap(v[gp].y, v[gp + 1].y, false, false);
                    const unsigned o0 = s0[0], o1 = s1[0], o2 = s0[1], o3 = s1[1];
                    *reinterpret_cast<uint4*>(dst + (gp >> 1) * gstride) = uint4{o0, o1, o2, o3};
                }
#pragma unroll
// ... 209 lines not shown
    float s1 = 0.f;
#pragma unroll
    for (int e = 0; e < 16; ++e) s1 += acc[e];
    s1 += __shfl_xor(s1, 32);
    if (h == 0) red[wave * 32 + r32] = s1;
    __syncthreads();
    float tot = 0.f;
#pragma unroll
    for (int w = 0; w < NW; ++w) tot += red[w * 32 + r32];
    const float mean = tot / (float)D;
    float s2 = 0.f;
#pragma unroll
    for (int e = 0; e < 16; ++e) { const float d = acc[e] - mean; s2 += d * d; }
    s2 += __shfl_xor(s2, 32);
    if (h == 0) red[(NW + wave) * 32 + r32] = s2;
    __syncthreads();
    float tq = 0.f;
#pragma unroll
    for (int w = 0; w < NW; ++w) tq += red[(NW + w) * 32 + r32];
    const float rstd = 1.0f / sqrtf(tq / (float)D + 1e-5f);
    const int idx = blockIdx.x * 32 + r32;
    if (idx >= a.n_extra) return;
    const long long row = row_of(idx);
#pragma unroll
    for (int g = 0; g < 4; ++g) {
        const int col = 32 * t + 8 * g + 4 * h;
        const f32x4 v = {acc[4 * g], acc[4 * g + 1], acc[4 * g + 2], acc[4 * g + 3]};
        *reinterpret_cast<f32x4*>(a.xres + row * D + col) = v;
        const f32x4 gv = *reinterpret_cast<const f32x4*>(a.ln_out_g + col), bv = *reinterpret_cast<const f32x4*>(a.ln_out_b + col);
        const f32x4 w = (v - mean) * rstd * gv + bv;
        *reinterpret_cast<uint2*>(a.ln_out + row * D + col) = uint2{cvt_pk_bf16(w[0], w[1]), cvt_pk_bf16(w[2], w[3])};
    }
}

template <int D>
__global__ void __launch_bounds__(256) qkv_rows_kernel(const MlpFusedArgs a) {
    using C = MlpCfg<D>;
    constexpr int LPR = D / 8, RPI = 64 / LPR, NI = 32 / RPI, IPITCH = 1024 + 32;
    extern __shared__ __attribute__((aligned(16))) char strip_lds[];
    const int lane = threadIdx.x & 63, wave = threadIdx.x >> 6, h = lane >> 5;
    const int t = blockIdx.x, idx0 = blockIdx.y * 128 + wave * 32;
    char* strip = strip_lds + wave * (NI * IPITCH);
    auto row_of = [&](int idx) { return extra_token_row(idx, a.n_extra, a.tok_e, a.tok_l); };
#pragma unroll
    for (int i = 0; i < NI; ++i)
        lds_dma16(a.ln_out + row_of(idx0 + i * RPI + lane / LPR) * D + (lane % LPR) * 8, strip + i * IPITCH);
    __builtin_amdgcn_sched_barrier(0);
    const int idx = idx0 + (lane & 31);
    const bool ok = idx < a.n_extra;
    const long long row = row_of(idx);
    const MlpImage im(D, a.nproj, a.nchunks, a.nskip, a.nqkv);
    const bf16x8* wb = reinterpret_cast<const bf16x8*>(a.wimg + im.at(im.qkv + t)) + lane;
    bf16x8 wf[C::F];
#pragma unroll
    for (int ks = 0; ks < C::F; ++ks) wf[ks] = wb[ks * 64];
    waitcnt_vm<0>();
    const char* my = strip + ((lane & 31) / RPI) * IPITCH + ((lane & 31) % RPI) * (D * 2) + 8 * h;
    f32x16 acc, acc1;
#pragma unroll
    for (int e = 0; e < 16; ++e) { acc[e] = 0.f; acc1[e] = 0.f; }
#pragma unroll
    for (int ks = 0; ks < C::F; ks += 2) {
        const u32x2 l0 = *reinterpret_cast<const u32x2*>(my + 32 * ks), h0 = *reinterpret_cast<const u32x2*>(my + 32 * ks + 16);
        const u32x2 l1 = *reinterpret_cast<const u32x2*>(my + 32 * ks + 32), h1 = *reinterpret_cast<const u32x2*>(my + 32 * ks + 48);
        acc = __builtin_amdgcn_mfma_f32_32x32x16_bf16(wf[ks], __builtin_bit_cast(bf16x8, u32x4{l0[0], l0[1], h0[0], h0[1]}), acc, 0, 0, 0);
        acc1 = __builtin_amdgcn_mfma_f32_32x32x16_bf16(wf[ks + 1], __builtin_bit_cast(bf16x8, u32x4{l1[0], l1[1], h1[0], h1[1]}), acc1, 0, 0, 0);
    }
    acc += acc1;
    if (!ok) return;
    bf16_t* dst = a.qkv_out + hm_offset(a.hm, (int)row, 32 * t) + 4 * h;
#pragma unroll
    for (int g = 0; g < 4; ++g)
        *reinterpret_cast<uint2*>(dst + 8 * g) = uint2{cvt_pk_bf16(acc[4 * g], acc[4 * g + 1]), cvt_pk_bf16(acc[4 * g + 2], acc[4 * g + 3])};
}

template <int D>
hipError_t launch_d(const MlpFusedArgs& a, hipStream_t s) {
    const size_t lds = MlpCfg<D>::RING + (size_t)(a.nchunks + 1) * 32 * sizeof(float) + 7 * D * sizeof(float);
    const int grid = a.tiles_main + a.tiles_left * a.groups;
    if (a.nskip > 0 && (a.nproj <= 0 || a.nskip != D / 16 || !a.skip || !a.bskip || (!a.ln_out && a.nqkv <= 0) || a.nchunks % 2)) return hipErrorInvalidValue;
    if (a.nqkv > 0 && a.nproj <= 0) return hipErrorInvalidValue;
    if (a.y_tap && (a.nskip <= 0 || a.nqkv > 0)) return hipErrorInvalidValue;
    if (a.ln_out_frag && (!a.ln_out || a.nqkv > 0 || a.tok_n % 32)) return hipErrorInvalidValue;
    if (a.nproj > 0) {
        if constexpr (D % 128 == 0) {
            if (!a.ln_in_g || !a.ao || !a.bproj || a.nproj != D / 32) return hipErrorInvalidValue;
            if (a.nqkv > 0) {
                if (a.nqkv != 3 * D / 32 || !a.qkv_out || !a.qkv_dump || !a.ln_out_g || !a.ln_out_b || a.hm.L != a.tok_l || a.nchunks % 2) return hipErrorInvalidValue;
                if (a.nskip > 0) hipLaunchKernelGGL((mlp_fused_kernel<D, true, true, true, true>), dim3(grid), dim3(256), lds, s, a);
                else hipLaunchKernelGGL((mlp_fused_kernel<D, true, true, false, true>), dim3(grid), dim3(256), lds, s, a);
            } else if (a.nskip > 0 && a.y_tap) hipLaunchKernelGGL((mlp_fused_kernel<D, true, true, true, false, true>), dim3(grid), dim3(256), lds, s, a);
            else if (a.nskip > 0) hipLaunchKernelGGL((mlp_fused_kernel<D, true, true, true>), dim3(grid), dim3(256), lds, s, a);
            else hipLaunchKernelGGL((mlp_fused_kernel<D, true, true>), dim3(grid), dim3(256), lds, s, a);
        } else {
            return hipErrorInvalidValue;
        }
    } else if (a.ln_in_g) {
        hipLaunchKernelGGL((mlp_fused_kernel<D, true, false>), dim3(grid), dim3(256), lds, s, a);
    } else {
        hipLaunchKernelGGL((mlp_fused_kernel<D, false, false>), dim3(grid), dim3(256), lds, s, a);
    }
    return hipGetLastError();
}

template <int D>
hipError_t launch_reduce_d(const MlpFusedArgs& a, hipStream_t s) {
    if (a.tiles_left <= 0) return hipSuccess;
    hipLaunchKernelGGL(mlp_reduce_kernel<D / 64>, dim3((unsigned)((a.n_extra + 3) / 4)), dim3(256), 0, s, a);
    return hipGetLastError();
}


}

static size_t skip_rows_lds(int D) { return (size_t)64 * (D * 2 + 16) + (size_t)2 * (D / 32) * 32 * sizeof(float); }

bool mlp_fused_supported(int D, int hidden) {
    return (D == 64 || D == 128 || D == 256 || D == 512) && hidden % 64 == 0 && hidden >= 64 && hidden <= kMaxHidden;
}

void mlp_fused_pack_rows(int D, int nrows, const float* w, unsigned short (*to_bf16)(float), unsigned short* img) {
    const int F = D / 16;
    for (int t = 0; t < nrows / 32; ++t)
        for (int f = 0; f < F; ++f) pack_fragment(w, D, 32 * t, 16 * f, FRAG_K_ACC, to_bf16, img + ((size_t)t * F + f) * 512);
}

void mlp_fused_pack_skip(int D, const float* ws, unsigned short (*to_bf16)(float), unsigned short* img) {
    const int F = D / 16, NT = D / 32, H2 = F / 2;
    for (int p = 0; p < 2 * NT; ++p)
        for (int f = 0; f < F; ++f) {
            unsigned short* dst = img + ((size_t)p * F + f) * 512;
            if (p < NT) {
                pack_fragment(ws, 2 * D, 32 * p, 16 * f, FRAG_K_ACC, to_bf16, dst);
            } else {
                const int q = p - NT, pass = q / (NT / 2), jj = q % (NT / 2);
                pack_fragment(ws, 2 * D, 32 * (2 * jj + (f >= H2 ? 1 : 0)), D + 16 * (pass * H2 + f % H2), FRAG_K_NATURAL, to_bf16, dst);
            }
        }
}

void mlp_fused_pack_proj(int D, const float* wp, unsigned short (*to_bf16)(float), unsigned short* img) {
    const int F = D / 16;
    for (int t = 0; t < D / 32; ++t)
        for (int ks = 0; ks < F; ++ks) pack_fragment(wp, D, 32 * t, 16 * ks, FRAG_K_NATURAL, to_bf16, img + ((size_t)t * F + ks) * 512);
}

void mlp_fused_plan(int B, int n_patches, int extras, int seq_len, int hidden, MlpFusedArgs& a) {
    const int nchunks = hidden / 32;
    a.nchunks = nchunks;
    a.tok_n = n_patches; a.tok_e = extras; a.tok_l = seq_len;
    a.n_main = B * n_patches;
    a.n_extra = B * extras;
    a.tiles_main = (a.n_main + 127) / 128;
    a.prows = 32;
    a.tiles_left = (a.n_extra + a.prows - 1) / a.prows;
    int g = nchunks / 2 < kGroups ? nchunks / 2 : kGroups;
    if (g < 1) g = 1;
    a.cpg = ((nchunks + g - 1) / g + 1) & ~1;
    a.groups = (nchunks + a.cpg - 1) / a.cpg;
}

size_t mlp_fused_partial_bytes(int max_batch, int extras, int D, int hidden) {
    MlpFusedArgs a{};
    mlp_fused_plan(max_batch, 1, extras, 1 + extras, hidden, a);
    return (size_t)a.tiles_left * a.groups * a.prows * D * sizeof(float);
}
// ... 110 lines not shown
```

include/duodiff_dev.h:

```cpp
#ifndef DUODIFF_DEV_H
#define DUODIFF_DEV_H

#include "duodiff.h"
#include <stddef.h>

#ifdef __cplusplus
extern "C" {
#endif

int dd_dev_mlp(dd_ctx* ctx, int M, int D, int hidden, int extras, const float* h_host, const float* w1, const float* b1,
               const float* w2, const float* b2, float* xres_host, unsigned short* out_host, const float* ln_in,
               const float* ln_out, unsigned short* ln_out_host, int iters, void* stream, float* ms_out,
               const float* ao_host, const float* wproj, const float* bproj, const float* skip_host, const float* wskip,
               const float* bskip, const float* wqkv, unsigned short* qkv_out_host);

int dd_dev_block_tail(dd_ctx* ctx, int B, int n_patches, int extras, int D, int hidden, int last, int poison, const float* h_host,
                      const float* w1, const float* b1, const float* w2, const float* b2, const float* ln_in, const float* ao_host,
                      const float* wproj, const float* bproj, const float* ln_out, const float* skip_host, const float* wskip,
                      const float* bskip, const float* wqkv, float* xres_host, unsigned short* out_host, unsigned short* ln_out_host,
                      unsigned short* frag_host, float* tap_host, unsigned short* qkv_host, float* slab_host, int slab_rows, int* plan_out,
                      int iters, void* stream, float* ms_out);

int dd_dev_qkv_attention(dd_ctx* ctx, int B, int L, int H, int extras, const float* h_host, const float* wqkv, const float* bqkv,
                         unsigned short* out_host, int iters, void* stream, float* ms_out);

int dd_dev_qkv_attention_rows(dd_ctx* ctx, int B, int L, int H, int extras, const float* h_host, const float* wqkv, const float* bqkv,
                              const float* xres_host, const float* ln, unsigned short* out_host, int iters, void* stream, float* ms_out);

int dd_dev_v_identity(dd_ctx* ctx, int B, int L, int H, int extras, const float* h_host, const float* wqkv, const float* bqkv,
                      const float* xres_host, const float* ln, unsigned short* out_host, int iters, void* stream, float* ms_out);

int dd_dev_v_copy(dd_ctx* ctx, int precision, int B, int L, int H, const float* qkv_host, void* out_host, int iters, void* stream,
                  float* ms_out);

int dd_dev_head_dec(dd_ctx* ctx, int M, int D, int pd, int tok_l, int tok_e, const float* x_host, const float* norm_g, const float* norm_b,
                    const float* wdec, const float* bdec, float* dec_host, const float* probe_w, const float* probe_b, float* srow_host,
                    int split, int iters, void* stream, float* ms_out);

int dd_dev_gemm(dd_ctx* ctx, int precision, int M, int N, int K, int K1, const float* A, const float* A2, const float* W, const float* bias,
                int epilogue, int tile128, int hm_L, int hm_H, int splits, int resid, const float* ln, int tok_l, int tok_e,
                float* xres_host, void* out_host, int ldo, unsigned short* h_host, unsigned short* frag_host, float* slab_host,
                int num_cus, int iters, void* stream, float* ms_out);

int dd_dev_rowlin(dd_ctx* ctx, int B, int n_patches, int extras, int K, int k_split, int set_x, const float* A, const float* A2, const float* W,
                  const float* bias, const float* ln, float* xres_host, unsigned short* x_copy_host, unsigned short* h_host, int frag,
                  int iters, void* stream, float* ms_out);

int dd_dev_attention(dd_ctx* ctx, int precision, int B, int L, int H, const float* q, const float* k, const float* v, void* out_host,
                     int iters, void* stream, float* ms_out);

int dd_dev_layernorm(dd_ctx* ctx, int precision, int rows, int D, const float* x_host, const float* gamma_beta, void* out_host,
                     unsigned short* frag_host, int tok_l, int tok_e, int iters, void* stream, float* ms_out);

int dd_dev_embed(dd_ctx* ctx, int B, int C, int S, int P, int D, int extras, int num_classes, int normalize, int generic, const float* x_img,
                 const float* w, const float* bias, const float* pos, const float* label_emb, const long long* y, const float* t_vec,
                 float t_state, const float* ln, float* x_tok_host, unsigned short* ln_frag_host, int iters, void* stream, float* ms_out);

int dd_dev_time_mlp(dd_ctx* ctx, int B, int D, int L, int extras, int normalize, const float* w1, const float* b1, const float* w2,
                    const float* b2, const float* pos, const float* t_vec, float t_state, float* x_tok_host, int iters, void* stream,
                    float* ms_out);

int dd_dev_vae_gather(dd_ctx* ctx, int kind, int precision, int B, int H, int W, int C, const void* src_host, void* dst_host,
                      size_t dst_bytes, void* stream);

#define DD_DEV_NO_FUSED_MLP 1u
#define DD_DEV_NO_FUSED_PROJ 2u
#define DD_DEV_NO_FUSED_HEAD 4u
#define DD_DEV_NO_FUSED_SKIP 32u
#define DD_DEV_NO_FUSED_QKV 64u
#define DD_DEV_NO_FUSED_QA 128u
#define DD_DEV_GENERIC_EMBED 8u
#define DD_DEV_MLP_EXTRAS_ONLY 16u
#define DD_DEV_NO_CHAINS 256u
#define DD_DEV_NO_ROWLIN 1024u
#define DD_DEV_NO_ROWLIN_PROJ 2048u
#define DD_DEV_NO_EMBED_LN 4096u
#define DD_DEV_NO_SPLITK 8192u
#define DD_DEV_NO_ROWLIN_SKIP 16384u
#define DD_DEV_NO_SPLIT_HEADS 32768u
#define DD_DEV_FORCE_CHAINS 512u
int dd_dev_set_flags(dd_ctx* ctx, unsigned flags);

long long dd_dev_graph_captures(dd_ctx* ctx);

int dd_dev_poison_workspaces(dd_ctx* ctx, dd_model* m, void* stream);

int dd_dev_last_sample_chains(dd_ctx* ctx);

#ifdef __cplusplus
}
#endif
#endif
```

Before: 48.30.

## Pass attention output, skip tensors and residual between fused kernels in fragment layout

Adds fragment-ordered buffers for the attention output, the U-Net skip activations and the fp32 residual stream. Producer kernels (fused QKV-attention and the block-tail MLP) write directly in the register-fragment order that the consuming fused kernel loads, so the consumer gets lane-contiguous vector loads instead of row-major gathers. This is meant to cut strided or uncoalesced memory traffic between blocks. The cost is extra workspace (one buffer per skip level) and more branching and register pressure inside the fused kernels. Each path can be disabled with a new flag.

After: 49.93, median of 6. +3.4%, better.

```diff
diff --git a/duodiff_amd/_lib.py b/duodiff_amd/_lib.py
--- a/duodiff_amd/_lib.py
+++ b/duodiff_amd/_lib.py
@@ -17,6 +17,7 @@
 DD_PROF_DOMINANT, DD_PROF_BLOCK_TAIL, DD_PROF_FC1, DD_PROF_ROWLIN, DD_PROF_QKV_ATTENTION, DD_PROF_SPLITK = 0, 1, 2, 3, 4, 5
 DD_DEV_NO_CHAINS, DD_DEV_FORCE_CHAINS, DD_DEV_NO_ROWLIN, DD_DEV_NO_ROWLIN_PROJ, DD_DEV_NO_EMBED_LN, DD_DEV_NO_SPLITK, DD_DEV_NO_ROWLIN_SKIP = 256, 512, 1024, 2048, 4096, 8192, 16384
 DD_DEV_NO_SPLIT_HEADS = 32768
+DD_DEV_NO_FRAG_AO, DD_DEV_NO_FRAG_SKIP, DD_DEV_NO_FRAG_X = 65536, 131072, 262144
 
 
 class dd_config(C.Structure):
@@ -153,6 +154,8 @@
     "dd_dev_v_copy": (C.c_int, [C.c_void_p] + [C.c_int] * 4 + [C.c_void_p] * 2 + [C.c_int, C.c_void_p, C.POINTER(C.c_float)]),
     "dd_dev_mlp": (C.c_int, [C.c_void_p, C.c_int, C.c_int, C.c_int, C.c_int] + [C.c_void_p] * 10 + [C.c_int, C.c_void_p, C.POINTER(C.c_float)] + [C.c_void_p] * 8),
     "dd_dev_block_tail": (C.c_int, [C.c_void_p] + [C.c_int] * 7 + [C.c_void_p] * 21 + [C.c_int, C.c_void_p, C.c_int, C.c_void_p, C.POINTER(C.c_float)]),
+    "dd_dev_block_tail_frag": (C.c_int, [C.c_void_p] + [C.c_int] * 7 + [C.c_void_p] * 21 + [C.c_int, C.c_void_p, C.c_int, C.c_void_p, C.POINTER(C.c_float)] + [C.c_void_p] * 5),
+    "dd_dev_qkv_attention_frag": (C.c_int, [C.c_void_p, C.c_int, C.c_int, C.c_int, C.c_int] + [C.c_void_p] * 7 + [C.c_int, C.c_void_p, C.POINTER(C.c_float)]),
     "dd_dev_head_dec": (C.c_int, [C.c_void_p] + [C.c_int] * 5 + [C.c_void_p] * 9 + [C.c_int, C.c_int, C.c_void_p, C.POINTER(C.c_float)]),
     "dd_dev_gemm": (C.c_int, [C.c_void_p] + [C.c_int] * 5 + [C.c_void_p] * 4 + [C.c_int] * 6 + [C.c_void_p] + [C.c_int] * 2 + [C.c_void_p] * 2 +
                     [C.c_int] + [C.c_void_p] * 3 + [C.c_int, C.c_int, C.c_void_p, C.POINTER(C.c_float)]),
diff --git a/duodiff_amd/csrc/attention.hip b/duodiff_amd/csrc/attention.hip
--- a/duodiff_amd/csrc/attention.hip
+++ b/duodiff_amd/csrc/attention.hip
@@ -358,6 +358,7 @@
     const float* ln_b;
     bf16_t* out;
     int B, L, H, Lp, E;
+    bf16_t* out_frag = nullptr;
 };
 
 constexpr int kQaPxBytes = 8 * 6 * 2 * 32 * 4;
@@ -575,7 +576,9 @@
         float mx, sum;
         attend_tiles<bf16_t, 9, kMaxKeyTiles, true>(Ks, Vt, L, kMaxKeyTiles, lane, [&](int k) { return k; }, qcur, o, mx, sum);
         const float inv = 1.0f / sum;
-        bf16_t* orow = a.out + ((long long)b * L + E + row) * D + hh * kHD;
+        bf16_t* orow = a.out + ((long long)b * L + E + row) * D + hh * kHD + 8 * half;
+        long long ostride = 16;
+        if (a.out_frag) { orow = a.out_frag + ((((long long)b * 8 + wave) * KS + 4 * hh) * 64 + lane) * 8; ostride = 512; }
 #pragma unroll
         for (int dt = 0; dt < 2; ++dt) {
             uint2 v[4];
@@ -590,7 +593,7 @@
             for (int gp = 0; gp < 4; gp += 2) {
                 const auto s0 = __builtin_amdgcn_permlane32_swap(v[gp].x, v[gp + 1].x, false, false);
                 const auto s1 = __builtin_amdgcn_permlane32_swap(v[gp].y, v[gp + 1].y, false, false);
-                *reinterpret_cast<uint4*>(orow + dt * 32 + 8 * gp + 8 * half) = uint4{s0[0], s1[0], s0[1], s1[1]};
+                *reinterpret_cast<uint4*>(orow + (2 * dt + gp / 2) * ostride) = uint4{s0[0], s1[0], s0[1], s1[1]};
             }
         }
     }
@@ -806,9 +809,9 @@
 static size_t qkv_attention_lds() { return (size_t)kLP * AttnLayout<bf16_t>::kRowK + AttnLayout<bf16_t>::kVBytes + kQaAuxBytes + kQaRing; }
 
 hipError_t launch_qkv_attention(const bf16_t* h, const bf16_t* wimg, const float* bias, const bf16_t* hx, const float* xres,
-                                const float* ln_g, const float* ln_b, bf16_t* out, int B, int L, int H, int D, int extras, hipStream_t s) {
+                                const float* ln_g, const float* ln_b, bf16_t* out, int B, int L, int H, int D, int extras, hipStream_t s, bf16_t* out_frag) {
     if (!qkv_attention_supported(D, H, L, extras) || !h || !wimg || (!hx && (!xres || !ln_g || !ln_b)) || !out || B < 1) return hipErrorInvalidValue;
-    const QkvAttnArgs a{h, wimg, bias, hx, xres, ln_g, ln_b, out, B, L, H, make_head_major(L, H).Lp, extras};
+    const QkvAttnArgs a{h, wimg, bias, hx, xres, ln_g, ln_b, out, B, L, H, make_head_major(L, H).Lp, extras, out_frag};
     switch (D) {
         case 512: hipLaunchKernelGGL((qkv_attention_kernel<512>), dim3(B * H), dim3(512), qkv_attention_lds(), s, a); break;
         case 768: hipLaunchKernelGGL((qkv_attention_kernel<768>), dim3(B * H), dim3(512), qkv_attention_lds(), s, a); break;
diff --git a/duodiff_amd/csrc/capi.hip b/duodiff_amd/csrc/capi.hip
--- a/duodiff_amd/csrc/capi.hip
+++ b/duodiff_amd/csrc/capi.hip
@@ -150,6 +150,9 @@
     float* mlp_partial = nullptr;
     bf16_t* qkv_dump = nullptr;
     bf16_t* hfrag = nullptr;
+    bf16_t* aofrag = nullptr;
+    std::vector<bf16_t*> skipfrags;
+    float* xfrag = nullptr;
     float* ytap = nullptr;
 };
 
@@ -182,6 +185,9 @@
     bool rowlin_skip = false;
     bool rowlin_proj = false;
     bool rowlin_fc2 = false;
+    bool frag_ao = false;
+    bool frag_skip = false;
+    bool frag_x = false;
     bool fused_qa = false;
     size_t ws_bytes[2] = {0, 0};
     char* wsarena[2] = {nullptr, nullptr};
@@ -333,6 +339,11 @@
     if (m->fused_qkv) a.space(w.qkv_dump, 16384);
     if (m->fused_qa) a.space(w.hfrag, (size_t)batch * m->N * D * 2);
     if (m->ee_type >= 0 && m->fused_skip) a.space(w.ytap, Mp * D * 4);
+    const size_t patch_elems = (size_t)batch * m->N * D;
+    if (m->frag_ao) a.space(w.aofrag, patch_elems * 2);
+    w.skipfrags.assign(m->frag_skip ? m->half_depth : 0, nullptr);
+    for (bf16_t*& sf : w.skipfrags) a.space(sf, patch_elems * 2);
+    if (m->frag_x) a.space(w.xfrag, patch_elems * 4);
 }
 void choose_paths(dd_model* m, int precision, unsigned flags) {
     const int D = m->D, hid = m->hidden, L = m->L;
@@ -341,6 +352,10 @@
     m->fused_skip = m->fused_proj && (hid / 32) % 2 == 0 && !(flags & DD_DEV_NO_FUSED_SKIP);
     m->fused_qkv = m->fused_proj && m->ee_type < 0 && (hid / 32) % 2 == 0 && !m->cfg.qkv_bias && !(flags & DD_DEV_NO_FUSED_QKV);
     m->fused_qa = precision == DD_PREC_BF16 && qkv_attention_supported(D, m->H, L, m->extras) && !(flags & DD_DEV_NO_FUSED_QA);
+    const bool frag = m->fused_qa && m->fused_proj && D == 512 && m->N % 32 == 0;
+    m->frag_ao = frag && !(flags & DD_DEV_NO_FRAG_AO);
+    m->frag_skip = frag && m->fused_skip && !(flags & DD_DEV_NO_FRAG_SKIP);
+    m->frag_x = frag && m->ee_type < 0 && !(flags & DD_DEV_NO_FRAG_X);
     m->rowlin_fc2 = precision == DD_PREC_BF16 && !m->fused_mlp && rowlin_supported(D, hid) && m->N % 32 == 0 && !(flags & DD_DEV_NO_ROWLIN);
     m->rowlin_proj = m->rowlin_fc2 && !(flags & DD_DEV_NO_ROWLIN_PROJ);
     m->rowlin_skip = m->rowlin_fc2 && rowlin_supported(D, 2 * D) && !(flags & DD_DEV_NO_ROWLIN_SKIP);
@@ -541,6 +556,7 @@
     bool frag = false;
     bool qkv = false;
     bool skip = false;
+    bool xfrag = false;
 };
 
 template <typename T>
@@ -560,6 +576,7 @@
     T *h = (T*)ws.h, *ao = (T*)ws.ao, *qkv = (T*)ws.qkv, *hid = (T*)ws.hid, *xb = (T*)ws.xb;
     float* ee_dec_all = ee && m->ee_batched ? (float*)ws.hid : nullptr;
     float* ee_srow_all = ee_dec_all ? ee_dec_all + (size_t)nb * M * m->pd : nullptr;
+    bool ao_in_frag = false;
 
     int mark(int kind) {
         if (!m->time_fc1 || kind != prof) return DD_OK;
@@ -679,10 +696,12 @@
         }
         const bool masked = (pert_mask >> bi) & 1u;
         const int Bn = masked ? pert_first : B, Bi = B - Bn;
+        ao_in_frag = qa && m->frag_ao && Bi == 0;
         if (qa) {
             if constexpr (bf16) {
                 if (Bn > 0)
-                    DD_TIMED(DD_PROF_QKV_ATTENTION, launch_qkv_attention(ws.hfrag, w.qa_img, w.qkv_b, nullptr, ws.x, w.ln1_g, w.ln1_b, (bf16_t*)ao, Bn, L, m->H, D, m->extras, s));
+                    DD_TIMED(DD_PROF_QKV_ATTENTION, launch_qkv_attention(ws.hfrag, w.qa_img, w.qkv_b, nullptr, ws.x, w.ln1_g, w.ln1_b, (bf16_t*)ao, Bn, L, m->H, D, m->extras, s,
+                                                                         ao_in_frag ? ws.aofrag : nullptr));
                 if (Bi > 0)
                     DD_HIP(c, launch_v_identity(ws.hfrag + (size_t)Bn * m->N * D, w.qa_img, w.qkv_b, ws.x + (size_t)Bn * L * D, w.ln1_g, w.ln1_b,
                                                 (bf16_t*)ao + (size_t)Bn * L * D, Bi, L, m->H, D, m->extras, s));
@@ -719,9 +738,10 @@
         const bool is_in = bi < m->half_depth;
         const BlockW* wn = bi + 1 < nb ? &m->blocks[bi + 1] : nullptr;
         T* copy = is_in ? (T*)ws.skips[bi] : (wn ? xb : nullptr);
+        const Handoff in = next;
         next = Handoff{};
         if constexpr (bf16) {
-            if (m->fused_mlp) return block_tail(bi, copy, next);
+            if (m->fused_mlp) return block_tail(bi, copy, in, next);
         }
         GemmArgs<T> g1{h, nullptr, (const T*)w.fc1_w, w.fc1_b, nullptr, hid, M, m->hidden, D, D, D, 0, m->hid_ld};
         g1.tile128 = tile128(m->hidden, D, D);
@@ -738,20 +758,26 @@
         return DD_OK;
     }
 
-    int block_tail(int bi, T* copy, Handoff& next) {
+    int block_tail(int bi, T* copy, const Handoff in, Handoff& next) {
         const BlockW& w = m->blocks[bi];
         MlpFusedArgs fa{};
         fa.X = nullptr; fa.ldx = D; fa.wimg = w.mlp_img; fa.b1p = w.mlp_b1p; fa.b2 = w.fc2_b;
         fa.ln_in_g = w.ln2_g; fa.ln_in_b = w.ln2_b;
         fa.xres = ws.x; fa.out = (bf16_t*)copy; fa.ldo = D; fa.partial = ws.mlp_partial;
         if (m->fused_proj) { fa.ao = (const bf16_t*)ao; fa.bproj = w.proj_b; fa.nproj = D / 32; }
+        if (ao_in_frag) fa.ao_frag = ws.aofrag;
+        if (m->frag_skip && bi < m->half_depth) fa.out_frag = ws.skipfrags[bi];
         next.skip = m->fused_skip && bi >= m->half_depth && bi + 1 < nb;
         if (next.skip) {
             fa.skip = (const bf16_t*)skip_of(bi + 1);
+            if (m->frag_skip) fa.skip_frag = ws.skipfrags[nb - 1 - (bi + 1)];
             if (ee) fa.y_tap = ws.ytap;
             fa.bskip = m->blocks[bi + 1].skip_b; fa.nskip = D / 16;
         }
         const bool h_next = bi < m->half_depth || next.skip;
+        if (in.xfrag) fa.x_in_frag = ws.xfrag;
+        next.xfrag = m->frag_x && h_next;
+        if (next.xfrag) fa.x_out_frag = ws.xfrag;
         next.frag = m->fused_qa && h_next;
         next.qkv = !next.frag && m->fused_qkv && h_next;
         next.h = h_next && !next.frag && !next.qkv;
diff --git a/duodiff_amd/csrc/dd_internal.h b/duodiff_amd/csrc/dd_internal.h
--- a/duodiff_amd/csrc/dd_internal.h
+++ b/duodiff_amd/csrc/dd_internal.h
@@ -134,6 +134,11 @@
     int prows;
     float* y_tap = nullptr;
     int reduce_set = 0;
+    const bf16_t* ao_frag = nullptr;
+    bf16_t* out_frag = nullptr;
+    const bf16_t* skip_frag = nullptr;
+    const float* x_in_frag = nullptr;
+    float* x_out_frag = nullptr;
 };
 enum FragK { FRAG_K_NATURAL = 0, FRAG_K_ACC = 1 };
 __host__ __device__ constexpr int frag_k_natural(int h, int j) { return 8 * h + j; }
@@ -250,7 +255,8 @@
 bool qkv_attention_supported(int D, int H, int L, int extras);
 void qkv_attention_pack(int D, int H, const float* w, unsigned short (*to_bf16)(float), unsigned short* img);
 hipError_t launch_qkv_attention(const bf16_t* h, const bf16_t* wimg, const float* bias, const bf16_t* hx, const float* xres,
-                                const float* ln_g, const float* ln_b, bf16_t* out, int B, int L, int H, int D, int extras, hipStream_t s);
+                                const float* ln_g, const float* ln_b, bf16_t* out, int B, int L, int H, int D, int extras, hipStream_t s,
+                                bf16_t* out_frag = nullptr);
 
 hipError_t launch_v_identity(const bf16_t* h, const bf16_t* wimg, const float* bias, const float* xres, const float* ln_g, const float* ln_b,
                              bf16_t* out, int B, int L, int H, int D, int extras, hipStream_t s);
diff --git a/duodiff_amd/csrc/dev_harness.hip b/duodiff_amd/csrc/dev_harness.hip
--- a/duodiff_amd/csrc/dev_harness.hip
+++ b/duodiff_amd/csrc/dev_harness.hip
@@ -86,12 +86,15 @@
     return dev.status();
 }
 
-int dd_dev_block_tail(dd_ctx* c, int B, int n_patches, int extras, int D, int hidden, int last, int poison, const float* h_host,
-                      const float* w1, const float* b1, const float* w2, const float* b2, const float* ln_in, const float* ao_host,
-                      const float* wproj, const float* bproj, const float* ln_out, const float* skip_host, const float* wskip,
-                      const float* bskip, const float* wqkv, float* xres_host, unsigned short* out_host, unsigned short* ln_out_host,
-                      unsigned short* frag_host, float* tap_host, unsigned short* qkv_host, float* slab_host, int slab_rows, int* plan_out,
-                      int iters, void* stream, float* ms_out) {
+}
+
+static int block_tail_run(dd_ctx* c, int B, int n_patches, int extras, int D, int hidden, int last, int poison, const float* h_host,
+                          const float* w1, const float* b1, const float* w2, const float* b2, const float* ln_in, const float* ao_host,
+                          const float* wproj, const float* bproj, const float* ln_out, const float* skip_host, const float* wskip,
+                          const float* bskip, const float* wqkv, float* xres_host, unsigned short* out_host, unsigned short* ln_out_host,
+                          unsigned short* frag_host, float* tap_host, unsigned short* qkv_host, float* slab_host, int slab_rows, int* plan_out,
+                          int iters, void* stream, float* ms_out, const unsigned short* ao_frag_host, const unsigned short* skip_frag_host,
+                          const float* xin_frag_host, unsigned short* out_frag_host, float* xout_frag_host) {
     const bool proj = ao_host && wproj && bproj;
     const bool skp = skip_host && wskip && bskip;
     const bool qk = wqkv && qkv_host;
@@ -105,8 +108,15 @@
         return DD_ERR_INVALID;
     if (!mlp_fused_supported(D, hidden)) return ctx_fail(c, DD_ERR_UNSUPPORTED, "fused MLP: D in {64,128,256,512}, hidden % 64 == 0");
     if (frag && skp && extras > 0 && D != 512) return ctx_fail(c, DD_ERR_UNSUPPORTED, "block tail: skip rows without their LayerNorm at D = 512 only");
+    if ((ao_frag_host && !proj) || (skip_frag_host && !skp) || (out_frag_host && !out_host)) return DD_ERR_INVALID;
     hipStream_t s = (hipStream_t)stream;
     const int L = extras + n_patches, M = B * L;
+    const size_t pe = (size_t)B * n_patches * D, guard = (size_t)8 * D;
+    auto rows_patch_poisoned = [&](const float* src) {
+        std::vector<unsigned short> r = bf16_rows(src, M, D, (size_t)round_up(M, 256) + 8, (unsigned char)poison);
+        for (int b = 0; b < B; ++b) std::memset(r.data() + ((size_t)b * L + extras) * D, poison, (size_t)n_patches * D * 2);
+        return r;
+    };
     const size_t Mo = (size_t)round_up(M, 256) + 8, n16 = Mo * D * 2, n32 = Mo * D * 4;
     const MlpImage im = MlpImage::of(D, hidden, proj, skp, qk);
     std::vector<unsigned short> img(im.bytes() / 2, 0);
@@ -126,15 +136,27 @@
     a.wimg = (const char*)dev.upload(img.data(), img.size() * 2);
     a.b1p = dev.upload(b1p.data(), (size_t)hidden * 4); a.b2 = dev.upload(b2, (size_t)D * 4);
     if (ln_in) { a.ln_in_g = dev.upload(ln_in, (size_t)2 * D * 4); a.ln_in_b = a.ln_in_g + D; }
-    a.xres = dev.upload(xres_host, n32);
+    if (xin_frag_host) {
+        std::vector<float> xr(xres_host, xres_host + Mo * D);
+        for (int b = 0; b < B; ++b) std::memset(xr.data() + ((size_t)b * L + extras) * D, poison, (size_t)n_patches * D * 4);
+        a.xres = dev.upload(xr.data(), n32);
+        a.x_in_frag = dev.upload(xin_frag_host, pe * 4);
+    } else {
+        a.xres = dev.upload(xres_host, n32);
+    }
+    if (xout_frag_host) a.x_out_frag = dev.filled<float>((pe + 2 * guard) * 4, 0xFF) + guard;
+    if (out_frag_host) a.out_frag = dev.filled<bf16_t>((pe + 2 * guard) * 2, 0xFF) + guard;
     a.out = out_host ? dev.filled<bf16_t>(n16, 0xFF) : nullptr; a.ldo = D;
     a.partial = slab_rows ? dev.filled<float>((size_t)slab_rows * D * 4, poison) : nullptr;
     if (proj) {
-        a.ao = dev.upload(bf16_rows(ao_host, M, D, Mo, (unsigned char)poison).data(), n16); a.bproj = dev.upload(bproj, (size_t)D * 4); a.nproj = D / 32;
+        a.ao = dev.upload((ao_frag_host ? rows_patch_poisoned(ao_host) : bf16_rows(ao_host, M, D, Mo, (unsigned char)poison)).data(), n16);
+        a.bproj = dev.upload(bproj, (size_t)D * 4); a.nproj = D / 32;
+        if (ao_frag_host) a.ao_frag = dev.upload(ao_frag_host, pe * 2);
         a.reduce_set = 1;
     }
     if (skp) {
-        a.skip = dev.upload(bf16_rows(skip_host, M, D, Mo, (unsigned char)poison).data(), n16);
+        a.skip = dev.upload((skip_frag_host ? rows_patch_poisoned(skip_host) : bf16_rows(skip_host, M, D, Mo, (unsigned char)poison)).data(), n16);
+        if (skip_frag_host) a.skip_frag = dev.upload(skip_frag_host, pe * 2);
         if (tap) a.y_tap = dev.filled<float>(n32, 0xFF);
         a.bskip = dev.upload(bskip, (size_t)D * 4); a.nskip = D / 16;
     }
@@ -166,12 +188,42 @@
     if (tap) dev.download(tap_host, a.y_tap, n32);
     if (qk) dev.download(qkv_host, a.qkv_out, qkv_elems * 2);
     if (slab_rows) dev.download(slab_host, a.partial, (size_t)slab_rows * D * 4);
-    DEV_HIP(dev, time_launches(s, iters, once, ms_out));
-    return dev.status();
-}
-
-int dd_dev_qkv_attention_rows(dd_ctx* c, int B, int L, int H, int extras, const float* h_host, const float* wqkv, const float* bqkv,
-                              const float* xres_host, const float* ln, unsigned short* out_host, int iters, void* stream, float* ms_out) {
+    if (xout_frag_host) dev.download(xout_frag_host, a.x_out_frag - guard, (pe + 2 * guard) * 4);
+    if (out_frag_host) dev.download(out_frag_host, a.out_frag - guard, (pe + 2 * guard) * 2);
+    DEV_HIP(dev, time_launches(s, iters, once, ms_out));
+    return dev.status();
+}
+
+extern "C" {
+
+int dd_dev_block_tail(dd_ctx* c, int B, int n_patches, int extras, int D, int hidden, int last, int poison, const float* h_host,
+                      const float* w1, const float* b1, const float* w2, const float* b2, const float* ln_in, const float* ao_host,
+                      const float* wproj, const float* bproj, const float* ln_out, const float* skip_host, const float* wskip,
+                      const float* bskip, const float* wqkv, float* xres_host, unsigned short* out_host, unsigned short* ln_out_host,
+                      unsigned short* frag_host, float* tap_host, unsigned short* qkv_host, float* slab_host, int slab_rows, int* plan_out,
+                      int iters, void* stream, float* ms_out) {
+    return block_tail_run(c, B, n_patches, extras, D, hidden, last, poison, h_host, w1, b1, w2, b2, ln_in, ao_host, wproj, bproj, ln_out, skip_host, wskip,
+                          bskip, wqkv, xres_host, out_host, ln_out_host, frag_host, tap_host, qkv_host, slab_host, slab_rows, plan_out, iters, stream,
+                          ms_out, nullptr, nullptr, nullptr, nullptr, nullptr);
+}
+
+int dd_dev_block_tail_frag(dd_ctx* c, int B, int n_patches, int extras, int D, int hidden, int last, int poison, const float* h_host,
+                           const float* w1, const float* b1, const float* w2, const float* b2, const float* ln_in, const float* ao_host,
+                           const float* wproj, const float* bproj, const float* ln_out, const float* skip_host, const float* wskip,
+                           const float* bskip, const float* wqkv, float* xres_host, unsigned short* out_host, unsigned short* ln_out_host,
+                           unsigned short* frag_host, float* tap_host, unsigned short* qkv_host, float* slab_host, int slab_rows, int* plan_out,
+                           int iters, void* stream, float* ms_out, const unsigned short* ao_frag_host, const unsigned short* skip_frag_host,
+                           const float* xin_frag_host, unsigned short* out_frag_host, float* xout_frag_host) {
+    return block_tail_run(c, B, n_patches, extras, D, hidden, last, poison, h_host, w1, b1, w2, b2, ln_in, ao_host, wproj, bproj, ln_out, skip_host, wskip,
+                          bskip, wqkv, xres_host, out_host, ln_out_host, frag_host, tap_host, qkv_host, slab_host, slab_rows, plan_out, iters, stream,
+                          ms_out, ao_frag_host, skip_frag_host, xin_frag_host, out_frag_host, xout_frag_host);
+}
+
+}
+
+static int qkv_attention_run(dd_ctx* c, int B, int L, int H, int extras, const float* h_host, const float* wqkv, const float* bqkv,
+                             const float* xres_host, const float* ln, unsigned short* out_host, unsigned short* out_frag_host, int iters, void* stream,
+                             float* ms_out) {
     if (!c || !h_host || !wqkv || !out_host || (xres_host && !ln) || B < 1 || iters < 0) return DD_ERR_INVALID;
     const int D = 64 * H;
     if (!qkv_attention_supported(D, H, L, extras)) return ctx_fail(c, DD_ERR_UNSUPPORTED, "qkv_attention: D = 512 / 768 / 1024, L = 256 + 1 or 2 extra tokens only");
@@ -199,13 +251,30 @@
     const float* dX = xres_host ? dev.upload(xr.data(), xr.size() * 4) : nullptr;
     const float* dL = xres_host ? dev.upload(ln, (size_t)2 * D * 4) : nullptr;
     bf16_t* dO = dev.filled<bf16_t>((M + 8) * D * 2, 0xFF);
+    const size_t pe = (size_t)B * 256 * D, guard = (size_t)8 * D;
+    bf16_t* dF = out_frag_host ? dev.filled<bf16_t>((pe + 2 * guard) * 2, 0xFF) + guard : nullptr;
     const float* dB = bqkv ? dev.upload(bqkv, (size_t)3 * D * 4) : nullptr;
-    auto once = [&]() { return launch_qkv_attention(dH, dW, dB, dQ, dX, dL, dL ? dL + D : nullptr, dO, B, L, H, D, extras, s); };
+    auto once = [&]() { return launch_qkv_attention(dH, dW, dB, dQ, dX, dL, dL ? dL + D : nullptr, dO, B, L, H, D, extras, s, dF); };
     DEV_HIP(dev, once());
     DEV_HIP(dev, hipStreamSynchronize(s));
     dev.download(out_host, dO, (M + 8) * D * 2);
-    DEV_HIP(dev, time_launches(s, iters, once, ms_out));
-    return dev.status();
+    if (out_frag_host) dev.download(out_frag_host, dF - guard, (pe + 2 * guard) * 2);
+    DEV_HIP(dev, time_launches(s, iters, once, ms_out));
+    return dev.status();
+}
+
+extern "C" {
+
+int dd_dev_qkv_attention_rows(dd_ctx* c, int B, int L, int H, int extras, const float* h_host, const float* wqkv, const float* bqkv,
+                              const float* xres_host, const float* ln, unsigned short* out_host, int iters, void* stream, float* ms_out) {
+    return qkv_attention_run(c, B, L, H, extras, h_host, wqkv, bqkv, xres_host, ln, out_host, nullptr, iters, stream, ms_out);
+}
+
+int dd_dev_qkv_attention_frag(dd_ctx* c, int B, int L, int H, int extras, const float* h_host, const float* wqkv, const float* bqkv,
+                              const float* xres_host, const float* ln, unsigned short* out_host, unsigned short* out_frag_host, int iters,
+                              void* stream, float* ms_out) {
+    if (!out_frag_host) return DD_ERR_INVALID;
+    return qkv_attention_run(c, B, L, H, extras, h_host, wqkv, bqkv, xres_host, ln, out_host, out_frag_host, iters, stream, ms_out);
 }
 
 int dd_dev_v_identity(dd_ctx* c, int B, int L, int H, int extras, const float* h_host, const float* wqkv, const float* bqkv,
diff --git a/duodiff_amd/csrc/mlp_fused.hip b/duodiff_amd/csrc/mlp_fused.hip
--- a/duodiff_amd/csrc/mlp_fused.hip
+++ b/duodiff_amd/csrc/mlp_fused.hip
@@ -127,6 +127,8 @@
 template <int D, bool LNIN, bool PARTIAL, bool PROJ, bool SKIP = false, bool QKV = false, bool TAP = false>
 __device__ __forceinline__ void mlp_body(const MlpFusedArgs& a, char* smem, const int tile_idx, const int c0, int c1, const int slab) {
     using C = MlpCfg<D>;
+    constexpr bool FRAG = PROJ && !PARTIAL && !QKV && D == 512;
+    constexpr bool FRAGX = FRAG && !TAP;
     static_assert(!PROJ || (LNIN && C::NT % 4 == 0), "proj fusion: the LayerNorm-in kernel, D % 128 == 0");
     static_assert(!SKIP || (PROJ && !PARTIAL), "skip fusion rides on the proj-fused main tiles");
     static_assert(!QKV || (PROJ && !PARTIAL), "qkv fusion rides on the proj-fused main tiles");
@@ -221,26 +223,40 @@
         __syncthreads();
     } else {
         const float* xr = a.xres + row_pro * D + 4 * h;
+        int xts = 32, xgs = 8;
+        if constexpr (FRAGX) {
+            const bool xfr = a.x_in_frag != nullptr;
+            const int grp = row_ok_pro ? tile_idx * 4 + wave : 0;
+            const float* const xfp = a.x_in_frag + ((long long)grp * (C::NT * 4) * 64 + lane) * 4;
+            xr = xfr ? xfp : xr; xts = xfr ? 1024 : 32; xgs = xfr ? 256 : 8;
+        }
         f32x4 s4 = {0.f, 0.f, 0.f, 0.f}, q4 = {0.f, 0.f, 0.f, 0.f};
         float cshift = 0.f;
         constexpr int LA = C::NT < 4 ? C::NT : (PARTIAL && !PROJ && C::NT >= 8) ? 8 : 4;
         f32x4 xq[LA][4];
         const float* lbp = vecs + 5 * D + 4 * h;
         if constexpr (PROJ) {
-            const bf16_t* ar = a.ao + row_pro * D + 8 * h;
-#pragma unroll
-            for (int ks = 0; ks < C::KS; ++ks) xf[ks] = *reinterpret_cast<const bf16x8*>(ar + 16 * ks);
-            __syncthreads();
+            if (FRAG && a.ao_frag) {
+                const int grp = row_ok_pro ? tile_idx * 4 + wave : 0;
+                const bf16_t* af = a.ao_frag + ((long long)grp * C::KS * 64 + lane) * 8;
+#pragma unroll
+                for (int ks = 0; ks < C::KS; ++ks) xf[ks] = *reinterpret_cast<const bf16x8*>(af + 512 * ks);
+            } else {
+                const bf16_t* ar = a.ao + row_pro * D + 8 * h;
+#pragma unroll
+                for (int ks = 0; ks < C::KS; ++ks) xf[ks] = *reinterpret_cast<const bf16x8*>(ar + 16 * ks);
+            }
         }
 #pragma unroll
         for (int t = 0; t < LA - 1; ++t)
 #pragma unroll
-            for (int g = 0; g < 4; ++g) xq[t][g] = *reinterpret_cast<const f32x4*>(xr + 32 * t + 8 * g);
+            for (int g = 0; g < 4; ++g) xq[t][g] = *reinterpret_cast<const f32x4*>(xr + (FRAGX ? xts * t + xgs * g : 32 * t + 8 * g));
+        if constexpr (PROJ) __syncthreads();
 #pragma unroll
         for (int t = 0; t < C::NT; ++t) {
             if (t + LA - 1 < C::NT) {
 #pragma unroll
-                for (int g = 0; g < 4; ++g) xq[(t + LA - 1) % LA][g] = *reinterpret_cast<const f32x4*>(xr + 32 * (t + LA - 1) + 8 * g);
+                for (int g = 0; g < 4; ++g) xq[(t + LA - 1) % LA][g] = *reinterpret_cast<const f32x4*>(xr + (FRAGX ? xts * (t + LA - 1) + xgs * g : 32 * (t + LA - 1) + 8 * g));
             }
             __builtin_amdgcn_sched_barrier(0);
 #pragma unroll
@@ -448,9 +464,18 @@
     const bf16_t* sr = nullptr;
     if constexpr (SKIP) {
         bool ok_s;
-        sr = a.skip + row_of(ok_s) * D + 8 * half_of();
-#pragma unroll
-        for (int ks = 0; ks < C::F / 2; ++ks) sk[ks] = *reinterpret_cast<const bf16x8*>(sr + 16 * ks);
+        const long long row_s = row_of(ok_s);
+        if (FRAG && a.skip_frag) {
+            unsigned l = (unsigned)threadIdx.x;
+            asm volatile("" : "+v"(l));
+            sr = a.skip_frag + ((long long)(ok_s ? tile_idx * 4 + (int)(l >> 6) : 0) * C::F * 64 + (l & 63)) * 8;
+#pragma unroll
+            for (int ks = 0; ks < C::F / 2; ++ks) sk[ks] = *reinterpret_cast<const bf16x8*>(sr + 512 * ks);
+        } else {
+            sr = a.skip + row_s * D + 8 * half_of();
+#pragma unroll
+            for (int ks = 0; ks < C::F / 2; ++ks) sk[ks] = *reinterpret_cast<const bf16x8*>(sr + 16 * ks);
+        }
     }
     [&]<int... FI>(std::integer_sequence<int, FI...>) {
         ([&] {
@@ -526,8 +551,13 @@
                     if constexpr (p == C::NT) {
                         asm volatile("" ::: "memory");
                         __builtin_amdgcn_sched_barrier(0);
-#pragma unroll
-                        for (int ks = 0; ks < H2; ++ks) xf[ks] = *reinterpret_cast<const bf16x8*>(sr + 16 * (H2 + ks));
+                        if (FRAG && a.skip_frag) {
+#pragma unroll
+                            for (int ks = 0; ks < H2; ++ks) xf[ks] = *reinterpret_cast<const bf16x8*>(sr + 512 * (H2 + ks));
+                        } else {
+#pragma unroll
+                            for (int ks = 0; ks < H2; ++ks) xf[ks] = *reinterpret_cast<const bf16x8*>(sr + 16 * (H2 + ks));
+                        }
                         __builtin_amdgcn_sched_barrier(0);
                         asm volatile("" ::: "memory");
                     }
@@ -575,6 +605,18 @@
         const float* lb2 = vecs + 4 * D + 4 * he;
         float* xrow = (!QKV || row_ok) ? a.xres + row * D + 4 * he : reinterpret_cast<float*>(reinterpret_cast<char*>(a.qkv_dump) + 8192) + 4 * he;
         bf16_t* orow = (!QKV || row_ok) ? a.out + row * a.ldo + 8 * he : reinterpret_cast<bf16_t*>(reinterpret_cast<char*>(a.qkv_dump) + 12288) + 8 * he;
+        int xts = 32, xgs = 8;
+        long long ostride = 16;
+        if constexpr (FRAG) {
+            unsigned l = (unsigned)threadIdx.x;
+            asm volatile("" : "+v"(l));
+            const long long grp = (long long)tile_idx * 4 + (l >> 6);
+            const bool xfr = FRAGX && a.x_out_frag != nullptr, ofr = !SKIP && a.out_frag != nullptr;
+            float* const xfp = a.x_out_frag + (grp * (C::NT * 4) * 64 + (l & 63)) * 4;
+            bf16_t* const ofp = a.out_frag + (grp * C::F * 64 + (l & 63)) * 8;
+            xrow = xfr ? xfp : xrow; xts = xfr ? 1024 : 32; xgs = xfr ? 256 : 8;
+            orow = ofr ? ofp : orow; ostride = ofr ? 512 : 16;
+        }
         f32x4 xl[2][4];
         if constexpr (!LNIN) {
 #pragma unroll
@@ -597,20 +639,20 @@
                 f32x4 q = {yt[4 * g], yt[4 * g + 1], yt[4 * g + 2], yt[4 * g + 3]};
                 if constexpr (!SKIP) q += *reinterpret_cast<const f32x4*>(lb2 + 32 * t + 8 * g);
                 if constexpr (!LNIN) q = xl[t & 1][g] + q;
-                *reinterpret_cast<f32x4*>(xrow + 32 * t + 8 * g) = q;
+                *reinterpret_cast<f32x4*>(xrow + (FRAGX ? xts * t + xgs * g : 32 * t + 8 * g)) = q;
                 v[g] = uint2{cvt_pk_bf16(q[0], q[1]), cvt_pk_bf16(q[2], q[3])};
                 if (t == 0 && g == 0) cshift = q[0];
                 const f32x4 dq = q - cshift;
                 s4 += dq;
                 q4 += dq * dq;
             }
-            if (!SKIP && a.out) {
+            if (!SKIP && (a.out || (FRAG && a.out_frag))) {
 #pragma unroll
                 for (int gp = 0; gp < 4; gp += 2) {
                     const auto s0 = __builtin_amdgcn_permlane32_swap(v[gp].x, v[gp + 1].x, false, false);
                     const auto s1 = __builtin_amdgcn_permlane32_swap(v[gp].y, v[gp + 1].y, false, false);
                     const uint4 o = {s0[0], s1[0], s0[1], s1[1]};
-                    *reinterpret_cast<uint4*>(orow + 32 * t + 8 * gp) = o;
+                    *reinterpret_cast<uint4*>(orow + (FRAG && !SKIP ? (2 * t + gp / 2) * ostride : (long long)(32 * t + 8 * gp))) = o;
                 }
             }
             acc_pin(Y[t]);
@@ -986,6 +1028,11 @@
     if (a.nqkv > 0 && a.nproj <= 0) return hipErrorInvalidValue;
     if (a.y_tap && (a.nskip <= 0 || a.nqkv > 0)) return hipErrorInvalidValue;
     if (a.ln_out_frag && (!a.ln_out || a.nqkv > 0 || a.tok_n % 32)) return hipErrorInvalidValue;
+    if (a.ao_frag || a.x_in_frag || a.x_out_frag || a.out_frag || a.skip_frag) {
+        if (D != 512 || a.nproj <= 0 || a.nqkv > 0 || a.tok_n % 32) return hipErrorInvalidValue;
+        if ((a.x_in_frag || a.x_out_frag) && a.y_tap) return hipErrorInvalidValue;
+        if ((a.out_frag && a.nskip > 0) || (a.skip_frag && a.nskip <= 0)) return hipErrorInvalidValue;
+    }
     if (a.nproj > 0) {
         if constexpr (D % 128 == 0) {
             if (!a.ln_in_g || !a.ao || !a.bproj || a.nproj != D / 32) return hipErrorInvalidValue;
diff --git a/include/duodiff_dev.h b/include/duodiff_dev.h
--- a/include/duodiff_dev.h
+++ b/include/duodiff_dev.h
@@ -21,11 +21,23 @@
                       unsigned short* frag_host, float* tap_host, unsigned short* qkv_host, float* slab_host, int slab_rows, int* plan_out,
                       int iters, void* stream, float* ms_out);
 
+int dd_dev_block_tail_frag(dd_ctx* ctx, int B, int n_patches, int extras, int D, int hidden, int last, int poison, const float* h_host,
+                           const float* w1, const float* b1, const float* w2, const float* b2, const float* ln_in, const float* ao_host,
+                           const float* wproj, const float* bproj, const float* ln_out, const float* skip_host, const float* wskip,
+                           const float* bskip, const float* wqkv, float* xres_host, unsigned short* out_host, unsigned short* ln_out_host,
+                           unsigned short* frag_host, float* tap_host, unsigned short* qkv_host, float* slab_host, int slab_rows, int* plan_out,
+                           int iters, void* stream, float* ms_out, const unsigned short* ao_frag_host, const unsigned short* skip_frag_host,
+                           const float* xin_frag_host, unsigned short* out_frag_host, float* xout_frag_host);
+
 int dd_dev_qkv_attention(dd_ctx* ctx, int B, int L, int H, int extras, const float* h_host, const float* wqkv, const float* bqkv,
                          unsigned short* out_host, int iters, void* stream, float* ms_out);
 
 int dd_dev_qkv_attention_rows(dd_ctx* ctx, int B, int L, int H, int extras, const float* h_host, const float* wqkv, const float* bqkv,
                               const float* xres_host, const float* ln, unsigned short* out_host, int iters, void* stream, float* ms_out);
+
+int dd_dev_qkv_attention_frag(dd_ctx* ctx, int B, int L, int H, int extras, const float* h_host, const float* wqkv, const float* bqkv,
+                              const float* xres_host, const float* ln, unsigned short* out_host, unsigned short* out_frag_host, int iters,
+                              void* stream, float* ms_out);
 
 int dd_dev_v_identity(dd_ctx* ctx, int B, int L, int H, int extras, const float* h_host, const float* wqkv, const float* bqkv,
                       const float* xres_host, const float* ln, unsigned short* out_host, int iters, void* stream, float* ms_out);
@@ -78,6 +90,9 @@
 #define DD_DEV_NO_SPLITK 8192u
 #define DD_DEV_NO_ROWLIN_SKIP 16384u
 #define DD_DEV_NO_SPLIT_HEADS 32768u
+#define DD_DEV_NO_FRAG_AO 65536u
+#define DD_DEV_NO_FRAG_SKIP 131072u
+#define DD_DEV_NO_FRAG_X 262144u
 #define DD_DEV_FORCE_CHAINS 512u
 int dd_dev_set_flags(dd_ctx* ctx, unsigned flags);
 
```
